# bryanlimy/tf2-cyclegan

Measured on AMD Instinct MI355X. Metric: images/sec (whole node) horse2zebra 256×256, higher is better.
Workload: dtype bf16; 1 GPU; model=cyclegan-resnet9-patchgan, global_batch=4, per_gpu_batch=4, image_size=256, parallelism=dp1

## Files before the change

cyclegan_amd/ops/_hip/bind.cpp:

```cpp
#include <torch/extension.h>

namespace cyg {
at::Tensor conv2d_fwd(at::Tensor, at::Tensor, c10::optional<at::Tensor>,
                      int64_t, int64_t, int64_t, int64_t, int64_t, bool,
                      int64_t, double);
at::Tensor convt2d_fwd(at::Tensor, at::Tensor, c10::optional<at::Tensor>,
                       int64_t, int64_t, int64_t, int64_t, int64_t, int64_t,
                       double);
at::Tensor conv2d_dgrad(at::Tensor, at::Tensor, int64_t, int64_t, int64_t,
                        int64_t, int64_t, int64_t, int64_t, bool);
at::Tensor convt2d_dgrad(at::Tensor, at::Tensor, int64_t, int64_t, int64_t,
                         int64_t, int64_t);
at::Tensor conv2d_wgrad(at::Tensor, at::Tensor, int64_t, int64_t, int64_t,
                        int64_t, int64_t, bool);
at::Tensor mfma_probe(at::Tensor, at::Tensor);
at::Tensor mx_probe(at::Tensor, at::Tensor, int64_t, int64_t);
at::Tensor mx_probe16(at::Tensor, at::Tensor, int64_t, int64_t);
at::Tensor glds_probe(at::Tensor, at::Tensor);
at::Tensor tr_probe(int64_t);
at::Tensor quant_fp8(at::Tensor, at::Tensor);
at::Tensor quant_fp8_d(at::Tensor, at::Tensor, at::Tensor);
void amax_roll(at::Tensor, int64_t);
at::Tensor conv2d_fp8_fwd(at::Tensor, at::Tensor, at::Tensor,
                          c10::optional<at::Tensor>, c10::optional<at::Tensor>,
                          int64_t, int64_t, int64_t, int64_t, int64_t, bool, int64_t, double);
std::vector<at::Tensor> instnorm_fwd(at::Tensor, at::Tensor, at::Tensor,
                                     double, int64_t, double,
                                     c10::optional<at::Tensor>);
std::vector<at::Tensor> instnorm_bwd(at::Tensor, at::Tensor, at::Tensor,
                                     at::Tensor, at::Tensor,
                                     c10::optional<at::Tensor>, int64_t,
                                     double);
at::Tensor act_bwd(at::Tensor, at::Tensor, int64_t, double);
at::Tensor channel_sum(at::Tensor);
at::Tensor reflect_pad_fwd(at::Tensor, int64_t, int64_t, int64_t, int64_t);
at::Tensor reflect_pad_bwd(at::Tensor, int64_t, int64_t, int64_t, int64_t);
at::Tensor persample_loss_fwd(at::Tensor, at::Tensor, bool);
at::Tensor persample_loss_const_fwd(at::Tensor, double, bool);
std::vector<at::Tensor> persample_loss_bwd(at::Tensor, at::Tensor, at::Tensor,
                                           bool, bool, bool);
at::Tensor persample_loss_const_bwd(at::Tensor, double, at::Tensor, bool);
void adam_step_dev(at::Tensor, at::Tensor, at::Tensor, at::Tensor, at::Tensor,
                   double, double, double);
void shadow_gather(at::Tensor, at::Tensor, at::Tensor);
void adam_step(at::Tensor, at::Tensor, at::Tensor, at::Tensor, double, double,
               double, double, int64_t);
}

PYBIND11_MODULE(TORCH_EXTENSION_NAME, m) {
  m.def("conv2d_fwd", &cyg::conv2d_fwd);
  m.def("convt2d_fwd", &cyg::convt2d_fwd);
  m.def("conv2d_dgrad", &cyg::conv2d_dgrad);
  m.def("convt2d_dgrad", &cyg::convt2d_dgrad);
  m.def("conv2d_wgrad", &cyg::conv2d_wgrad);
  m.def("mfma_probe", &cyg::mfma_probe);
  m.def("mx_probe", &cyg::mx_probe);
  m.def("mx_probe16", &cyg::mx_probe16);
  m.def("glds_probe", &cyg::glds_probe);
  m.def("tr_probe", &cyg::tr_probe);
  m.def("quant_fp8", &cyg::quant_fp8);
  m.def("quant_fp8_d", &cyg::quant_fp8_d);
  m.def("amax_roll", &cyg::amax_roll);
  m.def("conv2d_fp8_fwd", &cyg::conv2d_fp8_fwd);
  m.def("instnorm_fwd", &cyg::instnorm_fwd);
  m.def("instnorm_bwd", &cyg::instnorm_bwd);
  m.def("act_bwd", &cyg::act_bwd);
  m.def("channel_sum", &cyg::channel_sum);
  m.def("reflect_pad_fwd", &cyg::reflect_pad_fwd);
  m.def("reflect_pad_bwd", &cyg::reflect_pad_bwd);
  m.def("persample_loss_fwd", &cyg::persample_loss_fwd);
  m.def("persample_loss_const_fwd", &cyg::persample_loss_const_fwd);
  m.def("persample_loss_bwd", &cyg::persample_loss_bwd);
  m.def("persample_loss_const_bwd", &cyg::persample_loss_const_bwd);
  m.def("adam_step", &cyg::adam_step);
  m.def("adam_step_dev", &cyg::adam_step_dev);
  m.def("shadow_gather", &cyg::shadow_gather);
}
```

cyclegan_amd/ops/_hip/conv.hip:

```cpp

#include <torch/extension.h>
#include <ATen/cuda/CUDAContext.h>

#include "common.h"

namespace cyg {

constexpr int BM = 128, BN = 64, BK = 64;
constexpr int NTHREADS = 256;
constexpr int LDK = BK + 8;

struct ConvParams {
  const short* __restrict__ x;
  const short* __restrict__ w;
  const short* __restrict__ bias;
  short* __restrict__ y;
  int B, H, W, Cin, OH, OW, Cout, KH, KW;
  int stride, pt, pl;
  int reflect;
  int act;  float slope;
  const float* dq;
  const float* dqb;
  long M, KTOT;
  int mtiles, ntiles;
};

DEV int xcd_chunk(int bid, int nb) {
  return (nb % 8 == 0) ? (bid % 8) * (nb / 8) + bid / 8 : bid;
}


template <bool IS_CONVT, bool ALIGNED, int STRIDE>
__global__ __launch_bounds__(NTHREADS) void conv_gemm_kernel(ConvParams p) {
  const int stride = STRIDE ? STRIDE : p.stride;
  __shared__ short As[BM][LDK];
  __shared__ short Bs[BN][LDK];
  __shared__ long rowxb[BM];
  __shared__ long rowyb[BM];
  __shared__ int rowih[BM], rowiw[BM];
  __shared__ char rowok[BM];

  const int tid = threadIdx.x;
  const int lane = tid & 63;
  const int wid = tid >> 6;
  const int bid = xcd_chunk(blockIdx.x, gridDim.x);
  const int mt = bid % p.mtiles, nt = bid / p.mtiles;
  const long m0 = (long)mt * BM;
  const int n0 = nt * BN;

  for (int r = tid; r < BM; r += NTHREADS) {
    long m = m0 + r;
    bool ok = m < p.M;
    long mm = ok ? m : 0;
    int ow = (int)(mm % p.OW);
    int oh = (int)((mm / p.OW) % p.OH);
    int b = (int)(mm / ((long)p.OW * p.OH));
    rowok[r] = ok;
    rowxb[r] = (long)b * p.H * p.W * p.Cin;
    rowyb[r] = ((long)(b * p.OH + oh) * p.OW + ow) * p.Cout;
    if (IS_CONVT) {
      rowih[r] = oh + p.pt;
      rowiw[r] = ow + p.pl;
    } else {
      rowih[r] = oh * stride - p.pt;
      rowiw[r] = ow * stride - p.pl;
    }
  }
  __syncthreads();

  v4f acc[4][2] = {};

  const int wr = wid >> 1, wc = wid & 1;
  const int wm0 = wr * 64, wn0 = wc * 32;
  const int fr = lane & 15;
  const int fg = lane >> 4;

  for (long k0 = 0; k0 < p.KTOT; k0 += BK) {
    if (ALIGNED) {
      #pragma unroll 2
      for (int c = tid; c < BM * (BK / 8); c += NTHREADS) {
        int row = c >> 3;
        int kc = (c & 7) * 8;
        long k = k0 + kc;
        v8s val = {};
        if (k < p.KTOT && rowok[row]) {
          int tap = (int)(k / p.Cin);
          int ci = (int)(k - (long)tap * p.Cin);
          int dkh = tap / p.KW, dkw = tap - (tap / p.KW) * p.KW;
          bool valid = true;
          int ih, iw;
          if (IS_CONVT) {
            int nh = rowih[row] - dkh, nw = rowiw[row] - dkw;
            valid = nh >= 0 && nw >= 0 && (nh % stride) == 0 &&
                    (nw % stride) == 0;
            ih = nh / stride; iw = nw / stride;
            valid = valid && ih < p.H && iw < p.W;
          } else {
            ih = rowih[row] + dkh; iw = rowiw[row] + dkw;
            if (p.reflect) {
              ih = mirror_idx(ih, p.H); iw = mirror_idx(iw, p.W);
            } else {
              valid = ih >= 0 && ih < p.H && iw >= 0 && iw < p.W;
            }
          }
          if (valid)
            val = *(const v8s*)(p.x + rowxb[row] + ((long)ih * p.W + iw) * p.Cin + ci);
        }
        *(v8s*)&As[row][kc] = val;
      }
    } else {
      for (int c = tid; c < BM * BK; c += NTHREADS) {
        int row = c >> 6;
        int kc = c & 63;
        long k = k0 + kc;
        short val = 0;
        if (k < p.KTOT && rowok[row]) {
          int tap = (int)(k / p.Cin);
          int ci = (int)(k - (long)tap * p.Cin);
          int dkh = tap / p.KW, dkw = tap - (tap / p.KW) * p.KW;
          bool valid = true;
          int ih, iw;
          if (IS_CONVT) {
            int nh = rowih[row] - dkh, nw = rowiw[row] - dkw;
            valid = nh >= 0 && nw >= 0 && (nh % stride) == 0 &&
                    (nw % stride) == 0;
            ih = nh / stride; iw = nw / stride;
            valid = valid && ih < p.H && iw < p.W;
          } else {
            ih = rowih[row] + dkh; iw = rowiw[row] + dkw;
            if (p.reflect) {
              ih = mirror_idx(ih, p.H); iw = mirror_idx(iw, p.W);
            } else {
              valid = ih >= 0 && ih < p.H && iw >= 0 && iw < p.W;
            }
          }
          if (valid)
            val = p.x[rowxb[row] + ((long)ih * p.W + iw) * p.Cin + ci];
        }
        As[row][kc] = val;
      }
    }

    if (ALIGNED) {
      #pragma unroll 2
      for (int c = tid; c < BN * (BK / 8); c += NTHREADS) {
        int n = c >> 3;
        int kc = (c & 7) * 8;
        long k = k0 + kc;
        v8s val = {};
        if (n0 + n < p.Cout && k < p.KTOT)
          val = *(const v8s*)(p.w + (long)(n0 + n) * p.KTOT + k);
        *(v8s*)&Bs[n][kc] = val;
      }
    } else {
      for (int c = tid; c < BN * BK; c += NTHREADS) {
        int n = c >> 6;
        int kc = c & 63;
        long k = k0 + kc;
        Bs[n][kc] = (n0 + n < p.Cout && k < p.KTOT)
                        ? p.w[(long)(n0 + n) * p.KTOT + k] : (short)0;
      }
    }
    __syncthreads();

    #pragma unroll
    for (int kk = 0; kk < BK; kk += 32) {
      v8bf a0 = *(const v8bf*)&As[wm0 + 0 * 16 + fr][kk + fg * 8];
      v8bf a1 = *(const v8bf*)&As[wm0 + 1 * 16 + fr][kk + fg * 8];
      v8bf a2 = *(const v8bf*)&As[wm0 + 2 * 16 + fr][kk + fg * 8];
      v8bf a3 = *(const v8bf*)&As[wm0 + 3 * 16 + fr][kk + fg * 8];
      v8bf b0 = *(const v8bf*)&Bs[wn0 + 0 * 16 + fr][kk + fg * 8];
      v8bf b1 = *(const v8bf*)&Bs[wn0 + 1 * 16 + fr][kk + fg * 8];
      acc[0][0] = __builtin_amdgcn_mfma_f32_16x16x32_bf16(a0, b0, acc[0][0], 0, 0, 0);
      acc[0][1] = __builtin_amdgcn_mfma_f32_16x16x32_bf16(a0, b1, acc[0][1], 0, 0, 0);
      acc[1][0] = __builtin_amdgcn_mfma_f32_16x16x32_bf16(a1, b0, acc[1][0], 0, 0, 0);
      acc[1][1] = __builtin_amdgcn_mfma_f32_16x16x32_bf16(a1, b1, acc[1][1], 0, 0, 0);
      acc[2][0] = __builtin_amdgcn_mfma_f32_16x16x32_bf16(a2, b0, acc[2][0], 0, 0, 0);
      acc[2][1] = __builtin_amdgcn_mfma_f32_16x16x32_bf16(a2, b1, acc[2][1], 0, 0, 0);
      acc[3][0] = __builtin_amdgcn_mfma_f32_16x16x32_bf16(a3, b0, acc[3][0], 0, 0, 0);
      acc[3][1] = __builtin_amdgcn_mfma_f32_16x16x32_bf16(a3, b1, acc[3][1], 0, 0, 0);
    }
    __syncthreads();
  }

  #pragma unroll
  for (int nf = 0; nf < 2; ++nf) {
    int n = n0 + wn0 + nf * 16 + fr;
    if (n >= p.Cout) continue;
    float bv = p.bias ? b2f(p.bias[n]) : 0.f;
    #pragma unroll
    for (int mf = 0; mf < 4; ++mf) {
      #pragma unroll
      for (int r = 0; r < 4; ++r) {
        int rl = wm0 + mf * 16 + fg * 4 + r;
        if (!rowok[rl]) continue;
        float v = apply_act(acc[mf][nf][r] + bv, p.act, p.slope);
        p.y[rowyb[rl] + n] = f2b(v);
      }
    }
  }
}


template <int NBUF, int BNT = BN>
struct ConvSmemT {
  long rowyb[BM];
  int rowih[BM], rowiw[BM];
  unsigned rowxb[BM];
  char rowok[BM];
  char _pad[16 - (BM % 16 ? BM % 16 : 16)];
  short A[NBUF][BM * BK];
  short Bt[NBUF][BNT * BK];
};
using ConvSmem = ConvSmemT<2>;

template <bool IS_CONVT, int STRIDE, int NBUF = 2, int NW = 4, int BNT = BN,
          bool PHASED = false>
__global__ __launch_bounds__(NW * 64) void conv_glds_kernel(ConvParams p) {
  constexpr int NT = NW * 64;
  constexpr int API = 16 / NW;
  constexpr int TBI = BNT / 8;
  constexpr int BPI = TBI >= NW ? TBI / NW : 1;
  constexpr int NF = BNT >= 32 ? 2 : 1;
  constexpr int NWC = BNT / (NF * 16);
  constexpr int NWR = NW / NWC;
  constexpr int MF = (BM / NWR) / 16;
  const int stride = STRIDE ? STRIDE : p.stride;
  extern __shared__ __attribute__((aligned(16))) char smem_raw[];
  auto& sm = *reinterpret_cast<ConvSmemT<NBUF, BNT>*>(smem_raw);

  const int tid = threadIdx.x;
  const int lane = tid & 63;
  const int w = tid >> 6;
  const int bid = (IS_CONVT && STRIDE == 2)
                      ? blockIdx.x : xcd_chunk(blockIdx.x, gridDim.x);
  const int mt = bid % p.mtiles, nt = bid / p.mtiles;
  const int n0 = nt * BNT;

  static_assert(!PHASED || (IS_CONVT && STRIDE == 2), "PHASED");
  const int tpp = PHASED ? (p.mtiles >> 2) : 0;
  const int phase = PHASED ? mt / tpp : 0;
  const int phh = phase >> 1, phw = phase & 1;
  const int OH2 = p.OH >> 1, OW2 = p.OW >> 1;
  const long m0 = PHASED ? (long)(mt - phase * tpp) * BM : (long)mt * BM;
  const int nvh = PHASED ? ((p.KH - phh + 1) >> 1) : 0;
  const int nvw = PHASED ? ((p.KW - phw + 1) >> 1) : 0;
  const long KEFF = PHASED ? (long)nvh * nvw * p.Cin : p.KTOT;

  for (int r = tid; r < BM; r += NT) {
    if (PHASED) {
      long mp = m0 + r;
      long Mp = (long)p.B * OH2 * OW2;
      bool ok = mp < Mp;
      long mm = ok ? mp : 0;
      int owp = (int)(mm % OW2);
      int ohp = (int)((mm / OW2) % OH2);
      int b = (int)(mm / ((long)OW2 * OH2));
      int i = 2 * ohp + ((phh + p.pt) & 1);
      int j = 2 * owp + ((phw + p.pl) & 1);
      sm.rowok[r] = ok && i < p.OH && j < p.OW;
      sm.rowxb[r] = (unsigned)((long)b * p.H * p.W * p.Cin * 2);
      sm.rowyb[r] = ((long)(b * p.OH + i) * p.OW + j) * p.Cout;
      sm.rowih[r] = (i + p.pt - phh) >> 1;
      sm.rowiw[r] = (j + p.pl - phw) >> 1;
    } else {
      long m = m0 + r;
      bool ok = m < p.M;
      long mm = ok ? m : 0;
      int ow = (int)(mm % p.OW);
      int oh = (int)((mm / p.OW) % p.OH);
      int b = (int)(mm / ((long)p.OW * p.OH));
      sm.rowok[r] = ok;
      sm.rowxb[r] = (unsigned)((long)b * p.H * p.W * p.Cin * 2);
      sm.rowyb[r] = ((long)(b * p.OH + oh) * p.OW + ow) * p.Cout;
      if (IS_CONVT) {
        sm.rowih[r] = oh + p.pt;
        sm.rowiw[r] = ow + p.pl;
      } else {
        sm.rowih[r] = oh * stride - p.pt;
        sm.rowiw[r] = ow * stride - p.pl;
      }
    }
  }
  __syncthreads();

  const int lr = lane >> 3;
  const int klog = ((lane & 7) ^ lr) << 3;
  int aih[API], aiw[API];
  unsigned axb[API];
  bool aok[API];
  #pragma unroll
  for (int j = 0; j < API; ++j) {
    int r = (w * API + j) * 8 + lr;
    aih[j] = sm.rowih[r];
    aiw[j] = sm.rowiw[r];
    axb[j] = sm.rowxb[r];
    aok[j] = sm.rowok[r];
  }
  int bn[BPI];
  #pragma unroll
  for (int j = 0; j < BPI; ++j) bn[j] = (w * BPI + j) * 8 + lr + n0;
  const bool bw_on = w * BPI < TBI;
  static_assert(BNT == 16 || BNT == 64 || BNT == 128, "BNT");

  auto rx = __builtin_amdgcn_make_buffer_rsrc(
      (void*)p.x, 0, (unsigned)((long)p.B * p.H * p.W * p.Cin * 2), 0x00020000);
  auto rw = __builtin_amdgcn_make_buffer_rsrc(
      (void*)p.w, 0, (unsigned)(p.Cout * p.KTOT * 2), 0x00020000);

  const int nk = (int)((KEFF + BK - 1) / BK);
  const bool big_ci = p.Cin >= BK;

  long kcur;
  bool kv;
  int ci, dkh, dkw;
  unsigned avo[API];
  bool avalid[API];
  unsigned bvo[BPI];
  bool bnv[BPI];

  auto recompute_a = [&]() {
    #pragma unroll
    for (int j = 0; j < API; ++j) {
      avalid[j] = false;
      avo[j] = 0xFF000000u;
      if (!aok[j]) continue;
      bool valid = true;
      int ih, iw;
      if (PHASED) {
        ih = aih[j] - dkh; iw = aiw[j] - dkw;
        valid = ih >= 0 && iw >= 0 && ih < p.H && iw < p.W;
      } else if (IS_CONVT) {
        int nh = aih[j] - dkh, nw = aiw[j] - dkw;
        valid = nh >= 0 && nw >= 0 && (nh % stride) == 0 && (nw % stride) == 0;
        ih = nh / stride; iw = nw / stride;
        valid = valid && ih < p.H && iw < p.W;
      } else {
        ih = aih[j] + dkh; iw = aiw[j] + dkw;
        if (p.reflect) {
          ih = mirror_idx(ih, p.H); iw = mirror_idx(iw, p.W);
        } else {
          valid = ih >= 0 && ih < p.H && iw >= 0 && iw < p.W;
        }
      }
      if (valid) {
        avalid[j] = true;
        avo[j] = axb[j] + (unsigned)((((long)ih * p.W + iw) * p.Cin + ci) * 2);
      }
    }
  };

  auto recompute_b = [&]() {
    long kw_idx = kcur;
    if (PHASED)
      kw_idx = ((long)(2 * dkh + phh) * p.KW + (2 * dkw + phw)) * p.Cin + ci;
    #pragma unroll
    for (int j = 0; j < BPI; ++j)
      bvo[j] = (unsigned)(((long)bn[j] * p.KTOT + kw_idx) * 2);
  };

  auto decode_tap = [&]() {
    int tap = (int)(kcur / p.Cin);
    ci = (int)(kcur - (long)tap * p.Cin);
    if (PHASED) {
      dkh = tap / nvw;
      dkw = tap - dkh * nvw;
    } else {
      dkh = tap / p.KW;
      dkw = tap - dkh * p.KW;
    }
  };

  auto init_state = [&]() {
    kcur = klog;
    kv = kcur < KEFF;
    decode_tap();
    recompute_a();
    #pragma unroll
    for (int j = 0; j < BPI; ++j) bnv[j] = bn[j] < p.Cout;
    recompute_b();
  };

  auto advance = [&]() {
    kcur += BK;
    kv = kcur < KEFF;
    if (big_ci) {
      ci += BK;
      if (ci >= p.Cin) {
        ci -= p.Cin;
        if (PHASED) {
          if (++dkw == nvw) { dkw = 0; ++dkh; }
        } else {
          if (++dkw == p.KW) { dkw = 0; ++dkh; }
        }
        recompute_a();
        recompute_b();
      } else {
        #pragma unroll
        for (int j = 0; j < API; ++j) avo[j] += BK * 2;
        #pragma unroll
        for (int j = 0; j < BPI; ++j) bvo[j] += BK * 2;
      }
    } else {
      decode_tap();
      recompute_a();
      recompute_b();
    }
  };

  auto stage = [&](int buf) {
    #pragma unroll
    for (int j = 0; j < API; ++j) {
      unsigned vo = (kv && avalid[j]) ? avo[j] : 0xFF000000u;
      __builtin_amdgcn_raw_ptr_buffer_load_lds(
          rx, (__attribute__((address_space(3))) void*)&sm.A[buf][(w * API + j) * 512],
          16, vo, 0, 0, 0);
    }
    if (bw_on) {
      #pragma unroll
      for (int j = 0; j < BPI; ++j) {
        unsigned vo = (kv && bnv[j]) ? bvo[j] : 0xFF000000u;
        __builtin_amdgcn_raw_ptr_buffer_load_lds(
            rw, (__attribute__((address_space(3))) void*)&sm.Bt[buf][(w * BPI + j) * 512],
            16, vo, 0, 0, 0);
      }
    }
  };

  v4f acc[MF][NF] = {};
  const int wr = w / NWC, wc = w % NWC;
  const int wm0 = wr * (MF * 16), wn0 = wc * (NF * 16);
  const int fr = lane & 15;
  const int fg = lane >> 4;
  const int swz = (fr & 7) << 4;

  init_state();
  stage(0);
  __syncthreads();
#ifdef CYG_DEBUG_EPI
  if (bid == 0 && tid == 0)
    printf("dbg NW=%d BNT=%d API=%d TBI=%d BPI=%d NF=%d NWC=%d MF=%d nk=%d "
           "kv=%d klog=%d bvo0=%u bnv0=%d avo0=%u avalid0=%d "
           "A0123=%d %d %d %d Bt0123=%d %d %d %d\n",
           NW, BNT, API, TBI, BPI, NF, NWC, MF, nk, (int)kv, klog, bvo[0],
           (int)bnv[0], avo[0], (int)avalid[0],
           (int)sm.A[0][0], (int)sm.A[0][1], (int)sm.A[0][2], (int)sm.A[0][3],
           (int)sm.Bt[0][0], (int)sm.Bt[0][1], (int)sm.Bt[0][2],
           (int)sm.Bt[0][3]);
#endif

  for (int kt = 0; kt < nk; ++kt) {
    if (kt + 1 < nk) {
      advance();
      stage((kt + 1) & 1);
    }
    const char* Ab = (const char*)sm.A[kt & 1];
    const char* Bb = (const char*)sm.Bt[kt & 1];
    #pragma unroll
    for (int kk = 0; kk < BK; kk += 32) {
      const int kbyte = (kk + fg * 8) * 2;
      v8bf a[MF], b[NF];
      #pragma unroll
      for (int mf = 0; mf < MF; ++mf)
        a[mf] = *(const v8bf*)(Ab + ((wm0 + mf * 16 + fr) << 7) + (kbyte ^ swz));
      #pragma unroll
      for (int nf = 0; nf < NF; ++nf)
        b[nf] = *(const v8bf*)(Bb + ((wn0 + nf * 16 + fr) << 7) + (kbyte ^ swz));
      #pragma unroll
      for (int mf = 0; mf < MF; ++mf)
        #pragma unroll
        for (int nf = 0; nf < NF; ++nf)
          acc[mf][nf] = __builtin_amdgcn_mfma_f32_16x16x32_bf16(
              a[mf], b[nf], acc[mf][nf], 0, 0, 0);
    }
    __syncthreads();
  }

  #pragma unroll
  for (int nf = 0; nf < NF; ++nf) {
    int n = n0 + wn0 + nf * 16 + fr;
    if (n >= p.Cout) continue;
    float bv = p.bias ? b2f(p.bias[n]) : 0.f;
    #pragma unroll
    for (int mf = 0; mf < MF; ++mf) {
      #pragma unroll
      for (int r = 0; r < 4; ++r) {
        int rl = wm0 + mf * 16 + fg * 4 + r;
        if (!sm.rowok[rl]) continue;
#ifdef CYG_DEBUG_EPI
        if (sm.rowyb[rl] < 0 || sm.rowyb[rl] + n >= p.M * p.Cout) {
          printf("EPI OOB bid=%d tid=%d rl=%d rowyb=%ld n=%d\n",
                 bid, tid, rl, (long)sm.rowyb[rl], n);
          continue;
        }
#endif
        float v = apply_act(acc[mf][nf][r] + bv, p.act, p.slope);
        p.y[sm.rowyb[rl] + n] = f2b(v);
      }
    }
  }
}

constexpr int HB_BM = 64;

template <int NW = 4>
__global__ __launch_bounds__(NW * 64) void conv_halo_kernel(ConvParams p) {
  constexpr int NT = NW * 64;
  const int tid = threadIdx.x;
  const int lane = tid & 63;
  const int w = tid >> 6;
  const int tiles_w = (p.OW + HB_BM - 1) / HB_BM;
  const int bid = xcd_chunk(blockIdx.x, gridDim.x);
  const int owt = bid % tiles_w;
  const int t2 = bid / tiles_w;
  const int oh = t2 % p.OH;
  const int b = t2 / p.OH;
  const int ow0 = owt * HB_BM;
  const int CW = HB_BM + p.KW - 1;
  constexpr int CG = 8;
  constexpr int SL = CG + 1;
  constexpr int halves = 2;
  const int nk = p.KH * p.KW * halves;

  extern __shared__ __attribute__((aligned(16))) char smem_raw[];
  short* xs = (short*)smem_raw;
  const int xgr = p.KH * CW * SL;
  const int xgr_pad = ((xgr + NT - 1) / NT) * NT;

  auto rx = __builtin_amdgcn_make_buffer_rsrc(
      (void*)p.x, 0, (unsigned)((long)p.B * p.H * p.W * p.Cin * 2),
      0x00020000);

  const long xbase = (long)b * p.H * p.W * p.Cin;
  {
    int g = w * 64 + lane;
    int chs = g % SL;
    int pix = g / SL;
    int col = pix % CW;
    int row = pix / CW;
    constexpr int dpix = NT / SL;
    constexpr int dchs = NT - dpix * SL;
    for (int g0 = 0; g0 < xgr_pad; g0 += NT) {
      unsigned vo = 0xFF000000u;
      if (row < p.KH && chs < CG) {
        int ih = oh - p.pt + row;
        int iw = ow0 - p.pl + col;
        bool okp = true;
        if (p.reflect) {
          ih = mirror_idx(ih, p.H);
          iw = mirror_idx(iw, p.W);
        } else {
          okp = ih >= 0 && ih < p.H && iw >= 0 && iw < p.W;
        }
        if (okp)
          vo = (unsigned)((xbase + ((long)ih * p.W + iw) * p.Cin + chs * 8) * 2);
      }
      __builtin_amdgcn_raw_ptr_buffer_load_lds(
          rx, (__attribute__((address_space(3))) void*)(xs + (long)(g0 + w * 64) * 8),
          16, vo, 0, 0, 0);
      chs += dchs;
      col += dpix;
      if (chs >= SL) { chs -= SL; ++col; }
      while (col >= CW) { col -= CW; ++row; }
    }
  }

  __syncthreads();

  constexpr int KSPLIT = NW >= 8 ? 2 : 1;
  const int mf = KSPLIT > 1 ? (w & 3) : w;
  const int kh2 = KSPLIT > 1 ? (w >> 2) : 0;
  const int fr = lane & 15;
  const int fg = lane >> 4;
  const int p0 = mf * 16;
  const v8bf bz = {};
  v4f acc = {};
  const int k0 = kh2 * (nk / KSPLIT);
  const int k1 = (kh2 == KSPLIT - 1) ? nk : (kh2 + 1) * (nk / KSPLIT);
  int tap = k0 / halves, h = k0 - tap * halves;
  int ty = tap / p.KW, tx = tap - ty * p.KW;
  #pragma unroll 8
  for (int kt = k0; kt < k1; ++kt) {
    int col = p0 + fr + tx;
    int chs = h * 4 + fg;
    v8bf a = *(const v8bf*)(xs + (((ty * CW + col) * SL + chs) << 3));
    v8bf bf = bz;
    if (fr < 8)
      bf = *(const v8bf*)(p.w + (long)fr * p.KTOT + kt * 32 + fg * 8);
    acc = __builtin_amdgcn_mfma_f32_16x16x32_bf16(a, bf, acc, 0, 0, 0);
    if (++h == halves) {
      h = 0;
      ++tap;
      if (++tx == p.KW) { tx = 0; ++ty; }
    }
  }

  if (KSPLIT > 1) {
    __syncthreads();
    float* red = (float*)xs;
    if (kh2 == 1)
      *(v4f*)&red[(mf * 64 + lane) * 4] = acc;
    __syncthreads();
    if (kh2 != 0) return;
    acc += *(const v4f*)&red[(mf * 64 + lane) * 4];
  }

  if (fr < p.Cout) {
    float bv = p.bias ? b2f(p.bias[fr]) : 0.f;
    #pragma unroll
    for (int r = 0; r < 4; ++r) {
      int ow = ow0 + p0 + fg * 4 + r;
      if (ow >= p.OW) continue;
      float v = apply_act(acc[r] + bv, p.act, p.slope);
      p.y[(((long)b * p.OH + oh) * p.OW + ow) * p.Cout + fr] = f2b(v);
    }
  }
}


#include <hip/hip_fp8.h>

constexpr int BKF = 128;
typedef int v4i __attribute__((ext_vector_type(4)));
typedef int v8i __attribute__((ext_vector_type(8)));

struct Fp8Smem {
  unsigned char A[2][BM * BKF];
  unsigned char Bt[2][BN * BKF];
  long rowyb[BM];
  int rowih[BM], rowiw[BM];
  unsigned rowxb[BM];
  char rowok[BM];
};

__global__ void quant_fp8_kernel(const short* __restrict__ x,
                                 const float* __restrict__ scale,
                                 unsigned char* __restrict__ y, long n) {
  long i = ((long)blockIdx.x * blockDim.x + threadIdx.x) * 8;
  float s = scale[0];
  if (i + 8 <= n) {
    v8s v = *(const v8s*)(x + i);
    unsigned char out[8];
    #pragma unroll
    for (int j = 0; j < 8; ++j) {
      __hip_fp8_e4m3 q(b2f(v[j]) * s);
      out[j] = q.__x;
    }
    *(uint2*)(y + i) = *(uint2*)out;
  } else if (i < n) {
    for (long k = i; k < n; ++k) {
      __hip_fp8_e4m3 q(b2f(x[k]) * scale[0]);
      y[k] = q.__x;
    }
  }
}

DEV float delayed_sx(float amax_prev) {
  return fminf(448.f / fmaxf(amax_prev, 1e-12f), 65504.f);
}

__global__ __launch_bounds__(256) void quant_fp8_d_kernel(
    const short* __restrict__ x, const float* __restrict__ amax_prev,
    float* __restrict__ amax_cur, unsigned char* __restrict__ y, long n) {
  const float s = delayed_sx(amax_prev[0]);
  float mx = 0.f;
  long t = (long)blockIdx.x * 256 + threadIdx.x;
  long nthreads = (long)gridDim.x * 256;
  for (long i = t * 8; i + 8 <= n; i += nthreads * 8) {
    v8s v = *(const v8s*)(x + i);
    unsigned char out[8];
    #pragma unroll
    for (int j = 0; j < 8; ++j) {
      float f = b2f(v[j]);
      mx = fmaxf(mx, fabsf(f));
      __hip_fp8_e4m3 q(f * s);
      out[j] = q.__x;
    }
    *(uint2*)(y + i) = *(uint2*)out;
  }
  if (blockIdx.x == 0 && threadIdx.x == 0) {
    for (long k = n & ~7L; k < n; ++k) {
      float f = b2f(x[k]);
      mx = fmaxf(mx, fabsf(f));
      __hip_fp8_e4m3 q(f * s);
      y[k] = q.__x;
    }
  }
  __shared__ float red[256];
  red[threadIdx.x] = mx;
  __syncthreads();
  for (int off = 128; off > 0; off >>= 1) {
    if (threadIdx.x < off)
      red[threadIdx.x] = fmaxf(red[threadIdx.x], red[threadIdx.x + off]);
    __syncthreads();
  }
  if (threadIdx.x == 0)
    atomicMax((unsigned*)amax_cur, __float_as_uint(red[0]));
}

__global__ void amax_roll_kernel(float* __restrict__ arena, int n, int cap) {
  int i = blockIdx.x * blockDim.x + threadIdx.x;
  if (i < n) {
    arena[i] = arena[cap + i];
    arena[cap + i] = 0.f;
  }
}

template <int STRIDE>
__global__ __launch_bounds__(NTHREADS) void conv_fp8_kernel(ConvParams p) {
  const int stride = STRIDE ? STRIDE : p.stride;
  __shared__ Fp8Smem sm;

  const int tid = threadIdx.x;
  const int lane = tid & 63;
  const int w = tid >> 6;
  const int bid = xcd_chunk(blockIdx.x, gridDim.x);
  const int mt = bid % p.mtiles, nt = bid / p.mtiles;
  const long m0 = (long)mt * BM;
  const int n0 = nt * BN;
  const bool reflect = p.reflect != 0;

  for (int r = tid; r < BM; r += NTHREADS) {
    long m = m0 + r;
    bool ok = m < p.M;
    long mm = ok ? m : 0;
    int ow = (int)(mm % p.OW);
    int oh = (int)((mm / p.OW) % p.OH);
    int b = (int)(mm / ((long)p.OW * p.OH));
    sm.rowok[r] = ok;
    sm.rowxb[r] = (unsigned)((long)b * p.H * p.W * p.Cin);
    sm.rowyb[r] = ((long)(b * p.OH + oh) * p.OW + ow) * p.Cout;
    sm.rowih[r] = oh * stride - p.pt;
    sm.rowiw[r] = ow * stride - p.pl;
  }
  __syncthreads();

  const int lr = lane >> 3;
  const int klog = ((lane & 7) ^ lr) << 4;
  int aih[4], aiw[4];
  unsigned axb[4];
  bool aok[4];
  #pragma unroll
  for (int j = 0; j < 4; ++j) {
    int r = w * 32 + j * 8 + lr;
    aih[j] = sm.rowih[r];
    aiw[j] = sm.rowiw[r];
    axb[j] = sm.rowxb[r];
    aok[j] = sm.rowok[r];
  }
  const int bn[2] = {(w * 2 + 0) * 8 + lr + n0, (w * 2 + 1) * 8 + lr + n0};

  auto rx = __builtin_amdgcn_make_buffer_rsrc(
      (void*)p.x, 0, (unsigned)((long)p.B * p.H * p.W * p.Cin), 0x00020000);
  auto rw = __builtin_amdgcn_make_buffer_rsrc(
      (void*)p.w, 0, (unsigned)(p.Cout * p.KTOT), 0x00020000);

  const int nk = (int)((p.KTOT + BKF - 1) / BKF);
  const bool big_ci = p.Cin >= BKF;

  long kcur;
  bool kv;
  int ci, dkh, dkw;
  unsigned avo[4], bvo[2];
  bool avalid[4], bnv[2];

  auto recompute_a = [&]() {
    #pragma unroll
    for (int j = 0; j < 4; ++j) {
      avalid[j] = false;
      avo[j] = 0xFF000000u;
      if (!aok[j]) continue;
      bool valid = true;
      int ih = aih[j] + dkh, iw = aiw[j] + dkw;
      if (reflect) {
        ih = mirror_idx(ih, p.H); iw = mirror_idx(iw, p.W);
      } else {
        valid = ih >= 0 && ih < p.H && iw >= 0 && iw < p.W;
      }
      if (valid) {
        avalid[j] = true;
        avo[j] = axb[j] + (unsigned)(((long)ih * p.W + iw) * p.Cin + ci);
      }
    }
  };

  auto init_state = [&]() {
    kcur = klog;
    kv = kcur < p.KTOT;
    int tap = (int)(kcur / p.Cin);
    ci = (int)(kcur - (long)tap * p.Cin);
    dkh = tap / p.KW;
    dkw = tap - dkh * p.KW;
    recompute_a();
    #pragma unroll
    for (int j = 0; j < 2; ++j) {
      bnv[j] = bn[j] < p.Cout;
      bvo[j] = (unsigned)((long)bn[j] * p.KTOT + kcur);
    }
  };

  auto advance = [&]() {
    kcur += BKF;
    kv = kcur < p.KTOT;
    #pragma unroll
    for (int j = 0; j < 2; ++j) bvo[j] += BKF;
    if (big_ci) {
      ci += BKF;
      if (ci >= p.Cin) {
        ci -= p.Cin;
        if (++dkw == p.KW) { dkw = 0; ++dkh; }
        recompute_a();
      } else {
        #pragma unroll
        for (int j = 0; j < 4; ++j) avo[j] += BKF;
      }
    } else {
      int tap = (int)(kcur / p.Cin);
      ci = (int)(kcur - (long)tap * p.Cin);
      dkh = tap / p.KW;
      dkw = tap - dkh * p.KW;
      recompute_a();
    }
  };

  auto stage = [&](int buf) {
    #pragma unroll
    for (int j = 0; j < 4; ++j) {
      unsigned vo = (kv && avalid[j]) ? avo[j] : 0xFF000000u;
      __builtin_amdgcn_raw_ptr_buffer_load_lds(
          rx, (__attribute__((address_space(3))) void*)&sm.A[buf][(w * 4 + j) * 1024],
          16, vo, 0, 0, 0);
    }
    #pragma unroll
    for (int j = 0; j < 2; ++j) {
      unsigned vo = (kv && bnv[j]) ? bvo[j] : 0xFF000000u;
      __builtin_amdgcn_raw_ptr_buffer_load_lds(
          rw, (__attribute__((address_space(3))) void*)&sm.Bt[buf][(w * 2 + j) * 1024],
          16, vo, 0, 0, 0);
    }
  };

  v4f acc[4][2] = {};
  const int wr = w >> 1, wc = w & 1;
  const int wm0 = wr * 64, wn0 = wc * 32;
  const int fr = lane & 15;
  const int fg = lane >> 4;
  const int swz = (fr & 7) << 4;

  init_state();
  stage(0);
  __syncthreads();

  for (int kt = 0; kt < nk; ++kt) {
    if (kt + 1 < nk) {
      advance();
      stage((kt + 1) & 1);
    }
    const char* Ab = (const char*)sm.A[kt & 1];
    const char* Bb = (const char*)sm.Bt[kt & 1];
    {
      const int c0 = (fg * 32) ^ swz;
      const int c1 = (fg * 32 + 16) ^ swz;
      v8i fa[4], fb[2];
      #pragma unroll
      for (int mf = 0; mf < 4; ++mf) {
        const char* r = Ab + ((wm0 + mf * 16 + fr) << 7);
        v4i lo = *(const v4i*)(r + c0);
        v4i hi = *(const v4i*)(r + c1);
        fa[mf] = __builtin_shufflevector(lo, hi, 0, 1, 2, 3, 4, 5, 6, 7);
      }
      #pragma unroll
      for (int nf = 0; nf < 2; ++nf) {
        const char* r = Bb + ((wn0 + nf * 16 + fr) << 7);
        v4i lo = *(const v4i*)(r + c0);
        v4i hi = *(const v4i*)(r + c1);
        fb[nf] = __builtin_shufflevector(lo, hi, 0, 1, 2, 3, 4, 5, 6, 7);
      }
      #pragma unroll
      for (int mf = 0; mf < 4; ++mf)
        #pragma unroll
        for (int nf = 0; nf < 2; ++nf)
          acc[mf][nf] = __builtin_amdgcn_mfma_scale_f32_16x16x128_f8f6f4(
              fa[mf], fb[nf], acc[mf][nf], 0, 0, 0, 127, 0, 127);
    }
    __syncthreads();
  }

  const float dqs = p.dq
      ? (p.dqb ? 1.f / (delayed_sx(p.dq[0]) * p.dqb[0]) : p.dq[0])
      : 1.f;
  #pragma unroll
  for (int nf = 0; nf < 2; ++nf) {
    int n = n0 + wn0 + nf * 16 + fr;
    if (n >= p.Cout) continue;
    float bv = p.bias ? b2f(p.bias[n]) : 0.f;
    #pragma unroll
    for (int mf = 0; mf < 4; ++mf) {
      #pragma unroll
      for (int r = 0; r < 4; ++r) {
        int rl = wm0 + mf * 16 + fg * 4 + r;
        if (!sm.rowok[rl]) continue;
        float v = apply_act(acc[mf][nf][r] * dqs + bv, p.act, p.slope);
        p.y[sm.rowyb[rl] + n] = f2b(v);
      }
    }
  }
}


struct WgradParams {
  const short* __restrict__ x;
  const short* __restrict__ dy;
  float* __restrict__ dw;
  float* __restrict__ ws;
  int B, H, W, Cin, OH, OW, Cout, KH, KW;
  int stride, pt, pl, reflect;
  long M, KTOT;
  int ktiles, ntiles, slices;
  long mchunks_per_slice;
};

constexpr int WG_BK = 128;
constexpr int WG_BN = 64;
constexpr int WG_BM = 64;
constexpr int WG_LDM = WG_BM + 8;

__global__ __launch_bounds__(NTHREADS) void wgrad_kernel(WgradParams p) {
  __shared__ short At[WG_BK][WG_LDM];
  __shared__ short Dt[WG_BN][WG_LDM];
  __shared__ int mih[2][WG_BM], miw[2][WG_BM];
  __shared__ long mxb[2][WG_BM];
  __shared__ char mok[2][WG_BM];

  const int tid = threadIdx.x;
  const int lane = tid & 63;
  const int wid = tid >> 6;
  const int wbid = xcd_chunk(blockIdx.x, gridDim.x);
  const int kt = wbid % p.ktiles;
  const int nt = (wbid / p.ktiles) % p.ntiles;
  const int sl = wbid / (p.ktiles * p.ntiles);
  const long k0 = (long)kt * WG_BK;
  const int n0 = nt * WG_BN;
  const long mstart = sl * p.mchunks_per_slice * WG_BM;
  long mend = mstart + p.mchunks_per_slice * WG_BM;
  if (mend > p.M) mend = p.M;

  v4f acc[4][2] = {};
  const int wr = wid >> 1, wc = wid & 1;
  const int wk0 = wr * 64, wn0 = wc * 32;
  const int fr = lane & 15, fg = lane >> 4;

  const bool a_vec = (p.Cin % 8) == 0;
  const bool d_vec = (p.Cout % 8) == 0;

  if (a_vec && d_vec && mstart < mend) {
    const int a_mloc = (tid & 15) * 4, a_kc = (tid >> 4) * 8;
    const int d_mloc = (tid & 31) * 2, d_nc = (tid >> 5) * 8;
    const long ak = k0 + a_kc;
    const bool akv = ak < p.KTOT;
    int tap = akv ? (int)(ak / p.Cin) : 0;
    const int ci = (int)(ak - (long)tap * p.Cin);
    const int dkh = tap / p.KW, dkw = tap - (tap / p.KW) * p.KW;
    const bool dnv = n0 + d_nc < p.Cout;

    auto decode = [&](int buf, long ms) {
      for (int r = tid; r < WG_BM; r += NTHREADS) {
        bool ok = ms + r < p.M;
        int mm = ok ? (int)(ms + r) : 0;
        int ow = mm % p.OW;
        int t = mm / p.OW;
        int oh = t % p.OH;
        int b = t / p.OH;
        mok[buf][r] = ok;
        mih[buf][r] = oh * p.stride - p.pt;
        miw[buf][r] = ow * p.stride - p.pl;
        mxb[buf][r] = (long)b * p.H * p.W * p.Cin;
      }
    };

    const v8s VZERO = {};
    v8s areg[4], dreg[2];
    auto load_regs = [&](int buf, long ms) {
      #pragma unroll
      for (int u = 0; u < 4; ++u) {
        areg[u] = VZERO;
        if (akv && mok[buf][a_mloc + u]) {
          int ih = mih[buf][a_mloc + u] + dkh;
          int iw = miw[buf][a_mloc + u] + dkw;
          bool valid = true;
          if (p.reflect) {
            ih = mirror_idx(ih, p.H); iw = mirror_idx(iw, p.W);
          } else {
            valid = ih >= 0 && ih < p.H && iw >= 0 && iw < p.W;
          }
          if (valid)
            areg[u] = *(const v8s*)(p.x + mxb[buf][a_mloc + u] +
                                    ((long)ih * p.W + iw) * p.Cin + ci);
        }
      }
      #pragma unroll
      for (int u = 0; u < 2; ++u) {
        dreg[u] = VZERO;
        long m = ms + d_mloc + u;
        if (dnv && m < p.M)
          dreg[u] = *(const v8s*)(p.dy + m * p.Cout + n0 + d_nc);
      }
    };

    decode(0, mstart);
    __syncthreads();
    load_regs(0, mstart);

    int cur = 0;
    for (long ms = mstart; ms < mend; ms += WG_BM, cur ^= 1) {
      #pragma unroll
      for (int j = 0; j < 8; ++j) {
        short pa[4] = {areg[0][j], areg[1][j], areg[2][j], areg[3][j]};
        *(uint2*)&At[a_kc + j][a_mloc] = *(uint2*)pa;
        short pd[2] = {dreg[0][j], dreg[1][j]};
        *(unsigned*)&Dt[d_nc + j][d_mloc] = *(unsigned*)pd;
      }
      bool more = ms + WG_BM < mend;
      if (more) decode(cur ^ 1, ms + WG_BM);
      __syncthreads();
      if (more) load_regs(cur ^ 1, ms + WG_BM);
      #pragma unroll
      for (int kk = 0; kk < WG_BM; kk += 32) {
        v8bf a0 = *(const v8bf*)&At[wk0 + 0 * 16 + fr][kk + fg * 8];
        v8bf a1 = *(const v8bf*)&At[wk0 + 1 * 16 + fr][kk + fg * 8];
        v8bf a2 = *(const v8bf*)&At[wk0 + 2 * 16 + fr][kk + fg * 8];
        v8bf a3 = *(const v8bf*)&At[wk0 + 3 * 16 + fr][kk + fg * 8];
        v8bf b0 = *(const v8bf*)&Dt[wn0 + 0 * 16 + fr][kk + fg * 8];
        v8bf b1 = *(const v8bf*)&Dt[wn0 + 1 * 16 + fr][kk + fg * 8];
        acc[0][0] = __builtin_amdgcn_mfma_f32_16x16x32_bf16(a0, b0, acc[0][0], 0, 0, 0);
        acc[0][1] = __builtin_amdgcn_mfma_f32_16x16x32_bf16(a0, b1, acc[0][1], 0, 0, 0);
        acc[1][0] = __builtin_amdgcn_mfma_f32_16x16x32_bf16(a1, b0, acc[1][0], 0, 0, 0);
        acc[1][1] = __builtin_amdgcn_mfma_f32_16x16x32_bf16(a1, b1, acc[1][1], 0, 0, 0);
        acc[2][0] = __builtin_amdgcn_mfma_f32_16x16x32_bf16(a2, b0, acc[2][0], 0, 0, 0);
        acc[2][1] = __builtin_amdgcn_mfma_f32_16x16x32_bf16(a2, b1, acc[2][1], 0, 0, 0);
        acc[3][0] = __builtin_amdgcn_mfma_f32_16x16x32_bf16(a3, b0, acc[3][0], 0, 0, 0);
        acc[3][1] = __builtin_amdgcn_mfma_f32_16x16x32_bf16(a3, b1, acc[3][1], 0, 0, 0);
      }
      __syncthreads();
    }

    #pragma unroll
    for (int nf = 0; nf < 2; ++nf) {
      int n = n0 + wn0 + nf * 16 + fr;
      if (n >= p.Cout) continue;
      #pragma unroll
      for (int kf = 0; kf < 4; ++kf) {
        #pragma unroll
        for (int r = 0; r < 4; ++r) {
          long k = k0 + wk0 + kf * 16 + fg * 4 + r;
          if (k < p.KTOT)
            atomicAdd(&p.dw[(long)n * p.KTOT + k], acc[kf][nf][r]);
        }
      }
    }
    return;
  }

  for (long ms = mstart; ms < mend; ms += WG_BM) {
    __syncthreads();
    for (int r = tid; r < WG_BM; r += NTHREADS) {
      int m = (int)(ms + r);
      bool ok = ms + r < p.M;
      int mm = ok ? m : 0;
      int ow = mm % p.OW;
      int t = mm / p.OW;
      int oh = t % p.OH;
      int b = t / p.OH;
      mok[0][r] = ok;
      mih[0][r] = oh * p.stride - p.pt;
      miw[0][r] = ow * p.stride - p.pl;
      mxb[0][r] = (long)b * p.H * p.W * p.Cin;
    }
    __syncthreads();
    {
      for (int c = tid; c < WG_BK * 8; c += NTHREADS) {
        int krow = c >> 3;
        int mc = (c & 7) * 8;
        long k = k0 + krow;
        short vals[8];
        int tap = 0, ci = 0, dkh = 0, dkw = 0;
        bool krows_ok = k < p.KTOT;
        if (krows_ok) {
          tap = (int)(k / p.Cin);
          ci = (int)(k - (long)tap * p.Cin);
          dkh = tap / p.KW; dkw = tap - dkh * p.KW;
        }
        #pragma unroll
        for (int j = 0; j < 8; ++j) {
          long m = ms + mc + j;
          short v = 0;
          if (krows_ok && m < p.M) {
            int ow = (int)(m % p.OW);
            int oh = (int)((m / p.OW) % p.OH);
            int b = (int)(m / ((long)p.OW * p.OH));
            int ih = oh * p.stride - p.pt + dkh;
            int iw = ow * p.stride - p.pl + dkw;
            bool valid = true;
            if (p.reflect) {
              ih = mirror_idx(ih, p.H); iw = mirror_idx(iw, p.W);
            } else {
              valid = ih >= 0 && ih < p.H && iw >= 0 && iw < p.W;
            }
            if (valid)
              v = p.x[(((long)b * p.H + ih) * p.W + iw) * p.Cin + ci];
          }
          vals[j] = v;
        }
        *(v8s*)&At[krow][mc] = *(v8s*)vals;
      }
    }
    if (d_vec) {
      for (int c = tid; c < (WG_BM / 2) * (WG_BN / 8); c += NTHREADS) {
        int m_loc = (c % (WG_BM / 2)) * 2;
        int nc = (c / (WG_BM / 2)) * 8;
        v8s v0 = {}, v1 = {};
        if (n0 + nc < p.Cout) {
          long m = ms + m_loc;
          if (m < p.M) v0 = *(const v8s*)(p.dy + m * p.Cout + n0 + nc);
          if (m + 1 < p.M) v1 = *(const v8s*)(p.dy + (m + 1) * p.Cout + n0 + nc);
        }
        #pragma unroll
        for (int j = 0; j < 8; ++j) {
          short pack[2] = {v0[j], v1[j]};
          *(unsigned*)&Dt[nc + j][m_loc] = *(unsigned*)pack;
        }
      }
    } else {
      for (int c = tid; c < WG_BN * 8; c += NTHREADS) {
        int n = c >> 3;
        int mc = (c & 7) * 8;
        short vals[8];
        #pragma unroll
        for (int j = 0; j < 8; ++j) {
          long m = ms + mc + j;
          vals[j] = (n0 + n < p.Cout && m < p.M)
                        ? p.dy[m * p.Cout + n0 + n] : (short)0;
        }
        *(v8s*)&Dt[n][mc] = *(v8s*)vals;
      }
    }
    __syncthreads();

    #pragma unroll
    for (int kk = 0; kk < WG_BM; kk += 32) {
      v8bf a0 = *(const v8bf*)&At[wk0 + 0 * 16 + fr][kk + fg * 8];
      v8bf a1 = *(const v8bf*)&At[wk0 + 1 * 16 + fr][kk + fg * 8];
      v8bf a2 = *(const v8bf*)&At[wk0 + 2 * 16 + fr][kk + fg * 8];
      v8bf a3 = *(const v8bf*)&At[wk0 + 3 * 16 + fr][kk + fg * 8];
      v8bf b0 = *(const v8bf*)&Dt[wn0 + 0 * 16 + fr][kk + fg * 8];
      v8bf b1 = *(const v8bf*)&Dt[wn0 + 1 * 16 + fr][kk + fg * 8];
      acc[0][0] = __builtin_amdgcn_mfma_f32_16x16x32_bf16(a0, b0, acc[0][0], 0, 0, 0);
      acc[0][1] = __builtin_amdgcn_mfma_f32_16x16x32_bf16(a0, b1, acc[0][1], 0, 0, 0);
      acc[1][0] = __builtin_amdgcn_mfma_f32_16x16x32_bf16(a1, b0, acc[1][0], 0, 0, 0);
      acc[1][1] = __builtin_amdgcn_mfma_f32_16x16x32_bf16(a1, b1, acc[1][1], 0, 0, 0);
      acc[2][0] = __builtin_amdgcn_mfma_f32_16x16x32_bf16(a2, b0, acc[2][0], 0, 0, 0);
      acc[2][1] = __builtin_amdgcn_mfma_f32_16x16x32_bf16(a2, b1, acc[2][1], 0, 0, 0);
      acc[3][0] = __builtin_amdgcn_mfma_f32_16x16x32_bf16(a3, b0, acc[3][0], 0, 0, 0);
      acc[3][1] = __builtin_amdgcn_mfma_f32_16x16x32_bf16(a3, b1, acc[3][1], 0, 0, 0);
    }
    __syncthreads();
  }

  #pragma unroll
  for (int nf = 0; nf < 2; ++nf) {
    int n = n0 + wn0 + nf * 16 + fr;
    if (n >= p.Cout) continue;
    #pragma unroll
    for (int kf = 0; kf < 4; ++kf) {
      #pragma unroll
      for (int r = 0; r < 4; ++r) {
        long k = k0 + wk0 + kf * 16 + fg * 4 + r;
        if (k < p.KTOT)
          atomicAdd(&p.dw[(long)n * p.KTOT + k], acc[kf][nf][r]);
      }
    }
  }
}


typedef bf16r v4bfx __attribute__((ext_vector_type(4)));

#define AXOR(row) ((((row) & 7) << 5) | ((((row) >> 3) & 1) << 4))
#define DXOR(row) ((((row) & 3) << 5) | ((((row) >> 3) & 1) << 4))

DEV v4bfx tr16_read(const char* plds) {
  return __builtin_amdgcn_ds_read_tr16_b64_v4bf16(
      (__attribute__((address_space(3))) v4bfx*)plds);
}

template <int WBN, int KT = 1>
struct WgSmemT {
  short A[2][KT * WG_BM * WG_BK];
  short D[2][WG_BM * WBN];
};

template <int NW = 4, int WBN = 64, int KT = 1>
__global__ __launch_bounds__(NW * 64) void wgrad_glds_kernel(WgradParams p) {
  constexpr int API = 16 / NW;
  constexpr int AT = KT * API;
  constexpr int DCH = WBN / 8;
  constexpr int DRPI = 64 / DCH;
  constexpr int TDI = (WG_BM * DCH) / 64;
  constexpr int DPI = TDI >= NW ? TDI / NW : 1;
  constexpr int NFW = (NW == 4 && WBN == 128) ? 4 : (WBN >= 32 ? 2 : 1);
  constexpr int NWCW = WBN / (NFW * 16);
  constexpr int KF = (WG_BK / (NW / NWCW)) / 16;
  extern __shared__ __attribute__((aligned(16))) char wg_smem_raw[];
  auto& sm = *reinterpret_cast<WgSmemT<WBN, KT>*>(wg_smem_raw);

  const int tid = threadIdx.x;
  const int lane = tid & 63;
  const int w = tid >> 6;
  const int wbid = xcd_chunk(blockIdx.x, gridDim.x);
  const int pairs = p.ktiles / KT;
  const int ktp = wbid % pairs;
  const int kt = ktp * KT;
  const int nt = (wbid / pairs) % p.ntiles;
  const int sl = wbid / (pairs * p.ntiles);
  const long k0 = (long)kt * WG_BK;
  const int n0 = nt * WBN;
  const long mstart = sl * p.mchunks_per_slice * WG_BM;
  long mend = mstart + p.mchunks_per_slice * WG_BM;
  if (mend > p.M) mend = p.M;
  if (mstart >= mend) {
    for (int t = 0; t < KT; ++t) {
      long chunk = (((long)sl * p.ktiles + kt + t) * p.ntiles + nt) *
                   ((long)WBN * WG_BK);
      for (int i = tid; i < WBN * WG_BK; i += NW * 64) p.ws[chunk + i] = 0.f;
    }
    return;
  }

  auto rx = __builtin_amdgcn_make_buffer_rsrc(
      (void*)p.x, 0, (unsigned)((long)p.B * p.H * p.W * p.Cin * 2), 0x00020000);
  auto rd = __builtin_amdgcn_make_buffer_rsrc(
      (void*)p.dy, 0, (unsigned)(p.M * p.Cout * 2), 0x00020000);

  int a_row[AT], a_ci[AT], a_dkh[AT], a_dkw[AT];
  bool a_kv[AT];
  #pragma unroll
  for (int t = 0; t < KT; ++t) {
    #pragma unroll
    for (int j = 0; j < API; ++j) {
      int sidx = t * API + j;
      int row = (w * API + j) * 4 + (lane >> 4);
      int cb = ((lane & 15) * 16) ^ AXOR(row);
      long k = k0 + (long)t * WG_BK + cb / 2;
      a_row[sidx] = row;
      a_kv[sidx] = k < p.KTOT;
      int tap = a_kv[sidx] ? (int)(k / p.Cin) : 0;
      a_ci[sidx] = (int)(k - (long)tap * p.Cin);
      a_dkh[sidx] = tap / p.KW;
      a_dkw[sidx] = tap - a_dkh[sidx] * p.KW;
    }
  }
  const bool dw_on = w * DPI < TDI;
  int d_row[DPI], d_n[DPI];
  #pragma unroll
  for (int j = 0; j < DPI; ++j) {
    int row = (w * DPI + j) * DRPI + lane / DCH;
    int cb = ((lane % DCH) * 16) ^
             (WBN == 128 ? AXOR(row) : WBN == 64 ? DXOR(row) : 0);
    d_row[j] = row;
    d_n[j] = n0 + cb / 2;
  }

  const unsigned C2 = (unsigned)p.Cin * 2;
  const unsigned WC2 = (unsigned)p.W * C2;
  int a_ow[AT], a_oh[AT], a_b[AT], a_ih[AT], a_iw[AT];
  unsigned avo[AT];
  bool ainb[AT], avalid[AT], a_iw_ok[AT];
  unsigned dvo[DPI];

  auto full_a = [&](int j) {
    int ih = a_ih[j], iw = a_iw[j];
    bool valid = a_kv[j];
    if (p.reflect) {
      ih = mirror_idx(ih, p.H); iw = mirror_idx(iw, p.W);
    } else {
      valid = valid && ih >= 0 && ih < p.H && iw >= 0 && iw < p.W;
    }
    avalid[j] = valid;
    avo[j] = valid ? (unsigned)(((((long)a_b[j] * p.H + ih) * p.W + iw) *
                                 p.Cin + a_ci[j]) * 2)
                   : 0xFF000000u;
  };

  #pragma unroll
  for (int j = 0; j < AT; ++j) {
    long m = mstart + a_row[j];
    a_ow[j] = (int)(m % p.OW);
    int t = (int)(m / p.OW);
    a_oh[j] = t % p.OH;
    a_b[j] = t / p.OH;
    a_ih[j] = a_oh[j] * p.stride - p.pt + a_dkh[j];
    a_iw[j] = a_ow[j] * p.stride - p.pl + a_dkw[j];
    a_iw_ok[j] = (unsigned)a_iw[j] < (unsigned)p.W;
    ainb[j] = (unsigned)a_ih[j] < (unsigned)p.H && a_iw_ok[j];
    full_a(j);
  }
  #pragma unroll
  for (int j = 0; j < DPI; ++j)
    dvo[j] = d_n[j] < p.Cout
                 ? (unsigned)(((mstart + d_row[j]) * p.Cout + d_n[j]) * 2)
                 : 0xFF000000u;

  const bool ow_fast = (p.OW == WG_BM);
  const unsigned sWC2 = (unsigned)(p.stride * (int)WC2);
  auto advance = [&]() {
    if (ow_fast) {
      #pragma unroll
      for (int j = 0; j < AT; ++j) {
        bool rare = (++a_oh[j] >= p.OH);
        if (!rare) {
          int ih = a_ih[j] + p.stride;
          a_ih[j] = ih;
          bool inb = (unsigned)ih < (unsigned)p.H;
          if (inb && ainb[j] && avalid[j]) {
            avo[j] += sWC2;
          } else {
            rare = true;
          }
          ainb[j] = inb && a_iw_ok[j];
        }
        if (rare) {
          while (a_oh[j] >= p.OH) { a_oh[j] -= p.OH; ++a_b[j]; }
          a_ih[j] = a_oh[j] * p.stride - p.pt + a_dkh[j];
          full_a(j);
          ainb[j] = ((unsigned)a_ih[j] < (unsigned)p.H) && a_iw_ok[j];
        }
      }
    } else {
      #pragma unroll
      for (int j = 0; j < AT; ++j) {
        int ow0 = a_ow[j], oh0 = a_oh[j], b0 = a_b[j];
        a_ow[j] += WG_BM;
        while (a_ow[j] >= p.OW) { a_ow[j] -= p.OW; ++a_oh[j]; }
        while (a_oh[j] >= p.OH) { a_oh[j] -= p.OH; ++a_b[j]; }
        int dih = (a_oh[j] - oh0) * p.stride;
        int diw = (a_ow[j] - ow0) * p.stride;
        a_ih[j] += dih;
        a_iw[j] += diw;
        bool inb = (unsigned)a_ih[j] < (unsigned)p.H &&
                   (unsigned)a_iw[j] < (unsigned)p.W;
        if (a_b[j] == b0 && inb && ainb[j] && avalid[j]) {
          avo[j] += (unsigned)(dih * (int)WC2 + diw * (int)C2);
        } else {
          full_a(j);
        }
        ainb[j] = inb;
      }
    }
    #pragma unroll
    for (int j = 0; j < DPI; ++j) dvo[j] += (unsigned)(WG_BM * p.Cout * 2);
  };

  auto stage = [&](int buf, long ms, bool tail) {
    #pragma unroll
    for (int t = 0; t < KT; ++t) {
      #pragma unroll
      for (int j = 0; j < API; ++j) {
        int sidx = t * API + j;
        unsigned vo = (!tail || ms + a_row[sidx] < p.M) ? avo[sidx]
                                                        : 0xFF000000u;
        __builtin_amdgcn_raw_ptr_buffer_load_lds(
            rx, (__attribute__((address_space(3))) void*)
                &sm.A[buf][t * (WG_BM * WG_BK) + (w * API + j) * 512],
            16, vo, 0, 0, 0);
      }
    }
    if (dw_on) {
      #pragma unroll
      for (int j = 0; j < DPI; ++j) {
        unsigned vo = (!tail || ms + d_row[j] < p.M) ? dvo[j] : 0xFF000000u;
        __builtin_amdgcn_raw_ptr_buffer_load_lds(
            rd, (__attribute__((address_space(3))) void*)&sm.D[buf][(w * DPI + j) * 512],
            16, vo, 0, 0, 0);
      }
    }
  };

  v4f acc[KT][KF][NFW] = {};
  const int wr = w / NWCW, wc = w % NWCW;
  const int wk0 = wr * (KF * 16), wn0 = wc * (NFW * 16);
  const int fr = lane & 15, fg = lane >> 4;
  const int jg = lane & 15;
  const int tr_row_a = jg >> 2;
  const int tr_cb_a = (jg & 3) * 8;

  int a_base[KF][2], d_base[NFW][2];
  #pragma unroll
  for (int kf = 0; kf < KF; ++kf) {
    #pragma unroll
    for (int h = 0; h < 2; ++h) {
      int row = fg * 8 + tr_row_a + 4 * h;
      int cbl = (wk0 + kf * 16) * 2 + tr_cb_a;
      a_base[kf][h] = row * 256 + (cbl ^ AXOR(row));
    }
  }
  #pragma unroll
  for (int nf = 0; nf < NFW; ++nf) {
    #pragma unroll
    for (int h = 0; h < 2; ++h) {
      int row = fg * 8 + tr_row_a + 4 * h;
      int cbl = (wn0 + nf * 16) * 2 + tr_cb_a;
      d_base[nf][h] = row * (WBN * 2) +
          (cbl ^ (WBN == 128 ? AXOR(row) : WBN == 64 ? DXOR(row) : 0));
    }
  }

  stage(0, mstart, mstart + WG_BM > p.M);
  __syncthreads();

  int cur = 0;
  for (long ms = mstart; ms < mend; ms += WG_BM, cur ^= 1) {
    if (ms + WG_BM < mend) {
      advance();
      stage(cur ^ 1, ms + WG_BM, ms + 2 * WG_BM > p.M);
    }
    const char* Ab = (const char*)sm.A[cur];
    const char* Db = (const char*)sm.D[cur];
    #pragma unroll
    for (int kk = 0; kk < WG_BM; kk += 32) {
      v8bf bfr[NFW];
      #pragma unroll
      for (int nf = 0; nf < NFW; ++nf) {
        v4bfx lo = tr16_read(Db + kk * (WBN * 2) + d_base[nf][0]);
        v4bfx hi = tr16_read(Db + kk * (WBN * 2) + d_base[nf][1]);
        bfr[nf] = __builtin_shufflevector(lo, hi, 0, 1, 2, 3, 4, 5, 6, 7);
      }
      #pragma unroll
      for (int t = 0; t < KT; ++t) {
        const char* At = Ab + t * (WG_BM * WG_BK * 2);
        v8bf a[KF];
        #pragma unroll
        for (int kf = 0; kf < KF; ++kf) {
          v4bfx lo = tr16_read(At + kk * 256 + a_base[kf][0]);
          v4bfx hi = tr16_read(At + kk * 256 + a_base[kf][1]);
          a[kf] = __builtin_shufflevector(lo, hi, 0, 1, 2, 3, 4, 5, 6, 7);
        }
        #pragma unroll
        for (int kf = 0; kf < KF; ++kf)
          #pragma unroll
          for (int nf = 0; nf < NFW; ++nf)
            acc[t][kf][nf] = __builtin_amdgcn_mfma_f32_16x16x32_bf16(
                a[kf], bfr[nf], acc[t][kf][nf], 0, 0, 0);
      }
    }
    __syncthreads();
  }

  #pragma unroll
  for (int t = 0; t < KT; ++t) {
    long chunk = (((long)sl * p.ktiles + kt + t) * p.ntiles + nt) *
                 ((long)WBN * WG_BK);
    #pragma unroll
    for (int nf = 0; nf < NFW; ++nf) {
      int nl = wn0 + nf * 16 + fr;
      if (nl >= WBN) continue;
      #pragma unroll
      for (int kf = 0; kf < KF; ++kf) {
        int kl = wk0 + kf * 16 + fg * 4;
        *(float4*)&p.ws[chunk + (long)nl * WG_BK + kl] =
            *(const float4*)&acc[t][kf][nf];
      }
    }
  }
}

__global__ void wgrad_reduce_kernel(const float* __restrict__ ws,
                                    float* __restrict__ dw, long KTOT,
                                    int Cout, int ktiles, int ntiles,
                                    int slices, int wbn) {
  long idx = (long)blockIdx.x * blockDim.x + threadIdx.x;
  long total = (long)ktiles * WG_BK * ntiles * wbn;
  if (idx >= total) return;
  int kl = (int)(idx % WG_BK);
  long t = idx / WG_BK;
  int kt = (int)(t % ktiles);
  t /= ktiles;
  int nl = (int)(t % wbn);
  int nt = (int)(t / wbn);
  long k = (long)kt * WG_BK + kl;
  int n = nt * wbn + nl;
  if (k >= KTOT || n >= Cout) return;
  long stride = (long)ktiles * ntiles * wbn * WG_BK;
  long off = (((long)kt * ntiles + nt) * wbn + nl) * WG_BK + kl;
  float s0 = 0, s1 = 0, s2 = 0, s3 = 0;
  int sl = 0;
  for (; sl + 4 <= slices; sl += 4) {
    s0 += ws[off + (sl + 0) * stride];
    s1 += ws[off + (sl + 1) * stride];
    s2 += ws[off + (sl + 2) * stride];
    s3 += ws[off + (sl + 3) * stride];
  }
  for (; sl < slices; ++sl) s0 += ws[off + sl * stride];
  dw[(long)n * KTOT + k] = (s0 + s1) + (s2 + s3);
}

__global__ void reflect_fold_kernel(const short* __restrict__ dxp,
                                    short* __restrict__ dx,
                                    int B, int H, int W, int C,
                                    int pt, int pb, int pl, int pr) {
  long idx = (long)blockIdx.x * blockDim.x + threadIdx.x;
  int gpr = C / 8;
  long total = (long)B * H * W * gpr;
  if (idx >= total) return;
  int g = (int)(idx % gpr);
  long t = idx / gpr;
  int j = (int)(t % W);
  t /= W;
  int i = (int)(t % H);
  int b = (int)(t / H);
  int HP = H + pt + pb, WP = W + pl + pr;
  float s[8] = {};
  int hc[3] = {pt + i, pt - i, pt + 2 * (H - 1) - i};
  int wc_[3] = {pl + j, pl - j, pl + 2 * (W - 1) - j};
  #pragma unroll
  for (int a = 0; a < 3; ++a) {
    int qh = hc[a];
    if (qh < 0 || qh >= HP) continue;
    if (a > 0 && qh == hc[0]) continue;
    if (a == 2 && qh == hc[1]) continue;
    if (mirror_idx(qh - pt, H) != i) continue;
    #pragma unroll
    for (int d = 0; d < 3; ++d) {
      int qw = wc_[d];
      if (qw < 0 || qw >= WP) continue;
      if (d > 0 && qw == wc_[0]) continue;
      if (d == 2 && qw == wc_[1]) continue;
      if (mirror_idx(qw - pl, W) != j) continue;
      v8s v = *(const v8s*)(dxp + (((long)b * HP + qh) * WP + qw) * C + g * 8);
      #pragma unroll
      for (int e = 0; e < 8; ++e) s[e] += b2f(v[e]);
    }
  }
  v8s out;
  #pragma unroll
  for (int e = 0; e < 8; ++e) out[e] = f2b(s[e]);
  *(v8s*)(dx + (((long)b * H + i) * W + j) * C + g * 8) = out;
}


static inline int cdiv(long a, long b) { return (int)((a + b - 1) / b); }

template <bool IS_CONVT, bool ALIGNED>
static void launch_conv_s(const ConvParams& p, dim3 grid, hipStream_t stream) {
  switch (p.stride) {
    case 1:
      hipLaunchKernelGGL((conv_gemm_kernel<IS_CONVT, ALIGNED, 1>), grid,
                         dim3(NTHREADS), 0, stream, p);
      break;
    case 2:
      hipLaunchKernelGGL((conv_gemm_kernel<IS_CONVT, ALIGNED, 2>), grid,
                         dim3(NTHREADS), 0, stream, p);
      break;
    default:
      hipLaunchKernelGGL((conv_gemm_kernel<IS_CONVT, ALIGNED, 0>), grid,
                         dim3(NTHREADS), 0, stream, p);
  }
}

static int conv_nw() {
  static int v = []() {
    const char* e = getenv("CYG_CONV_NW");
    return e ? atoi(e) : 8;
  }();
  return v;
}

static int conv_bn() {
  static int v = []() {
    const char* e = getenv("CYG_CONV_BN");
    return e ? atoi(e) : 128;
  }();
  return v;
}

template <bool IS_CONVT, int STRIDE, int NBUF, int NW, int BNT,
          bool PHASED = false>
static void launch_one_glds(const ConvParams& p, dim3 grid,
                            hipStream_t stream) {
  constexpr size_t SMB = sizeof(ConvSmemT<NBUF, BNT>);
  static bool init = []() {
    hipFuncSetAttribute(
        (const void*)(conv_glds_kernel<IS_CONVT, STRIDE, NBUF, NW, BNT,
                                       PHASED>),
        hipFuncAttributeMaxDynamicSharedMemorySize, (int)SMB);
    return true;
  }();
  (void)init;
  hipLaunchKernelGGL(
      (conv_glds_kernel<IS_CONVT, STRIDE, NBUF, NW, BNT, PHASED>), grid,
      dim3(NW * 64), SMB, stream, p);
  hipError_t err = hipGetLastError();
  TORCH_CHECK(err == hipSuccess, "conv_glds launch failed (NW=", NW,
              " BNT=", BNT, " PHASED=", PHASED, "): ",
              hipGetErrorString(err));
}

template <bool IS_CONVT>
static void launch_glds_s(const ConvParams& p, dim3 grid, hipStream_t stream) {
  if constexpr (!IS_CONVT) {
    static const bool use_halo = []() {
      const char* e = getenv("CYG_HALO");
      return e && atoi(e) != 0;
    }();
    if (use_halo && p.Cout == 8 && p.stride == 1 && p.Cin == 64) {
      const int CW = HB_BM + p.KW - 1;
      const int xgr = p.KH * CW * 9;
      const int xgr_pad = ((xgr + 511) / 512) * 512;
      const size_t smb = (size_t)xgr_pad * 16;
      if (smb <= 150 * 1024) {
        static bool init = []() {
          hipFuncSetAttribute((const void*)(conv_halo_kernel<8>),
                              hipFuncAttributeMaxDynamicSharedMemorySize,
                              150 * 1024);
          return true;
        }();
        (void)init;
        const int tiles_w = (p.OW + HB_BM - 1) / HB_BM;
        dim3 gh((long)p.B * p.OH * tiles_w);
        hipLaunchKernelGGL((conv_halo_kernel<8>), gh, dim3(512), smb,
                           stream, p);
        hipError_t err = hipGetLastError();
        TORCH_CHECK(err == hipSuccess, "conv_halo launch failed: ",
                    hipGetErrorString(err));
        return;
      }
    }
  }
  if (p.Cout <= 16) {
    ConvParams q = p;
    q.ntiles = (p.Cout + 15) / 16;
    dim3 g2((long)q.mtiles * q.ntiles);
    switch (p.stride) {
      case 1: launch_one_glds<IS_CONVT, 1, 2, 8, 16>(q, g2, stream); return;
      case 2: launch_one_glds<IS_CONVT, 2, 2, 8, 16>(q, g2, stream); return;
      default: launch_one_glds<IS_CONVT, 0, 2, 8, 16>(q, g2, stream); return;
    }
  }
  if (conv_nw() == 8 && conv_bn() == 128 && (p.Cout % 128) == 0) {
    ConvParams q = p;
    q.ntiles = (p.Cout + 127) / 128;
    dim3 g2((long)q.mtiles * q.ntiles);
    switch (p.stride) {
      case 1: launch_one_glds<IS_CONVT, 1, 2, 8, 128>(q, g2, stream); return;
      case 2: launch_one_glds<IS_CONVT, 2, 2, 8, 128>(q, g2, stream); return;
      default: launch_one_glds<IS_CONVT, 0, 2, 8, 128>(q, g2, stream); return;
    }
  }
  if (conv_nw() == 8) {
    switch (p.stride) {
      case 1: launch_one_glds<IS_CONVT, 1, 2, 8, 64>(p, grid, stream); return;
      case 2: launch_one_glds<IS_CONVT, 2, 2, 8, 64>(p, grid, stream); return;
      default: launch_one_glds<IS_CONVT, 0, 2, 8, 64>(p, grid, stream); return;
    }
  }
  switch (p.stride) {
    case 1: launch_one_glds<IS_CONVT, 1, 2, 4, 64>(p, grid, stream); break;
    case 2: launch_one_glds<IS_CONVT, 2, 2, 4, 64>(p, grid, stream); break;
    default: launch_one_glds<IS_CONVT, 0, 2, 4, 64>(p, grid, stream);
  }
}

static void launch_conv(const ConvParams& p, bool is_convt, hipStream_t stream) {
  dim3 grid(p.mtiles * p.ntiles);
  bool aligned = (p.Cin % 8) == 0;
  bool glds_ok = aligned &&
                 (long)p.B * p.H * p.W * p.Cin * 2 < (1L << 31) &&
                 (long)p.Cout * p.KTOT * 2 < (1L << 31);
  if (glds_ok && is_convt && p.stride == 2 && (p.OH % 2) == 0 &&
      (p.OW % 2) == 0) {
    ConvParams q = p;
    long Mp = (long)q.B * (q.OH / 2) * (q.OW / 2);
    q.mtiles = 4 * cdiv(Mp, BM);
    if (conv_nw() == 8 && conv_bn() == 128 && (q.Cout % 128) == 0) {
      q.ntiles = (q.Cout + 127) / 128;
      dim3 g2((long)q.mtiles * q.ntiles);
      launch_one_glds<true, 2, 2, 8, 128, true>(q, g2, stream);
    } else if (conv_nw() == 8) {
      dim3 g2((long)q.mtiles * q.ntiles);
      launch_one_glds<true, 2, 2, 8, 64, true>(q, g2, stream);
    } else {
      dim3 g2((long)q.mtiles * q.ntiles);
      launch_one_glds<true, 2, 2, 4, 64, true>(q, g2, stream);
    }
    return;
  }
  if (glds_ok) {
    if (is_convt) launch_glds_s<true>(p, grid, stream);
    else launch_glds_s<false>(p, grid, stream);
    return;
  }
  if (is_convt) {
    if (aligned) launch_conv_s<true, true>(p, grid, stream);
    else launch_conv_s<true, false>(p, grid, stream);
  } else {
    if (aligned) launch_conv_s<false, true>(p, grid, stream);
    else launch_conv_s<false, false>(p, grid, stream);
  }
}

static ConvParams fill_common(const at::Tensor& x, const at::Tensor& w,
                              const c10::optional<at::Tensor>& bias,
                              at::Tensor& y, int stride, int act, double slope) {
  ConvParams p{};
  p.x = (const short*)x.const_data_ptr();
  p.w = (const short*)w.const_data_ptr();
  p.bias = bias.has_value() ? (const short*)bias->const_data_ptr() : nullptr;
  p.y = (short*)y.mutable_data_ptr();
  p.B = x.size(0); p.H = x.size(1); p.W = x.size(2); p.Cin = x.size(3);
  p.OH = y.size(1); p.OW = y.size(2); p.Cout = y.size(3);
  p.KH = w.size(1); p.KW = w.size(2);
  p.stride = stride;
  p.act = act; p.slope = (float)slope;
  p.M = (long)p.B * p.OH * p.OW;
  p.KTOT = (long)p.KH * p.KW * p.Cin;
  p.mtiles = cdiv(p.M, BM);
  p.ntiles = cdiv(p.Cout, BN);
  return p;
}

static void check_conv_inputs(const at::Tensor& x, const at::Tensor& w) {
  TORCH_CHECK(x.is_cuda() && w.is_cuda(), "conv: tensors must be on GPU");
  TORCH_CHECK(x.scalar_type() == at::kBFloat16 && w.scalar_type() == at::kBFloat16,
              "conv: GPU path is bf16 (got ", x.scalar_type(), ")");
  TORCH_CHECK(x.is_contiguous() && w.is_contiguous(), "conv: need contiguous");
  TORCH_CHECK(w.size(3) == x.size(3), "conv: Cin mismatch");
}

at::Tensor conv2d_fwd(at::Tensor x, at::Tensor w, c10::optional<at::Tensor> bias,
                      int64_t stride, int64_t pt, int64_t pb, int64_t pl,
                      int64_t pr, bool reflect, int64_t act, double slope) {
  check_conv_inputs(x, w);
  int H = x.size(1), W = x.size(2);
  int KH = w.size(1), KW = w.size(2);
  int OH = (H + pt + pb - KH) / stride + 1;
  int OW = (W + pl + pr - KW) / stride + 1;
  auto y = at::empty({x.size(0), OH, OW, w.size(0)}, x.options());
  auto p = fill_common(x, w, bias, y, stride, act, slope);
  p.pt = pt; p.pl = pl; p.reflect = reflect ? 1 : 0;
  launch_conv(p, false, at::cuda::getCurrentCUDAStream());
  return y;
}

at::Tensor convt2d_fwd(at::Tensor x, at::Tensor w, c10::optional<at::Tensor> bias,
                       int64_t stride, int64_t pt, int64_t pl,
                       int64_t out_h, int64_t out_w, int64_t act, double slope) {
  check_conv_inputs(x, w);
  auto y = at::empty({x.size(0), out_h, out_w, w.size(0)}, x.options());
  auto p = fill_common(x, w, bias, y, stride, act, slope);
  p.pt = pt; p.pl = pl; p.reflect = 0;
  launch_conv(p, true, at::cuda::getCurrentCUDAStream());
  return y;
}

at::Tensor conv2d_dgrad(at::Tensor dy, at::Tensor wt, int64_t H, int64_t W,
                        int64_t stride, int64_t pt, int64_t pb, int64_t pl,
                        int64_t pr, bool reflect) {
  check_conv_inputs(dy, wt);
  auto stream = at::cuda::getCurrentCUDAStream();
  if (!reflect) {
    auto dx = at::empty({dy.size(0), H, W, wt.size(0)}, dy.options());
    auto p = fill_common(dy, wt, c10::nullopt, dx, stride, ACT_NONE, 0.0);
    p.pt = pt; p.pl = pl;
    launch_conv(p, true, stream);
    return dx;
  }
  long HP = H + pt + pb, WP = W + pl + pr;
  auto dxp = at::empty({dy.size(0), HP, WP, wt.size(0)}, dy.options());
  auto p = fill_common(dy, wt, c10::nullopt, dxp, stride, ACT_NONE, 0.0);
  p.pt = 0; p.pl = 0;
  launch_conv(p, true, stream);
  auto dx = at::empty({dy.size(0), H, W, wt.size(0)}, dy.options());
  TORCH_CHECK(wt.size(0) % 8 == 0, "reflect dgrad: Cin % 8 != 0");
  long total = dx.numel() / 8;
  int threads = 256;
  hipLaunchKernelGGL(reflect_fold_kernel, dim3(cdiv(total, threads)),
                     dim3(threads), 0, stream,
                     (const short*)dxp.const_data_ptr(),
                     (short*)dx.mutable_data_ptr(),
                     (int)dy.size(0), (int)H, (int)W, (int)wt.size(0),
                     (int)pt, (int)pb, (int)pl, (int)pr);
  return dx;
}

at::Tensor convt2d_dgrad(at::Tensor dy, at::Tensor wt, int64_t IH, int64_t IW,
                         int64_t stride, int64_t pt, int64_t pl) {
  check_conv_inputs(dy, wt);
  int KH = wt.size(1), KW = wt.size(2);
  auto dx = at::empty({dy.size(0), IH, IW, wt.size(0)}, dy.options());
  auto p = fill_common(dy, wt, c10::nullopt, dx, stride, ACT_NONE, 0.0);
  p.pt = pt; p.pl = pl; p.reflect = 0;
  launch_conv(p, false, at::cuda::getCurrentCUDAStream());
  return dx;
}

at::Tensor conv2d_wgrad(at::Tensor x, at::Tensor dy, int64_t KH, int64_t KW,
                        int64_t stride, int64_t pt, int64_t pl, bool reflect) {
  TORCH_CHECK(x.is_cuda() && dy.is_cuda() && x.is_contiguous() && dy.is_contiguous());
  TORCH_CHECK(x.scalar_type() == at::kBFloat16 && dy.scalar_type() == at::kBFloat16);
  TORCH_CHECK(dy.size(0) == x.size(0));
  WgradParams p{};
  p.x = (const short*)x.const_data_ptr();
  p.dy = (const short*)dy.const_data_ptr();
  p.B = x.size(0); p.H = x.size(1); p.W = x.size(2); p.Cin = x.size(3);
  p.OH = dy.size(1); p.OW = dy.size(2); p.Cout = dy.size(3);
  p.KH = KH; p.KW = KW; p.stride = stride; p.pt = pt; p.pl = pl;
  p.reflect = reflect ? 1 : 0;
  p.M = (long)p.B * p.OH * p.OW;
  p.KTOT = (long)KH * KW * p.Cin;
  p.ktiles = cdiv(p.KTOT, WG_BK);
  p.ntiles = cdiv(p.Cout, WG_BN);
  long mchunks = (p.M + WG_BM - 1) / WG_BM;
  static int tgt_blocks = []() {
    const char* e = getenv("CYG_WG_BLOCKS");
    return e ? atoi(e) : 512;
  }();
  int target = std::max<long>(1, tgt_blocks / ((long)p.ktiles * p.ntiles));
  int slices = (int)std::min<long>(mchunks, target);
  p.mchunks_per_slice = (mchunks + slices - 1) / slices;
  p.slices = (int)((mchunks + p.mchunks_per_slice - 1) / p.mchunks_per_slice);
  dim3 grid((long)p.ktiles * p.ntiles * p.slices);
  bool glds_ok = (p.Cin % 8) == 0 && (p.Cout % 8) == 0 &&
                 (long)p.B * p.H * p.W * p.Cin * 2 < (1L << 31) &&
                 p.M * p.Cout * 2 < (1L << 31);
  auto stream = at::cuda::getCurrentCUDAStream();
  if (glds_ok) {
    auto dw = at::empty({p.Cout, (long)KH, (long)KW, p.Cin},
                        x.options().dtype(at::kFloat));
    p.dw = (float*)dw.mutable_data_ptr();
    int wbn = (conv_nw() == 8 && conv_bn() == 128 && (p.Cout % 128) == 0)
                  ? 128 : WG_BN;
    if (p.Cout <= 16) wbn = 16;
    if (wbn != WG_BN) {
      p.ntiles = (p.Cout + wbn - 1) / wbn;
      long mchunks = (p.M + WG_BM - 1) / WG_BM;
      static int tgt2 = []() {
        const char* e = getenv("CYG_WG_BLOCKS");
        return e ? atoi(e) : 512;
      }();
      int target = std::max<long>(1, tgt2 / ((long)p.ktiles * p.ntiles));
      p.slices = (int)std::min<long>(mchunks, target);
      p.mchunks_per_slice = (mchunks + p.slices - 1) / p.slices;
      p.slices = (int)((mchunks + p.mchunks_per_slice - 1) /
                       p.mchunks_per_slice);
      grid = dim3((long)p.ktiles * p.ntiles * p.slices);
    }
    static int wg_nw = []() {
      const char* e = getenv("CYG_WG_NW");
      return e ? atoi(e) : 8;
    }();
    static int wg_kt = []() {
      const char* e = getenv("CYG_WG_KT");
      return e ? atoi(e) : 1;
    }();
    bool kt2 = wbn == 128 && wg_nw == 8 && wg_kt == 2 &&
               (p.ktiles % 2) == 0;
    if (kt2) {
      long mchunks2 = (p.M + WG_BM - 1) / WG_BM;
      int pairs = p.ktiles / 2;
      int target2 =
          std::max<long>(1, tgt_blocks / ((long)pairs * p.ntiles));
      p.slices = (int)std::min<long>(mchunks2, target2);
      p.mchunks_per_slice = (mchunks2 + p.slices - 1) / p.slices;
      p.slices = (int)((mchunks2 + p.mchunks_per_slice - 1) /
                       p.mchunks_per_slice);
      grid = dim3((long)pairs * p.ntiles * p.slices);
    }
    auto ws = at::empty({(long)p.slices * p.ktiles * p.ntiles *
                         wbn * WG_BK},
                        x.options().dtype(at::kFloat));
    p.ws = (float*)ws.mutable_data_ptr();
    if (wbn == 128) {
      constexpr size_t SMB = sizeof(WgSmemT<128>);
      constexpr size_t SMB2 = sizeof(WgSmemT<128, 2>);
      static bool init = []() {
        hipFuncSetAttribute((const void*)(wgrad_glds_kernel<8, 128>),
                            hipFuncAttributeMaxDynamicSharedMemorySize,
                            (int)SMB);
        hipFuncSetAttribute((const void*)(wgrad_glds_kernel<4, 128>),
                            hipFuncAttributeMaxDynamicSharedMemorySize,
                            (int)SMB);
        hipFuncSetAttribute((const void*)(wgrad_glds_kernel<8, 128, 2>),
                            hipFuncAttributeMaxDynamicSharedMemorySize,
                            (int)SMB2);
        return true;
      }();
      (void)init;
      if (kt2)
        hipLaunchKernelGGL((wgrad_glds_kernel<8, 128, 2>), grid, dim3(512),
                           SMB2, stream, p);
      else if (wg_nw == 4)
        hipLaunchKernelGGL((wgrad_glds_kernel<4, 128>), grid, dim3(256), SMB,
                           stream, p);
      else
        hipLaunchKernelGGL((wgrad_glds_kernel<8, 128>), grid, dim3(512), SMB,
                           stream, p);
    } else if (wbn == 16) {
      hipLaunchKernelGGL((wgrad_glds_kernel<8, 16>), grid, dim3(512),
                         sizeof(WgSmemT<16>), stream, p);
    } else if (conv_nw() == 8) {
      hipLaunchKernelGGL((wgrad_glds_kernel<8, 64>), grid, dim3(512),
                         sizeof(WgSmemT<64>), stream, p);
    } else {
      hipLaunchKernelGGL((wgrad_glds_kernel<4, 64>), grid, dim3(NTHREADS),
                         sizeof(WgSmemT<64>), stream, p);
    }
    long total = (long)p.ktiles * WG_BK * p.ntiles * wbn;
    hipLaunchKernelGGL(wgrad_reduce_kernel, dim3(cdiv(total, 256)),
                       dim3(256), 0, stream,
                       (const float*)ws.const_data_ptr(), p.dw, p.KTOT,
                       p.Cout, p.ktiles, p.ntiles, p.slices, wbn);
    return dw;
  }
  auto dw = at::zeros({p.Cout, (long)KH, (long)KW, p.Cin},
                      x.options().dtype(at::kFloat));
  p.dw = (float*)dw.mutable_data_ptr();
  hipLaunchKernelGGL(wgrad_kernel, grid, dim3(NTHREADS), 0, stream, p);
  return dw;
}

at::Tensor quant_fp8(at::Tensor x, at::Tensor scale) {
  TORCH_CHECK(x.is_cuda() && x.scalar_type() == at::kBFloat16 && x.is_contiguous());
  TORCH_CHECK(scale.scalar_type() == at::kFloat);
  auto y = at::empty_like(x, x.options().dtype(at::kByte));
  long n = x.numel();
  long blocks = (n / 8 + 255) / 256 + 1;
  hipLaunchKernelGGL(quant_fp8_kernel, dim3((unsigned)blocks), dim3(256), 0,
                     at::cuda::getCurrentCUDAStream(),
                     (const short*)x.const_data_ptr(),
                     (const float*)scale.const_data_ptr(),
                     (unsigned char*)y.mutable_data_ptr(), n);
  return y;
}

at::Tensor quant_fp8_d(at::Tensor x, at::Tensor amax_prev,
                       at::Tensor amax_cur) {
  TORCH_CHECK(x.is_cuda() && x.scalar_type() == at::kBFloat16 &&
              x.is_contiguous());
  TORCH_CHECK(amax_prev.scalar_type() == at::kFloat &&
              amax_cur.scalar_type() == at::kFloat);
  auto y = at::empty_like(x, x.options().dtype(at::kByte));
  long n = x.numel();
  long blocks = std::min<long>((n / 8 + 255) / 256 + 1, 768);
  hipLaunchKernelGGL(quant_fp8_d_kernel, dim3((unsigned)blocks), dim3(256), 0,
                     at::cuda::getCurrentCUDAStream(),
                     (const short*)x.const_data_ptr(),
                     (const float*)amax_prev.const_data_ptr(),
                     (float*)amax_cur.mutable_data_ptr(),
                     (unsigned char*)y.mutable_data_ptr(), n);
  return y;
}

void amax_roll(at::Tensor arena, int64_t n) {
  TORCH_CHECK(arena.is_cuda() && arena.scalar_type() == at::kFloat &&
              arena.dim() == 2 && arena.size(0) == 2 && arena.is_contiguous());
  int cap = (int)arena.size(1);
  TORCH_CHECK(n <= cap);
  hipLaunchKernelGGL(amax_roll_kernel, dim3(cdiv(n, 256)), dim3(256), 0,
                     at::cuda::getCurrentCUDAStream(),
                     (float*)arena.mutable_data_ptr(), (int)n, cap);
}

at::Tensor conv2d_fp8_fwd(at::Tensor xq, at::Tensor wq, at::Tensor dq,
                          c10::optional<at::Tensor> sw,
                          c10::optional<at::Tensor> bias, int64_t stride,
                          int64_t pt, int64_t pb, int64_t pl, int64_t pr,
                          bool reflect, int64_t act, double slope) {
  TORCH_CHECK(xq.is_cuda() && xq.scalar_type() == at::kByte && xq.is_contiguous());
  TORCH_CHECK(wq.scalar_type() == at::kByte && wq.is_contiguous());
  TORCH_CHECK(xq.size(3) == wq.size(3) && xq.size(3) % 16 == 0,
              "fp8 conv: Cin % 16 != 0");
  int H = xq.size(1), W = xq.size(2);
  int KH = wq.size(1), KW = wq.size(2);
  int OH = (H + pt + pb - KH) / stride + 1;
  int OW = (W + pl + pr - KW) / stride + 1;
  auto y = at::empty({xq.size(0), OH, OW, wq.size(0)},
                     xq.options().dtype(at::kBFloat16));
  ConvParams p{};
  p.x = (const short*)xq.const_data_ptr();
  p.w = (const short*)wq.const_data_ptr();
  p.bias = bias.has_value() ? (const short*)bias->const_data_ptr() : nullptr;
  p.dq = (const float*)dq.const_data_ptr();
  p.dqb = sw.has_value() ? (const float*)sw->const_data_ptr() : nullptr;
  p.y = (short*)y.mutable_data_ptr();
  p.B = xq.size(0); p.H = H; p.W = W; p.Cin = xq.size(3);
  p.OH = OH; p.OW = OW; p.Cout = wq.size(0);
  p.KH = KH; p.KW = KW;
  p.stride = stride; p.pt = pt; p.pl = pl;
  p.reflect = reflect ? 1 : 0;
  p.act = act; p.slope = (float)slope;
  p.M = (long)p.B * OH * OW;
  p.KTOT = (long)KH * KW * p.Cin;
  p.mtiles = cdiv(p.M, BM);
  p.ntiles = cdiv(p.Cout, BN);
  TORCH_CHECK((long)p.B * H * W * p.Cin < (1L << 31) &&
              (long)p.Cout * p.KTOT < (1L << 31));
  auto stream = at::cuda::getCurrentCUDAStream();
  dim3 grid(p.mtiles * p.ntiles);
  switch (p.stride) {
    case 1: hipLaunchKernelGGL((conv_fp8_kernel<1>), grid, dim3(NTHREADS), 0, stream, p); break;
    case 2: hipLaunchKernelGGL((conv_fp8_kernel<2>), grid, dim3(NTHREADS), 0, stream, p); break;
    default: hipLaunchKernelGGL((conv_fp8_kernel<0>), grid, dim3(NTHREADS), 0, stream, p);
  }
  return y;
}

__global__ void glds_probe_kernel(const float* x, const unsigned* voff,
                                  int nbytes, float* out) {
  __shared__ float lds[128];
  int l = threadIdx.x;
  lds[l] = -1.f; lds[64 + l] = -1.f;
  __syncthreads();
  auto rsrc = __builtin_amdgcn_make_buffer_rsrc((void*)x, 0, nbytes, 0x00020000);
  __builtin_amdgcn_raw_ptr_buffer_load_lds(
      rsrc, (__attribute__((address_space(3))) void*)&lds[0], 16, voff[l], 0,
      0, 0);
  __builtin_amdgcn_s_waitcnt(0);
  __syncthreads();
  out[l] = lds[l];
  out[64 + l] = lds[64 + l];
}

at::Tensor glds_probe(at::Tensor x, at::Tensor voff) {
  TORCH_CHECK(x.is_cuda() && x.scalar_type() == at::kFloat);
  TORCH_CHECK(voff.scalar_type() == at::kInt && voff.numel() == 64);
  auto out = at::empty({128}, x.options());
  hipLaunchKernelGGL(glds_probe_kernel, dim3(1), dim3(64), 0,
                     at::cuda::getCurrentCUDAStream(),
                     (const float*)x.const_data_ptr(),
                     (const unsigned*)voff.const_data_ptr(),
                     (int)(x.numel() * 4), (float*)out.mutable_data_ptr());
  return out;
}

typedef bf16r v4bf __attribute__((ext_vector_type(4)));
typedef short v4sh __attribute__((ext_vector_type(4)));
__global__ void tr_probe_kernel(short* out, int mode) {
  __shared__ short lds[1024];
  int l = threadIdx.x;
  for (int i = l; i < 1024; i += 64) lds[i] = (short)i;
  __syncthreads();
  int addr;
  switch (mode) {
    case 0: addr = (l & 15) + (l >> 4) * 64; break;
    case 1: addr = 0; break;
    case 2: addr = l * 4; break;
    default: addr = (l & 15) * 2 + (l >> 4) * 64; break;
  }
  auto p = (__attribute__((address_space(3))) v4bf*)(
      (__attribute__((address_space(3))) short*)lds + addr);
  v4bf r = __builtin_amdgcn_ds_read_tr16_b64_v4bf16(p);
  #pragma unroll
  for (int j = 0; j < 4; ++j) out[l * 4 + j] = ((v4sh&)r)[j];
}

at::Tensor tr_probe(int64_t mode) {
  auto out = at::empty({256}, at::TensorOptions().dtype(at::kShort).device(at::kCUDA));
  hipLaunchKernelGGL(tr_probe_kernel, dim3(1), dim3(64), 0,
                     at::cuda::getCurrentCUDAStream(),
                     (short*)out.mutable_data_ptr(), (int)mode);
  return out;
}

typedef int v8i_ __attribute__((ext_vector_type(8)));
typedef float v16f_ __attribute__((ext_vector_type(16)));
__global__ void mx_probe_kernel(const int* a, const int* b, float* d,
                                int sa, int sb) {
  int lane = threadIdx.x & 63;
  v8i_ av = *(const v8i_*)(a + lane * 8);
  v8i_ bv = *(const v8i_*)(b + lane * 8);
  v16f_ acc = {};
  acc = __builtin_amdgcn_mfma_scale_f32_32x32x64_f8f6f4(
      av, bv, acc, 0, 0, 0, sa, 0, sb);
  #pragma unroll
  for (int r = 0; r < 16; ++r) d[lane * 16 + r] = acc[r];
}

__global__ void mx_probe16_kernel(const int* a, const int* b, float* d,
                                  int sa, int sb) {
  int lane = threadIdx.x & 63;
  v8i_ av = *(const v8i_*)(a + lane * 8);
  v8i_ bv = *(const v8i_*)(b + lane * 8);
  v4f acc = {};
  acc = __builtin_amdgcn_mfma_scale_f32_16x16x128_f8f6f4(
      av, bv, acc, 0, 0, 0, sa, 0, sb);
  #pragma unroll
  for (int r = 0; r < 4; ++r) d[lane * 4 + r] = acc[r];
}

at::Tensor mx_probe16(at::Tensor a, at::Tensor b, int64_t sa, int64_t sb) {
  TORCH_CHECK(a.is_cuda() && a.scalar_type() == at::kInt &&
              a.sizes() == at::IntArrayRef({64, 8}) &&
              b.sizes() == at::IntArrayRef({64, 8}));
  auto d = at::empty({64, 4}, a.options().dtype(at::kFloat));
  hipLaunchKernelGGL(mx_probe16_kernel, dim3(1), dim3(64), 0,
                     at::cuda::getCurrentCUDAStream(),
                     (const int*)a.contiguous().const_data_ptr(),
                     (const int*)b.contiguous().const_data_ptr(),
                     (float*)d.mutable_data_ptr(), (int)sa, (int)sb);
  return d;
}

at::Tensor mx_probe(at::Tensor a, at::Tensor b, int64_t sa, int64_t sb) {
  TORCH_CHECK(a.is_cuda() && a.scalar_type() == at::kInt &&
              a.sizes() == at::IntArrayRef({64, 8}) &&
              b.sizes() == at::IntArrayRef({64, 8}));
  auto d = at::empty({64, 16}, a.options().dtype(at::kFloat));
  hipLaunchKernelGGL(mx_probe_kernel, dim3(1), dim3(64), 0,
                     at::cuda::getCurrentCUDAStream(),
                     (const int*)a.contiguous().const_data_ptr(),
                     (const int*)b.contiguous().const_data_ptr(),
                     (float*)d.mutable_data_ptr(), (int)sa, (int)sb);
  return d;
}

__global__ void mfma_probe_kernel(const short* a, const short* bt, float* c) {
  int lane = threadIdx.x & 63;
  int fr = lane & 15, fg = lane >> 4;
  v8bf av = *(const v8bf*)(a + fr * 32 + fg * 8);
  v8bf bv = *(const v8bf*)(bt + fr * 32 + fg * 8);
  v4f d = {};
  d = __builtin_amdgcn_mfma_f32_16x16x32_bf16(av, bv, d, 0, 0, 0);
  #pragma unroll
  for (int r = 0; r < 4; ++r) c[(fg * 4 + r) * 16 + fr] = d[r];
}

at::Tensor mfma_probe(at::Tensor a, at::Tensor bt) {
  TORCH_CHECK(a.sizes() == at::IntArrayRef({16, 32}) &&
              bt.sizes() == at::IntArrayRef({16, 32}));
  auto c = at::empty({16, 16}, a.options().dtype(at::kFloat));
  hipLaunchKernelGGL(mfma_probe_kernel, dim3(1), dim3(64), 0,
                     at::cuda::getCurrentCUDAStream(),
                     (const short*)a.contiguous().const_data_ptr(),
                     (const short*)bt.contiguous().const_data_ptr(),
                     (float*)c.mutable_data_ptr());
  return c;
}

}
```

cyclegan_amd/ops/_hip/norm_elem.hip:

```cpp

#include <torch/extension.h>
#include <ATen/cuda/CUDAContext.h>

#include "common.h"

namespace cyg {

constexpr int NT = 256;

static inline int cdiv64(long a, long b) { return (int)((a + b - 1) / b); }

__global__ __launch_bounds__(NT) void in_reduce_kernel(
    const short* __restrict__ x, float* __restrict__ psum,
    float* __restrict__ psq, int B, long HW, int C, int S) {
  int b = blockIdx.x / S;
  int sl = blockIdx.x % S;
  long rows = (HW + S - 1) / S;
  long r0 = sl * rows, r1 = min(r0 + rows, HW);
  const int gpr = C / 8;
  const int tid = threadIdx.x;
  const short* xb = x + (long)b * HW * C;

  int g = tid % gpr;
  int rstep = NT / gpr;
  int rof = tid / gpr;
  float s[8] = {}, q[8] = {};
  #pragma unroll 4
  for (long r = r0 + rof; r < r1; r += rstep) {
    v8s v = *(const v8s*)(xb + r * C + g * 8);
    #pragma unroll
    for (int j = 0; j < 8; ++j) {
      float f = b2f(v[j]);
      s[j] += f; q[j] += f * f;
    }
  }
  __shared__ float red[NT * 17];
  #pragma unroll
  for (int j = 0; j < 8; ++j) {
    red[tid * 17 + j] = s[j];
    red[tid * 17 + 8 + j] = q[j];
  }
  __syncthreads();
  long out = ((long)sl * B + b) * C;
  for (int o = tid; o < C * 2; o += NT) {
    int c = o % C;
    int issq = o / C;
    int g2 = c / 8, j = c % 8;
    float t = 0;
    for (int k = 0; k < rstep; ++k)
      t += red[(g2 + k * gpr) * 17 + issq * 8 + j];
    (issq ? psq : psum)[out + c] = t;
  }
}



__global__ __launch_bounds__(NT) void in_stats_kernel(
    const float* __restrict__ psum, const float* __restrict__ psq,
    float* __restrict__ mean, float* __restrict__ rstd, int B, long HW,
    int C, int S, float eps) {
  int b = blockIdx.x;
  const float inv_hw = 1.f / (float)HW;
  for (int c = threadIdx.x; c < C; c += NT) {
    float sv = 0, qv = 0;
    int k = 0;
    for (; k + 4 <= S; k += 4) {
      float s0 = psum[((long)(k + 0) * B + b) * C + c];
      float s1 = psum[((long)(k + 1) * B + b) * C + c];
      float s2 = psum[((long)(k + 2) * B + b) * C + c];
      float s3 = psum[((long)(k + 3) * B + b) * C + c];
      float q0 = psq[((long)(k + 0) * B + b) * C + c];
      float q1 = psq[((long)(k + 1) * B + b) * C + c];
      float q2 = psq[((long)(k + 2) * B + b) * C + c];
      float q3 = psq[((long)(k + 3) * B + b) * C + c];
      sv += (s0 + s1) + (s2 + s3);
      qv += (q0 + q1) + (q2 + q3);
    }
    for (; k < S; ++k) {
      sv += psum[((long)k * B + b) * C + c];
      qv += psq[((long)k * B + b) * C + c];
    }
    float m = sv * inv_hw;
    float var = qv * inv_hw - m * m;
    if (var < 0.f) var = 0.f;
    mean[(long)b * C + c] = m;
    rstd[(long)b * C + c] = rsqrtf(var + eps);
  }
}

__global__ __launch_bounds__(NT) void in_bwd_stats_kernel(
    const float* __restrict__ p1, const float* __restrict__ p2,
    float* __restrict__ s1m, float* __restrict__ s2m,
    float* __restrict__ dbeta, float* __restrict__ dgamma, int B, long HW,
    int C, int S) {
  int b = blockIdx.x;
  const float inv_hw = 1.f / (float)HW;
  for (int c = threadIdx.x; c < C; c += NT) {
    float t1 = 0, t2 = 0;
    int k = 0;
    for (; k + 4 <= S; k += 4) {
      float a0 = p1[((long)(k + 0) * B + b) * C + c];
      float a1 = p1[((long)(k + 1) * B + b) * C + c];
      float a2 = p1[((long)(k + 2) * B + b) * C + c];
      float a3 = p1[((long)(k + 3) * B + b) * C + c];
      float b0 = p2[((long)(k + 0) * B + b) * C + c];
      float b1 = p2[((long)(k + 1) * B + b) * C + c];
      float b2 = p2[((long)(k + 2) * B + b) * C + c];
      float b3 = p2[((long)(k + 3) * B + b) * C + c];
      t1 += (a0 + a1) + (a2 + a3);
      t2 += (b0 + b1) + (b2 + b3);
    }
    for (; k < S; ++k) {
      t1 += p1[((long)k * B + b) * C + c];
      t2 += p2[((long)k * B + b) * C + c];
    }
    s1m[(long)b * C + c] = t1 * inv_hw;
    s2m[(long)b * C + c] = t2 * inv_hw;
    atomicAdd(&dbeta[c], t1);
    atomicAdd(&dgamma[c], t2);
  }
}

constexpr int MAXC = 2048;
__global__ __launch_bounds__(NT) void in_norm_kernel(
    const short* __restrict__ x, const float* __restrict__ gamma,
    const float* __restrict__ beta, const float* __restrict__ psum,
    const float* __restrict__ psq, float* __restrict__ mean,
    float* __restrict__ rstd, const short* __restrict__ res,
    short* __restrict__ y, int B, long HW, int C, int S, int act,
    float slope, float eps) {
  int b = blockIdx.x / S;
  int sl = blockIdx.x % S;
  long rows = (HW + S - 1) / S;
  long r0 = sl * rows, r1 = min(r0 + rows, HW);
  const int gpr = C / 8;
  const int tid = threadIdx.x;
  const long base = (long)b * HW * C;
  const float inv_hw = 1.f / (float)HW;

  __shared__ float sm[MAXC], sr[MAXC];
  __shared__ float part[2 * NT];
  if (psum == nullptr) {
    for (int c = tid; c < C; c += NT) {
      sm[c] = mean[(long)b * C + c];
      sr[c] = rstd[(long)b * C + c];
    }
  } else if (C >= NT) {
    for (int c = tid; c < C; c += NT) {
      float sv = 0, qv = 0;
      int k = 0;
      for (; k + 4 <= S; k += 4) {
        float s0 = psum[((long)(k + 0) * B + b) * C + c];
        float s1 = psum[((long)(k + 1) * B + b) * C + c];
        float s2 = psum[((long)(k + 2) * B + b) * C + c];
        float s3 = psum[((long)(k + 3) * B + b) * C + c];
        float q0 = psq[((long)(k + 0) * B + b) * C + c];
        float q1 = psq[((long)(k + 1) * B + b) * C + c];
        float q2 = psq[((long)(k + 2) * B + b) * C + c];
        float q3 = psq[((long)(k + 3) * B + b) * C + c];
        sv += (s0 + s1) + (s2 + s3);
        qv += (q0 + q1) + (q2 + q3);
      }
      for (; k < S; ++k) {
        sv += psum[((long)k * B + b) * C + c];
        qv += psq[((long)k * B + b) * C + c];
      }
      float m = sv * inv_hw;
      float var = qv * inv_hw - m * m;
      if (var < 0.f) var = 0.f;
      float rs = rsqrtf(var + eps);
      sm[c] = m;
      sr[c] = rs;
      if (sl == 0) {
        mean[(long)b * C + c] = m;
        rstd[(long)b * C + c] = rs;
      }
    }
  } else {
    const int PS = NT / C;
    const int kc = tid / C;
    const int c = tid - kc * C;
    float sv = 0, qv = 0;
    int k = kc;
    for (; k + 3 * PS < S; k += 4 * PS) {
      float s0 = psum[((long)(k + 0 * PS) * B + b) * C + c];
      float s1 = psum[((long)(k + 1 * PS) * B + b) * C + c];
      float s2 = psum[((long)(k + 2 * PS) * B + b) * C + c];
      float s3 = psum[((long)(k + 3 * PS) * B + b) * C + c];
      float q0 = psq[((long)(k + 0 * PS) * B + b) * C + c];
      float q1 = psq[((long)(k + 1 * PS) * B + b) * C + c];
      float q2 = psq[((long)(k + 2 * PS) * B + b) * C + c];
      float q3 = psq[((long)(k + 3 * PS) * B + b) * C + c];
      sv += (s0 + s1) + (s2 + s3);
      qv += (q0 + q1) + (q2 + q3);
    }
    for (; k < S; k += PS) {
      sv += psum[((long)k * B + b) * C + c];
      qv += psq[((long)k * B + b) * C + c];
    }
    part[tid] = sv;
    part[NT + tid] = qv;
    __syncthreads();
    if (tid < C) {
      float svt = 0, qvt = 0;
      for (int j = 0; j < PS; ++j) {
        svt += part[j * C + tid];
        qvt += part[NT + j * C + tid];
      }
      float m = svt * inv_hw;
      float var = qvt * inv_hw - m * m;
      if (var < 0.f) var = 0.f;
      float rs = rsqrtf(var + eps);
      sm[tid] = m;
      sr[tid] = rs;
      if (sl == 0) {
        mean[(long)b * C + tid] = m;
        rstd[(long)b * C + tid] = rs;
      }
    }
  }
  __syncthreads();

  {
    int g = tid % gpr;
    int rstep = NT / gpr;
    int rof = tid / gpr;
    #pragma unroll 4
    for (long r = r0 + rof; r < r1; r += rstep) {
      long off = base + r * C + g * 8;
      v8s v = *(const v8s*)(x + off);
      v8s rv = {};
      if (res) rv = *(const v8s*)(res + off);
      v8s out;
      #pragma unroll
      for (int j = 0; j < 8; ++j) {
        int c = g * 8 + j;
        float val = (b2f(v[j]) - sm[c]) * sr[c] * gamma[c] + beta[c];
        if (res) val += b2f(rv[j]);
        out[j] = f2b(apply_act(val, act, slope));
      }
      *(v8s*)(y + off) = out;
    }
  }
}

DEV float actbw(float d, float yy, int act, float slope) {
  if (act == ACT_RELU) return yy > 0.f ? d : 0.f;
  if (act == ACT_LRELU) return yy > 0.f ? d : d * slope;
  if (act == ACT_TANH) return d * (1.f - yy * yy);
  return d;
}

__global__ __launch_bounds__(NT) void in_bwd_reduce_kernel(
    const short* __restrict__ dy, const short* __restrict__ x,
    const short* __restrict__ yact, const float* __restrict__ mean,
    const float* __restrict__ rstd,
    float* __restrict__ p1, float* __restrict__ p2, int B, long HW, int C,
    int S, int act, float slope, float* __restrict__ dgb) {
  int b = blockIdx.x / S;
  int sl = blockIdx.x % S;
  if (blockIdx.x == 0)
    for (int i = threadIdx.x; i < 2 * C; i += NT) dgb[i] = 0.f;
  long rows = (HW + S - 1) / S;
  long r0 = sl * rows, r1 = min(r0 + rows, HW);
  const int gpr = C / 8;
  const int tid = threadIdx.x;
  const long base = (long)b * HW * C;

  int g = tid % gpr;
  int rstep = NT / gpr;
  int rof = tid / gpr;
  float a1[8] = {}, a2[8] = {};
  float mv[8], rv[8];
  #pragma unroll
  for (int j = 0; j < 8; ++j) {
    mv[j] = mean[(long)b * C + g * 8 + j];
    rv[j] = rstd[(long)b * C + g * 8 + j];
  }
  #pragma unroll 4
  for (long r = r0 + rof; r < r1; r += rstep) {
    long off = base + r * C + g * 8;
    v8s dv = *(const v8s*)(dy + off);
    v8s xv = *(const v8s*)(x + off);
    v8s yv = {};
    if (act != ACT_NONE) yv = *(const v8s*)(yact + off);
    #pragma unroll
    for (int j = 0; j < 8; ++j) {
      float d = b2f(dv[j]);
      if (act != ACT_NONE) d = actbw(d, b2f(yv[j]), act, slope);
      float xh = (b2f(xv[j]) - mv[j]) * rv[j];
      a1[j] += d; a2[j] += d * xh;
    }
  }
  __shared__ float red[NT * 17];
  #pragma unroll
  for (int j = 0; j < 8; ++j) {
    red[tid * 17 + j] = a1[j];
    red[tid * 17 + 8 + j] = a2[j];
  }
  __syncthreads();
  long out = ((long)sl * B + b) * C;
  for (int o = tid; o < C * 2; o += NT) {
    int c = o % C;
    int is2 = o / C;
    int g2 = c / 8, j = c % 8;
    float t = 0;
    for (int k = 0; k < rstep; ++k)
      t += red[(g2 + k * gpr) * 17 + is2 * 8 + j];
    (is2 ? p2 : p1)[out + c] = t;
  }
}



__global__ __launch_bounds__(NT) void in_bwd_dx_kernel(
    const short* __restrict__ dy, const short* __restrict__ x,
    const short* __restrict__ yact, const float* __restrict__ gamma,
    const float* __restrict__ mean,
    const float* __restrict__ rstd, const float* __restrict__ p1,
    const float* __restrict__ p2, short* __restrict__ dx,
    float* __restrict__ dbeta, float* __restrict__ dgamma, int B, long HW,
    int C, int S, int act, float slope) {
  const bool sready = S < 0;
  if (sready) S = -S;
  int b = blockIdx.x / S;
  int sl = blockIdx.x % S;
  long rows = (HW + S - 1) / S;
  long r0 = sl * rows, r1 = min(r0 + rows, HW);
  const int gpr = C / 8;
  const int tid = threadIdx.x;
  const long base = (long)b * HW * C;
  const float inv_hw = 1.f / (float)HW;

  __shared__ float sm1[MAXC], sm2[MAXC], smean[MAXC], srstd[MAXC];
  __shared__ float part[2 * NT];
  if (sready) {
    for (int c = tid; c < C; c += NT) {
      sm1[c] = p1[(long)b * C + c];
      sm2[c] = p2[(long)b * C + c];
      smean[c] = mean[(long)b * C + c];
      srstd[c] = rstd[(long)b * C + c];
    }
  } else if (C >= NT) {
    for (int c = tid; c < C; c += NT) {
      float t1 = 0, t2 = 0;
      int k = 0;
      for (; k + 4 <= S; k += 4) {
        float a0 = p1[((long)(k + 0) * B + b) * C + c];
        float a1 = p1[((long)(k + 1) * B + b) * C + c];
        float a2 = p1[((long)(k + 2) * B + b) * C + c];
        float a3 = p1[((long)(k + 3) * B + b) * C + c];
        float b0 = p2[((long)(k + 0) * B + b) * C + c];
        float b1 = p2[((long)(k + 1) * B + b) * C + c];
        float b2 = p2[((long)(k + 2) * B + b) * C + c];
        float b3 = p2[((long)(k + 3) * B + b) * C + c];
        t1 += (a0 + a1) + (a2 + a3);
        t2 += (b0 + b1) + (b2 + b3);
      }
      for (; k < S; ++k) {
        t1 += p1[((long)k * B + b) * C + c];
        t2 += p2[((long)k * B + b) * C + c];
      }
      sm1[c] = t1 * inv_hw;
      sm2[c] = t2 * inv_hw;
      smean[c] = mean[(long)b * C + c];
      srstd[c] = rstd[(long)b * C + c];
      if (sl == 0) {
        atomicAdd(&dbeta[c], t1);
        atomicAdd(&dgamma[c], t2);
      }
    }
  } else {
    const int PS = NT / C;
    const int kc = tid / C;
    const int c = tid - kc * C;
    float t1 = 0, t2 = 0;
    int k = kc;
    for (; k + 3 * PS < S; k += 4 * PS) {
      float a0 = p1[((long)(k + 0 * PS) * B + b) * C + c];
      float a1 = p1[((long)(k + 1 * PS) * B + b) * C + c];
      float a2 = p1[((long)(k + 2 * PS) * B + b) * C + c];
      float a3 = p1[((long)(k + 3 * PS) * B + b) * C + c];
      float b0 = p2[((long)(k + 0 * PS) * B + b) * C + c];
      float b1 = p2[((long)(k + 1 * PS) * B + b) * C + c];
      float b2 = p2[((long)(k + 2 * PS) * B + b) * C + c];
      float b3 = p2[((long)(k + 3 * PS) * B + b) * C + c];
      t1 += (a0 + a1) + (a2 + a3);
      t2 += (b0 + b1) + (b2 + b3);
    }
    for (; k < S; k += PS) {
      t1 += p1[((long)k * B + b) * C + c];
      t2 += p2[((long)k * B + b) * C + c];
    }
    part[tid] = t1;
    part[NT + tid] = t2;
    __syncthreads();
    if (tid < C) {
      float s1 = 0, s2 = 0;
      for (int j = 0; j < PS; ++j) {
        s1 += part[j * C + tid];
        s2 += part[NT + j * C + tid];
      }
      sm1[tid] = s1 * inv_hw;
      sm2[tid] = s2 * inv_hw;
      smean[tid] = mean[(long)b * C + tid];
      srstd[tid] = rstd[(long)b * C + tid];
      if (sl == 0) {
        atomicAdd(&dbeta[tid], s1);
        atomicAdd(&dgamma[tid], s2);
      }
    }
  }
  __syncthreads();

  {
    int g = tid % gpr;
    int rstep = NT / gpr;
    int rof = tid / gpr;
    #pragma unroll 4
    for (long r = r0 + rof; r < r1; r += rstep) {
      long off = base + r * C + g * 8;
      v8s dv = *(const v8s*)(dy + off);
      v8s xv = *(const v8s*)(x + off);
      v8s yv = {};
      if (act != ACT_NONE) yv = *(const v8s*)(yact + off);
      v8s out;
      #pragma unroll
      for (int j = 0; j < 8; ++j) {
        int c = g * 8 + j;
        float rs = srstd[c];
        float xh = (b2f(xv[j]) - smean[c]) * rs;
        float d = b2f(dv[j]);
        if (act != ACT_NONE) d = actbw(d, b2f(yv[j]), act, slope);
        out[j] = f2b(gamma[c] * rs * (d - sm1[c] - xh * sm2[c]));
      }
      *(v8s*)(dx + off) = out;
    }
  }
}


#define RLX_AGENT __ATOMIC_RELAXED, __HIP_MEMORY_SCOPE_AGENT
typedef __attribute__((address_space(1))) unsigned long long gu64;
typedef __attribute__((address_space(1))) unsigned int gu32;

__global__ __launch_bounds__(NT) void in_bwd_fused_kernel(
    const short* __restrict__ dy, const short* __restrict__ x,
    const short* __restrict__ yact, const float* __restrict__ gamma,
    const float* __restrict__ mean, const float* __restrict__ rstd,
    unsigned long long* __restrict__ gq,
    unsigned int* __restrict__ arrive,
    short* __restrict__ dx, float* __restrict__ dbeta,
    float* __restrict__ dgamma, int B, long HW, int C, int S, int act,
    float slope) {
  int b = blockIdx.x / S;
  int sl = blockIdx.x % S;
  long rows = (HW + S - 1) / S;
  long r0 = sl * rows, r1 = min(r0 + rows, HW);
  const int gpr = C / 8;
  const int tid = threadIdx.x;
  const long base = (long)b * HW * C;
  const float inv_hw = 1.f / (float)HW;

  int g = tid % gpr;
  int rstep = NT / gpr;
  int rof = tid / gpr;
  float a1[8] = {}, a2[8] = {};
  float mv[8], rv[8];
  #pragma unroll
  for (int j = 0; j < 8; ++j) {
    mv[j] = mean[(long)b * C + g * 8 + j];
    rv[j] = rstd[(long)b * C + g * 8 + j];
  }
  #pragma unroll 4
  for (long r = r0 + rof; r < r1; r += rstep) {
    long off = base + r * C + g * 8;
    v8s dv = *(const v8s*)(dy + off);
    v8s xv = *(const v8s*)(x + off);
    v8s yv = {};
    if (act != ACT_NONE) yv = *(const v8s*)(yact + off);
    #pragma unroll
    for (int j = 0; j < 8; ++j) {
      float d = b2f(dv[j]);
      if (act != ACT_NONE) d = actbw(d, b2f(yv[j]), act, slope);
      float xh = (b2f(xv[j]) - mv[j]) * rv[j];
      a1[j] += d; a2[j] += d * xh;
    }
  }
  __shared__ float red[NT * 17];
  #pragma unroll
  for (int j = 0; j < 8; ++j) {
    red[tid * 17 + j] = a1[j];
    red[tid * 17 + 8 + j] = a2[j];
  }
  __syncthreads();
  long gout = ((long)sl * B + b) * C;
  for (int c = tid; c < C; c += NT) {
    int g2 = c / 8, j = c % 8;
    float t1 = 0, t2 = 0;
    for (int k = 0; k < rstep; ++k) {
      t1 += red[(g2 + k * gpr) * 17 + j];
      t2 += red[(g2 + k * gpr) * 17 + 8 + j];
    }
    unsigned long long pack =
        ((unsigned long long)__float_as_uint(t2) << 32) | __float_as_uint(t1);
    __hip_atomic_store((gu64*)&gq[gout + c], pack, RLX_AGENT);
  }
  asm volatile("s_waitcnt vmcnt(0)" ::: "memory");
  __syncthreads();
  if (tid == 0)
    __hip_atomic_fetch_add((gu32*)&arrive[b], 1u, RLX_AGENT);

  __shared__ float sm1[MAXC], sm2[MAXC], smean[MAXC], srstd[MAXC];
  __shared__ int failed;
  if (tid == 0) {
    failed = 0;
    unsigned spins = 0;
    while (__hip_atomic_load((gu32*)&arrive[b], RLX_AGENT) < (unsigned)S) {
      __builtin_amdgcn_s_sleep(8);
      if (++spins > (1u << 24)) { failed = 1; break; }
    }
    __builtin_amdgcn_fence(__ATOMIC_ACQUIRE, "agent");
  }
  __syncthreads();
  if (failed) {
    for (long r = r0 + rof; r < r1; r += rstep) {
      long off = base + r * C + g * 8;
      v8s out;
      #pragma unroll
      for (int j = 0; j < 8; ++j) out[j] = f2b(__int_as_float(0x7FC00000));
      *(v8s*)(dx + off) = out;
    }
    return;
  }
  bool sl0 = (sl == 0);
  for (int c = tid; c < C; c += NT) {
    float t1 = 0, t2 = 0;
    int k = 0;
    for (; k + 4 <= S; k += 4) {
      unsigned long long v0 = gq[((long)(k + 0) * B + b) * C + c];
      unsigned long long v1 = gq[((long)(k + 1) * B + b) * C + c];
      unsigned long long v2 = gq[((long)(k + 2) * B + b) * C + c];
      unsigned long long v3 = gq[((long)(k + 3) * B + b) * C + c];
      t1 += (__uint_as_float((unsigned)v0) + __uint_as_float((unsigned)v1)) +
            (__uint_as_float((unsigned)v2) + __uint_as_float((unsigned)v3));
      t2 += (__uint_as_float((unsigned)(v0 >> 32)) +
             __uint_as_float((unsigned)(v1 >> 32))) +
            (__uint_as_float((unsigned)(v2 >> 32)) +
             __uint_as_float((unsigned)(v3 >> 32)));
    }
    for (; k < S; ++k) {
      unsigned long long v = gq[((long)k * B + b) * C + c];
      t1 += __uint_as_float((unsigned)v);
      t2 += __uint_as_float((unsigned)(v >> 32));
    }
    sm1[c] = t1 * inv_hw;
    sm2[c] = t2 * inv_hw;
    smean[c] = mean[(long)b * C + c];
    srstd[c] = rstd[(long)b * C + c];
    if (sl0) {
      atomicAdd(&dbeta[c], t1);
      atomicAdd(&dgamma[c], t2);
    }
  }
  __syncthreads();

  #pragma unroll 4
  for (long r = r0 + rof; r < r1; r += rstep) {
    long off = base + r * C + g * 8;
    v8s dv = *(const v8s*)(dy + off);
    v8s xv = *(const v8s*)(x + off);
    v8s yv = {};
    if (act != ACT_NONE) yv = *(const v8s*)(yact + off);
    v8s out;
    #pragma unroll
    for (int j = 0; j < 8; ++j) {
      int c = g * 8 + j;
      float rs = srstd[c];
      float xh = (b2f(xv[j]) - smean[c]) * rs;
      float d = b2f(dv[j]);
      if (act != ACT_NONE) d = actbw(d, b2f(yv[j]), act, slope);
      out[j] = f2b(gamma[c] * rs * (d - sm1[c] - xh * sm2[c]));
    }
    *(v8s*)(dx + off) = out;
  }
}

__global__ __launch_bounds__(NT) void in_fwd_fused_kernel(
    const short* __restrict__ x, const float* __restrict__ gamma,
    const float* __restrict__ beta,
    unsigned long long* __restrict__ gq,
    unsigned int* __restrict__ arrive,
    float* __restrict__ mean, float* __restrict__ rstd,
    const short* __restrict__ res, short* __restrict__ y, int B, long HW,
    int C, int S, int act, float slope, float eps) {
  int b = blockIdx.x / S;
  int sl = blockIdx.x % S;
  long rows = (HW + S - 1) / S;
  long r0 = sl * rows, r1 = min(r0 + rows, HW);
  const int gpr = C / 8;
  const int tid = threadIdx.x;
  const long base = (long)b * HW * C;
  const float inv_hw = 1.f / (float)HW;

  int g = tid % gpr;
  int rstep = NT / gpr;
  int rof = tid / gpr;
  float s[8] = {}, q[8] = {};
  #pragma unroll 4
  for (long r = r0 + rof; r < r1; r += rstep) {
    v8s v = *(const v8s*)(x + base + r * C + g * 8);
    #pragma unroll
    for (int j = 0; j < 8; ++j) {
      float f = b2f(v[j]);
      s[j] += f; q[j] += f * f;
    }
  }
  __shared__ float red[NT * 17];
  #pragma unroll
  for (int j = 0; j < 8; ++j) {
    red[tid * 17 + j] = s[j];
    red[tid * 17 + 8 + j] = q[j];
  }
  __syncthreads();
  long gout = ((long)sl * B + b) * C;
  for (int c = tid; c < C; c += NT) {
    int g2 = c / 8, j = c % 8;
    float ts = 0, tq = 0;
    for (int k = 0; k < rstep; ++k) {
      ts += red[(g2 + k * gpr) * 17 + j];
      tq += red[(g2 + k * gpr) * 17 + 8 + j];
    }
    unsigned long long pack =
        ((unsigned long long)__float_as_uint(tq) << 32) | __float_as_uint(ts);
    __hip_atomic_store((gu64*)&gq[gout + c], pack, RLX_AGENT);
  }
  asm volatile("s_waitcnt vmcnt(0)" ::: "memory");
  __syncthreads();
  if (tid == 0)
    __hip_atomic_fetch_add((gu32*)&arrive[b], 1u, RLX_AGENT);

  __shared__ float sm[MAXC], sr[MAXC];
  __shared__ int failed;
  if (tid == 0) {
    failed = 0;
    unsigned spins = 0;
    while (__hip_atomic_load((gu32*)&arrive[b], RLX_AGENT) < (unsigned)S) {
      __builtin_amdgcn_s_sleep(8);
      if (++spins > (1u << 24)) { failed = 1; break; }
    }
    __builtin_amdgcn_fence(__ATOMIC_ACQUIRE, "agent");
  }
  __syncthreads();
  if (failed) {
    for (long r = r0 + rof; r < r1; r += rstep) {
      long off = base + r * C + g * 8;
      v8s out;
      #pragma unroll
      for (int j = 0; j < 8; ++j) out[j] = f2b(__int_as_float(0x7FC00000));
      *(v8s*)(y + off) = out;
    }
    return;
  }
  for (int c = tid; c < C; c += NT) {
    float sv = 0, qv = 0;
    int k = 0;
    for (; k + 4 <= S; k += 4) {
      unsigned long long v0 = gq[((long)(k + 0) * B + b) * C + c];
      unsigned long long v1 = gq[((long)(k + 1) * B + b) * C + c];
      unsigned long long v2 = gq[((long)(k + 2) * B + b) * C + c];
      unsigned long long v3 = gq[((long)(k + 3) * B + b) * C + c];
      sv += (__uint_as_float((unsigned)v0) + __uint_as_float((unsigned)v1)) +
            (__uint_as_float((unsigned)v2) + __uint_as_float((unsigned)v3));
      qv += (__uint_as_float((unsigned)(v0 >> 32)) +
             __uint_as_float((unsigned)(v1 >> 32))) +
            (__uint_as_float((unsigned)(v2 >> 32)) +
             __uint_as_float((unsigned)(v3 >> 32)));
    }
    for (; k < S; ++k) {
      unsigned long long v = gq[((long)k * B + b) * C + c];
      sv += __uint_as_float((unsigned)v);
      qv += __uint_as_float((unsigned)(v >> 32));
    }
    float m = sv * inv_hw;
    float var = qv * inv_hw - m * m;
    if (var < 0.f) var = 0.f;
    float rs = rsqrtf(var + eps);
    sm[c] = m;
    sr[c] = rs;
    if (sl == 0) {
      mean[(long)b * C + c] = m;
      rstd[(long)b * C + c] = rs;
    }
  }
  __syncthreads();

  #pragma unroll 4
  for (long r = r0 + rof; r < r1; r += rstep) {
    long off = base + r * C + g * 8;
    v8s v = *(const v8s*)(x + off);
    v8s rv = {};
    if (res) rv = *(const v8s*)(res + off);
    v8s out;
    #pragma unroll
    for (int j = 0; j < 8; ++j) {
      int c = g * 8 + j;
      float val = (b2f(v[j]) - sm[c]) * sr[c] * gamma[c] + beta[c];
      if (res) val += b2f(rv[j]);
      out[j] = f2b(apply_act(val, act, slope));
    }
    *(v8s*)(y + off) = out;
  }
}

__global__ __launch_bounds__(NT) void channel_sum_kernel(
    const short* __restrict__ x, float* __restrict__ out, long rows, int C,
    int S) {
  int sl = blockIdx.x;
  long per = (rows + S - 1) / S;
  long r0 = sl * per, r1 = min(r0 + per, rows);
  const int gpr = C / 8;
  const int tid = threadIdx.x;
  int g = tid % gpr;
  int rstep = NT / gpr;
  int rof = tid / gpr;
  float a[8] = {};
  for (long r = r0 + rof; r < r1; r += rstep) {
    v8s v = *(const v8s*)(x + r * C + g * 8);
    #pragma unroll
    for (int j = 0; j < 8; ++j) a[j] += b2f(v[j]);
  }
  __shared__ float red[NT * 17];
  #pragma unroll
  for (int j = 0; j < 8; ++j) red[tid * 17 + j] = a[j];
  __syncthreads();
  for (int c = tid; c < C; c += NT) {
    int g2 = c / 8, j = c % 8;
    float t = 0;
    for (int k = 0; k < rstep; ++k) t += red[(g2 + k * gpr) * 17 + j];
    atomicAdd(&out[c], t);
  }
}

__global__ void act_bwd_kernel(const short* __restrict__ dy,
                               const short* __restrict__ y,
                               short* __restrict__ out, long n, int act,
                               float slope) {
  long i = ((long)blockIdx.x * blockDim.x + threadIdx.x) * 8;
  if (i >= n) return;
  if (i + 8 <= n) {
    v8s dv = *(const v8s*)(dy + i);
    v8s yv = *(const v8s*)(y + i);
    v8s o;
    #pragma unroll
    for (int j = 0; j < 8; ++j) {
      float d = b2f(dv[j]), yy = b2f(yv[j]);
      float r;
      if (act == ACT_RELU) r = yy > 0.f ? d : 0.f;
      else if (act == ACT_LRELU) r = yy > 0.f ? d : d * slope;
      else r = d * (1.f - yy * yy);
      o[j] = f2b(r);
    }
    *(v8s*)(out + i) = o;
  } else {
    for (long k = i; k < n; ++k) {
      float d = b2f(dy[k]), yy = b2f(y[k]);
      float r;
      if (act == ACT_RELU) r = yy > 0.f ? d : 0.f;
      else if (act == ACT_LRELU) r = yy > 0.f ? d : d * slope;
      else r = d * (1.f - yy * yy);
      out[k] = f2b(r);
    }
  }
}

__global__ void reflect_pad_fwd_kernel(const short* __restrict__ x,
                                       short* __restrict__ y, int B, int H,
                                       int W, int C, int pt, int pb, int pl,
                                       int pr) {
  int HP = H + pt + pb, WP = W + pl + pr;
  long total = (long)B * HP * WP * C;
  long i = (long)blockIdx.x * blockDim.x + threadIdx.x;
  if (i >= total) return;
  int c = (int)(i % C);
  long t = i / C;
  int qw = (int)(t % WP);
  t /= WP;
  int qh = (int)(t % HP);
  int b = (int)(t / HP);
  int ih = mirror_idx(qh - pt, H);
  int iw = mirror_idx(qw - pl, W);
  y[i] = x[(((long)b * H + ih) * W + iw) * C + c];
}

__global__ void reflect_pad_bwd_kernel(const short* __restrict__ dyp,
                                       short* __restrict__ dx, int B, int H,
                                       int W, int C, int pt, int pb, int pl,
                                       int pr) {
  long total = (long)B * H * W * C;
  long idx = (long)blockIdx.x * blockDim.x + threadIdx.x;
  if (idx >= total) return;
  int c = (int)(idx % C);
  long t = idx / C;
  int j = (int)(t % W);
  t /= W;
  int i = (int)(t % H);
  int b = (int)(t / H);
  int HP = H + pt + pb, WP = W + pl + pr;
  float s = 0.f;
  int hc[3] = {pt + i, pt - i, pt + 2 * (H - 1) - i};
  int wc_[3] = {pl + j, pl - j, pl + 2 * (W - 1) - j};
  #pragma unroll
  for (int a = 0; a < 3; ++a) {
    int qh = hc[a];
    if (qh < 0 || qh >= HP) continue;
    if (a > 0 && qh == hc[0]) continue;
    if (a == 2 && qh == hc[1]) continue;
    #pragma unroll
    for (int d = 0; d < 3; ++d) {
      int qw = wc_[d];
      if (qw < 0 || qw >= WP) continue;
      if (d > 0 && qw == wc_[0]) continue;
      if (d == 2 && qw == wc_[1]) continue;
      s += b2f(dyp[(((long)b * HP + qh) * WP + qw) * C + c]);
    }
  }
  dx[idx] = f2b(s);
}

__global__ __launch_bounds__(NT) void persample_loss_kernel(
    const short* __restrict__ yt, const short* __restrict__ yp,
    float* __restrict__ out, long D, int squared, float cconst,
    int use_const) {
  int b = blockIdx.y;
  long base = (long)b * D;
  long per = (D + gridDim.x - 1) / gridDim.x;
  long i0 = blockIdx.x * per, i1 = min(i0 + per, D);
  float acc = 0.f;
  for (long i = i0 + threadIdx.x * 8; i < i1; i += (long)NT * 8) {
    if (i + 8 <= i1) {
      v8s pv = *(const v8s*)(yp + base + i);
      #pragma unroll
      for (int j = 0; j < 8; ++j) {
        float t = use_const ? cconst : b2f(yt[base + i + j]);
        float d = b2f(pv[j]) - t;
        acc += squared ? d * d : fabsf(d);
      }
    } else {
      for (long k = i; k < i1; ++k) {
        float t = use_const ? cconst : b2f(yt[base + k]);
        float d = b2f(yp[k + base]) - t;
        acc += squared ? d * d : fabsf(d);
      }
    }
  }
  #pragma unroll
  for (int off = 32; off; off >>= 1) acc += __shfl_down(acc, off, 64);
  __shared__ float red[NT / 64];
  if ((threadIdx.x & 63) == 0) red[threadIdx.x >> 6] = acc;
  __syncthreads();
  if (threadIdx.x == 0) {
    float s = 0;
    #pragma unroll
    for (int k = 0; k < NT / 64; ++k) s += red[k];
    atomicAdd(&out[b], s / (float)D);
  }
}

__global__ void persample_loss_bwd_kernel(
    const short* __restrict__ yt, const short* __restrict__ yp,
    const float* __restrict__ dout, short* __restrict__ gt,
    short* __restrict__ gp, long D, int squared, float cconst,
    int use_const) {
  long n = (long)gridDim.y * D;
  long i = (long)blockIdx.x * blockDim.x + threadIdx.x;
  int b = blockIdx.y;
  long base = (long)b * D;
  if (i >= D) return;
  float t = use_const ? cconst : b2f(yt[base + i]);
  float p = b2f(yp[base + i]);
  float d = p - t;
  float g = dout[b] / (float)D;
  float gpv = squared ? 2.f * d * g : (d > 0.f ? g : (d < 0.f ? -g : 0.f));
  if (gp) gp[base + i] = f2b(gpv);
  if (gt) gt[base + i] = f2b(-gpv);
  (void)n;
}

__global__ void adam_kernel(float* __restrict__ p, const float* __restrict__ g,
                            float* __restrict__ m, float* __restrict__ v,
                            long n, float lr_t, float b1, float b2,
                            float eps) {
  long i = (long)blockIdx.x * blockDim.x + threadIdx.x;
  long stride = (long)gridDim.x * blockDim.x;
  for (; i < n; i += stride) {
    float gi = g[i];
    float mi = b1 * m[i] + (1.f - b1) * gi;
    float vi = b2 * v[i] + (1.f - b2) * gi * gi;
    m[i] = mi;
    v[i] = vi;
    p[i] -= lr_t * mi / (sqrtf(vi) + eps);
  }
}

__global__ void adam_kernel_dev(float* __restrict__ p,
                                const float* __restrict__ g,
                                float* __restrict__ m, float* __restrict__ v,
                                long n, const float* __restrict__ lr_t_ptr,
                                float b1, float b2, float eps) {
  const float lr_t = *lr_t_ptr;
  long i = (long)blockIdx.x * blockDim.x + threadIdx.x;
  long stride = (long)gridDim.x * blockDim.x;
  for (; i < n; i += stride) {
    float gi = g[i];
    float mi = b1 * m[i] + (1.f - b1) * gi;
    float vi = b2 * v[i] + (1.f - b2) * gi * gi;
    m[i] = mi;
    v[i] = vi;
    p[i] -= lr_t * mi / (sqrtf(vi) + eps);
  }
}


static int slices_for(long HW, int B) {
  int s = (int)std::min<long>(std::max<long>(1, 512 / std::max(B, 1)),
                              std::max<long>(1, HW / 64));
  return std::max(1, s);
}

std::vector<at::Tensor> instnorm_fwd(at::Tensor x, at::Tensor gamma,
                                     at::Tensor beta, double eps, int64_t act,
                                     double slope,
                                     c10::optional<at::Tensor> residual) {
  TORCH_CHECK(x.is_cuda() && x.scalar_type() == at::kBFloat16 && x.is_contiguous());
  int B = x.size(0), C = x.size(3);
  long HW = (long)x.size(1) * x.size(2);
  TORCH_CHECK(C % 8 == 0 && (C / 8) <= 256 && 256 % std::min(C / 8, 256) == 0,
              "instnorm: unsupported channel count ", C);
  auto stream = at::cuda::getCurrentCUDAStream();
  auto fopt = x.options().dtype(at::kFloat);
  int S = slices_for(HW, B);
  auto mean = at::empty({B, C}, fopt);
  auto rstd = at::empty({B, C}, fopt);
  auto y = at::empty_like(x);
  const short* resf = residual.has_value()
                          ? (const short*)residual->const_data_ptr() : nullptr;

  static int fused_cap = []() {
    if (const char* e = getenv("CYG_IN_FUSED"); !(e && e[0] == '1')) return 0;
    int bpc = 0, ncu = 0, dev = 0;
    if (hipGetDevice(&dev) != hipSuccess) return 0;
    if (hipOccupancyMaxActiveBlocksPerMultiprocessor(
            &bpc, (const void*)in_fwd_fused_kernel, NT, 0) != hipSuccess)
      return 0;
    if (hipDeviceGetAttribute(&ncu, hipDeviceAttributeMultiprocessorCount,
                              dev) != hipSuccess)
      return 0;
    return bpc * ncu;
  }();
  if (fused_cap > 0 && B < fused_cap) {
    int Sf = std::max(1, std::min(S, fused_cap / B));
    auto gq = at::empty({(long)Sf * B * C}, x.options().dtype(at::kLong));
    auto arr = at::empty({B}, x.options().dtype(at::kInt));
    CHECK_HIP(hipMemsetAsync(arr.mutable_data_ptr(), 0, (size_t)B * 4,
                             stream));
    hipLaunchKernelGGL(in_fwd_fused_kernel, dim3(B * Sf), dim3(NT), 0,
                       stream, (const short*)x.const_data_ptr(),
                       (const float*)gamma.const_data_ptr(),
                       (const float*)beta.const_data_ptr(),
                       (unsigned long long*)gq.mutable_data_ptr(),
                       (unsigned int*)arr.mutable_data_ptr(),
                       (float*)mean.mutable_data_ptr(),
                       (float*)rstd.mutable_data_ptr(), resf,
                       (short*)y.mutable_data_ptr(), B, HW, C, Sf,
                       (int)act, (float)slope, (float)eps);
    return {y, mean, rstd};
  }

  auto psum = at::empty({S, B, C}, fopt);
  auto psq = at::empty({S, B, C}, fopt);
  hipLaunchKernelGGL(in_reduce_kernel, dim3(B * S), dim3(NT), 0, stream,
                     (const short*)x.const_data_ptr(),
                     (float*)psum.mutable_data_ptr(),
                     (float*)psq.mutable_data_ptr(), B, HW, C, S);
  const short* res = residual.has_value()
                         ? (const short*)residual->const_data_ptr() : nullptr;
  static bool use_stats = []() {
    const char* e = getenv("CYG_IN_STATS");
    return e && e[0] == '1';
  }();
  if (use_stats) {
    hipLaunchKernelGGL(in_stats_kernel, dim3(B), dim3(NT), 0, stream,
                       (const float*)psum.const_data_ptr(),
                       (const float*)psq.const_data_ptr(),
                       (float*)mean.mutable_data_ptr(),
                       (float*)rstd.mutable_data_ptr(), B, HW, C, S,
                       (float)eps);
    hipLaunchKernelGGL(in_norm_kernel, dim3(B * S), dim3(NT), 0, stream,
                       (const short*)x.const_data_ptr(),
                       (const float*)gamma.const_data_ptr(),
                       (const float*)beta.const_data_ptr(), nullptr, nullptr,
                       (float*)mean.mutable_data_ptr(),
                       (float*)rstd.mutable_data_ptr(), res,
                       (short*)y.mutable_data_ptr(), B, HW, C, S, (int)act,
                       (float)slope, (float)eps);
    return {y, mean, rstd};
  }
  hipLaunchKernelGGL(in_norm_kernel, dim3(B * S), dim3(NT), 0, stream,
                     (const short*)x.const_data_ptr(),
                     (const float*)gamma.const_data_ptr(),
                     (const float*)beta.const_data_ptr(),
                     (const float*)psum.const_data_ptr(),
                     (const float*)psq.const_data_ptr(),
                     (float*)mean.mutable_data_ptr(),
                     (float*)rstd.mutable_data_ptr(), res,
                     (short*)y.mutable_data_ptr(), B, HW, C, S, (int)act,
                     (float)slope, (float)eps);
  return {y, mean, rstd};
}

std::vector<at::Tensor> instnorm_bwd(at::Tensor dy, at::Tensor x,
                                     at::Tensor gamma, at::Tensor mean,
                                     at::Tensor rstd,
                                     c10::optional<at::Tensor> yact,
                                     int64_t act, double slope) {
  TORCH_CHECK(dy.is_cuda() && dy.scalar_type() == at::kBFloat16 &&
              dy.is_contiguous() && x.is_contiguous());
  int B = x.size(0), C = x.size(3);
  long HW = (long)x.size(1) * x.size(2);
  TORCH_CHECK(C % 8 == 0 && (C / 8) <= 256 && 256 % std::min(C / 8, 256) == 0,
              "instnorm_bwd: unsupported channel count ", C);
  auto stream = at::cuda::getCurrentCUDAStream();
  auto fopt = x.options().dtype(at::kFloat);
  int S = slices_for(HW, B);
  auto dx = at::empty_like(x);
  auto dgb = at::empty({2, C}, fopt);
  auto dbeta = dgb[0];
  auto dgamma = dgb[1];
  const short* yp = yact.has_value()
                        ? (const short*)yact->const_data_ptr() : nullptr;

  static int fused_cap = []() {
    if (const char* e = getenv("CYG_IN_FUSED"); !(e && e[0] == '1')) return 0;
    int bpc = 0, ncu = 0, dev = 0;
    if (hipGetDevice(&dev) != hipSuccess) return 0;
    if (hipOccupancyMaxActiveBlocksPerMultiprocessor(
            &bpc, (const void*)in_bwd_fused_kernel, NT, 0) != hipSuccess)
      return 0;
    if (hipDeviceGetAttribute(&ncu, hipDeviceAttributeMultiprocessorCount,
                              dev) != hipSuccess)
      return 0;
    return bpc * ncu;
  }();
  if (fused_cap > 0 && B < fused_cap) {
    int Sf = std::max(1, std::min(S, fused_cap / B));
    auto gq = at::empty({(long)Sf * B * C},
                        x.options().dtype(at::kLong));
    auto arr = at::empty({B}, x.options().dtype(at::kInt));
    CHECK_HIP(hipMemsetAsync(arr.mutable_data_ptr(), 0, (size_t)B * 4,
                             stream));
    CHECK_HIP(hipMemsetAsync(dgb.mutable_data_ptr(), 0,
                             (size_t)2 * C * 4, stream));
    hipLaunchKernelGGL(in_bwd_fused_kernel, dim3(B * Sf), dim3(NT), 0,
                       stream, (const short*)dy.const_data_ptr(),
                       (const short*)x.const_data_ptr(), yp,
                       (const float*)gamma.const_data_ptr(),
                       (const float*)mean.const_data_ptr(),
                       (const float*)rstd.const_data_ptr(),
                       (unsigned long long*)gq.mutable_data_ptr(),
                       (unsigned int*)arr.mutable_data_ptr(),
                       (short*)dx.mutable_data_ptr(),
                       (float*)dbeta.mutable_data_ptr(),
                       (float*)dgamma.mutable_data_ptr(), B, HW, C, Sf,
                       (int)act, (float)slope);
    return {dx, dgamma, dbeta};
  }

  auto p1 = at::empty({S, B, C}, fopt);
  auto p2 = at::empty({S, B, C}, fopt);
  hipLaunchKernelGGL(in_bwd_reduce_kernel, dim3(B * S), dim3(NT), 0, stream,
                     (const short*)dy.const_data_ptr(),
                     (const short*)x.const_data_ptr(), yp,
                     (const float*)mean.const_data_ptr(),
                     (const float*)rstd.const_data_ptr(),
                     (float*)p1.mutable_data_ptr(),
                     (float*)p2.mutable_data_ptr(), B, HW, C, S, (int)act,
                     (float)slope, (float*)dgb.mutable_data_ptr());
  static bool use_stats = []() {
    const char* e = getenv("CYG_IN_STATS");
    return e && e[0] == '1';
  }();
  if (use_stats) {
    auto s1m = at::empty({B, C}, fopt);
    auto s2m = at::empty({B, C}, fopt);
    hipLaunchKernelGGL(in_bwd_stats_kernel, dim3(B), dim3(NT), 0, stream,
                       (const float*)p1.const_data_ptr(),
                       (const float*)p2.const_data_ptr(),
                       (float*)s1m.mutable_data_ptr(),
                       (float*)s2m.mutable_data_ptr(),
                       (float*)dbeta.mutable_data_ptr(),
                       (float*)dgamma.mutable_data_ptr(), B, HW, C, S);
    hipLaunchKernelGGL(in_bwd_dx_kernel, dim3(B * S), dim3(NT), 0, stream,
                       (const short*)dy.const_data_ptr(),
                       (const short*)x.const_data_ptr(), yp,
                       (const float*)gamma.const_data_ptr(),
                       (const float*)mean.const_data_ptr(),
                       (const float*)rstd.const_data_ptr(),
                       (const float*)s1m.const_data_ptr(),
                       (const float*)s2m.const_data_ptr(),
                       (short*)dx.mutable_data_ptr(),
                       (float*)dbeta.mutable_data_ptr(),
                       (float*)dgamma.mutable_data_ptr(), B, HW, C, -S,
                       (int)act, (float)slope);
    return {dx, dgamma, dbeta};
  }
  hipLaunchKernelGGL(in_bwd_dx_kernel, dim3(B * S), dim3(NT), 0, stream,
                     (const short*)dy.const_data_ptr(),
                     (const short*)x.const_data_ptr(), yp,
                     (const float*)gamma.const_data_ptr(),
                     (const float*)mean.const_data_ptr(),
                     (const float*)rstd.const_data_ptr(),
                     (const float*)p1.const_data_ptr(),
                     (const float*)p2.const_data_ptr(),
                     (short*)dx.mutable_data_ptr(),
                     (float*)dbeta.mutable_data_ptr(),
                     (float*)dgamma.mutable_data_ptr(), B, HW, C, S,
                     (int)act, (float)slope);
  return {dx, dgamma, dbeta};
}

at::Tensor channel_sum(at::Tensor x) {
  TORCH_CHECK(x.is_cuda() && x.scalar_type() == at::kBFloat16 && x.is_contiguous());
  int C = x.size(-1);
  long rows = x.numel() / C;
  TORCH_CHECK(C % 8 == 0 && (C / 8) <= NT && NT % (C / 8) == 0,
              "channel_sum: unsupported C ", C);
  auto out = at::empty({C}, x.options().dtype(at::kFloat));
  CHECK_HIP(hipMemsetAsync(out.mutable_data_ptr(), 0, C * sizeof(float),
                           at::cuda::getCurrentCUDAStream()));
  int S = (int)std::min<long>(512, std::max<long>(1, rows / 64));
  hipLaunchKernelGGL(channel_sum_kernel, dim3(S), dim3(NT), 0,
                     at::cuda::getCurrentCUDAStream(),
                     (const short*)x.const_data_ptr(),
                     (float*)out.mutable_data_ptr(), rows, C, S);
  return out;
}

at::Tensor act_bwd(at::Tensor dy, at::Tensor y, int64_t act, double slope) {
  TORCH_CHECK(dy.is_cuda() && dy.scalar_type() == at::kBFloat16);
  auto out = at::empty_like(dy);
  long n = dy.numel();
  long blocks = (n / 8 + 255) / 256 + 1;
  hipLaunchKernelGGL(act_bwd_kernel, dim3((unsigned)blocks), dim3(256), 0,
                     at::cuda::getCurrentCUDAStream(),
                     (const short*)dy.const_data_ptr(),
                     (const short*)y.const_data_ptr(),
                     (short*)out.mutable_data_ptr(), n, (int)act,
                     (float)slope);
  return out;
}

at::Tensor reflect_pad_fwd(at::Tensor x, int64_t pt, int64_t pb, int64_t pl,
                           int64_t pr) {
  TORCH_CHECK(x.is_cuda() && x.scalar_type() == at::kBFloat16 && x.is_contiguous());
  int B = x.size(0), H = x.size(1), W = x.size(2), C = x.size(3);
  auto y = at::empty({B, H + pt + pb, W + pl + pr, C}, x.options());
  long total = y.numel();
  hipLaunchKernelGGL(reflect_pad_fwd_kernel, dim3(cdiv64(total, 256)),
                     dim3(256), 0, at::cuda::getCurrentCUDAStream(),
                     (const short*)x.const_data_ptr(),
                     (short*)y.mutable_data_ptr(), B, H, W, C, (int)pt,
                     (int)pb, (int)pl, (int)pr);
  return y;
}

at::Tensor reflect_pad_bwd(at::Tensor dyp, int64_t pt, int64_t pb, int64_t pl,
                           int64_t pr) {
  TORCH_CHECK(dyp.is_cuda() && dyp.scalar_type() == at::kBFloat16 && dyp.is_contiguous());
  int B = dyp.size(0);
  int H = dyp.size(1) - pt - pb, W = dyp.size(2) - pl - pr, C = dyp.size(3);
  auto dx = at::empty({B, H, W, C}, dyp.options());
  long total = dx.numel();
  hipLaunchKernelGGL(reflect_pad_bwd_kernel, dim3(cdiv64(total, 256)),
                     dim3(256), 0, at::cuda::getCurrentCUDAStream(),
                     (const short*)dyp.const_data_ptr(),
                     (short*)dx.mutable_data_ptr(), B, H, W, C, (int)pt,
                     (int)pb, (int)pl, (int)pr);
  return dx;
}

static at::Tensor persample_fwd_impl(c10::optional<at::Tensor> yt,
                                     at::Tensor yp, bool squared,
                                     double cconst) {
  TORCH_CHECK(yp.is_cuda() && yp.scalar_type() == at::kBFloat16 && yp.is_contiguous());
  int B = yp.size(0);
  long D = yp.numel() / B;
  auto out = at::empty({B}, yp.options().dtype(at::kFloat));
  CHECK_HIP(hipMemsetAsync(out.mutable_data_ptr(), 0, B * sizeof(float),
                           at::cuda::getCurrentCUDAStream()));
  int gx = (int)std::min<long>(32, std::max<long>(1, D / (256 * 8)));
  dim3 grid(gx, B);
  hipLaunchKernelGGL(persample_loss_kernel, grid, dim3(NT), 0,
                     at::cuda::getCurrentCUDAStream(),
                     yt.has_value() ? (const short*)yt->const_data_ptr() : nullptr,
                     (const short*)yp.const_data_ptr(),
                     (float*)out.mutable_data_ptr(), D, squared ? 1 : 0,
                     (float)cconst, yt.has_value() ? 0 : 1);
  return out;
}

at::Tensor persample_loss_fwd(at::Tensor yt, at::Tensor yp, bool squared) {
  return persample_fwd_impl(yt.contiguous(), yp, squared, 0.0);
}

at::Tensor persample_loss_const_fwd(at::Tensor yp, double cconst, bool squared) {
  return persample_fwd_impl(c10::nullopt, yp, squared, cconst);
}

std::vector<at::Tensor> persample_loss_bwd(at::Tensor yt, at::Tensor yp,
                                           at::Tensor dout, bool squared,
                                           bool need_gt, bool need_gp) {
  int B = yp.size(0);
  long D = yp.numel() / B;
  auto gt = need_gt ? at::empty_like(yt) : at::Tensor();
  auto gp = need_gp ? at::empty_like(yp) : at::Tensor();
  dim3 grid(cdiv64(D, 256), B);
  hipLaunchKernelGGL(persample_loss_bwd_kernel, grid, dim3(256), 0,
                     at::cuda::getCurrentCUDAStream(),
                     (const short*)yt.const_data_ptr(),
                     (const short*)yp.const_data_ptr(),
                     (const float*)dout.const_data_ptr(),
                     need_gt ? (short*)gt.mutable_data_ptr() : nullptr,
                     need_gp ? (short*)gp.mutable_data_ptr() : nullptr, D,
                     squared ? 1 : 0, 0.f, 0);
  return {gt, gp};
}

at::Tensor persample_loss_const_bwd(at::Tensor yp, double cconst,
                                    at::Tensor dout, bool squared) {
  int B = yp.size(0);
  long D = yp.numel() / B;
  auto gp = at::empty_like(yp);
  dim3 grid(cdiv64(D, 256), B);
  hipLaunchKernelGGL(persample_loss_bwd_kernel, grid, dim3(256), 0,
                     at::cuda::getCurrentCUDAStream(), nullptr,
                     (const short*)yp.const_data_ptr(),
                     (const float*)dout.const_data_ptr(), nullptr,
                     (short*)gp.mutable_data_ptr(), D, squared ? 1 : 0,
                     (float)cconst, 1);
  return gp;
}

void adam_step(at::Tensor p, at::Tensor g, at::Tensor m, at::Tensor v,
               double lr, double b1, double b2, double eps, int64_t t) {
  TORCH_CHECK(p.is_cuda() && p.scalar_type() == at::kFloat);
  long n = p.numel();
  double lr_t = lr * std::sqrt(1.0 - std::pow(b2, (double)t)) /
                (1.0 - std::pow(b1, (double)t));
  int blocks = (int)std::min<long>(2048, (n + 255) / 256);
  hipLaunchKernelGGL(adam_kernel, dim3(blocks), dim3(256), 0,
                     at::cuda::getCurrentCUDAStream(),
                     (float*)p.mutable_data_ptr(),
                     (const float*)g.const_data_ptr(),
                     (float*)m.mutable_data_ptr(),
                     (float*)v.mutable_data_ptr(), n, (float)lr_t, (float)b1,
                     (float)b2, (float)eps);
}

void adam_step_dev(at::Tensor p, at::Tensor g, at::Tensor m, at::Tensor v,
                   at::Tensor lr_t, double b1, double b2, double eps) {
  TORCH_CHECK(p.is_cuda() && p.scalar_type() == at::kFloat);
  TORCH_CHECK(lr_t.is_cuda() && lr_t.scalar_type() == at::kFloat);
  long n = p.numel();
  int blocks = (int)std::min<long>(2048, (n + 255) / 256);
  hipLaunchKernelGGL(adam_kernel_dev, dim3(blocks), dim3(256), 0,
                     at::cuda::getCurrentCUDAStream(),
                     (float*)p.mutable_data_ptr(),
                     (const float*)g.const_data_ptr(),
                     (float*)m.mutable_data_ptr(),
                     (float*)v.mutable_data_ptr(), n,
                     (const float*)lr_t.const_data_ptr(), (float)b1,
                     (float)b2, (float)eps);
}

}
```

cyclegan_amd/ops/conv.py:

```python

from __future__ import annotations

from typing import Optional, Tuple

import torch
import torch.nn.functional as F

from . import backend
from .shadow import (compute_weight, compute_weight_t, compute_weight_p,
                     compute_weight_tp, compute_bias_p, compute_weight_packp,
                     compute_bias_packb, fp8_weight_shadow)

ACT_NONE, ACT_RELU, ACT_LRELU, ACT_TANH = 0, 1, 2, 3

_ACT = {None: ACT_NONE, "none": ACT_NONE, "relu": ACT_RELU, "lrelu": ACT_LRELU, "tanh": ACT_TANH}


def same_pads(in_h: int, in_w: int, kh: int, kw: int, stride: int) -> Tuple[int, int, int, int]:
    out_h = -(-in_h // stride)
    out_w = -(-in_w // stride)
    ph = max(0, (out_h - 1) * stride + kh - in_h)
    pw = max(0, (out_w - 1) * stride + kw - in_w)
    return ph // 2, ph - ph // 2, pw // 2, pw - pw // 2


def _apply_act(y: torch.Tensor, act: int, slope: float) -> torch.Tensor:
    if act == ACT_RELU:
        return torch.relu(y)
    if act == ACT_LRELU:
        return F.leaky_relu(y, slope)
    if act == ACT_TANH:
        return torch.tanh(y)
    return y


def act_bwd_from_output(dy: torch.Tensor, y: torch.Tensor, act: int, slope: float) -> torch.Tensor:
    if act == ACT_RELU:
        return dy * (y > 0).to(dy.dtype)
    if act == ACT_LRELU:
        return torch.where(y > 0, dy, dy * slope)
    if act == ACT_TANH:
        return dy * (1 - y.float() * y.float()).to(dy.dtype)
    return dy


def _conv_ref(x, w, bias, stride, pads, pad_mode):
    pt, pb, pl, pr = pads
    xn = x.permute(0, 3, 1, 2)
    if pt or pb or pl or pr:
        mode = "reflect" if pad_mode == "reflect" else "constant"
        xn = F.pad(xn, (pl, pr, pt, pb), mode=mode)
    wn = w.permute(0, 3, 1, 2)
    y = F.conv2d(xn.contiguous(), wn.contiguous(), bias, stride=stride)
    return y.permute(0, 2, 3, 1)


def _convt_ref(x, w, bias, stride, pt, pl, out_h, out_w):
    xn = x.permute(0, 3, 1, 2)
    wn = w.permute(3, 0, 1, 2)
    y = F.conv_transpose2d(xn.contiguous(), wn.contiguous(), bias, stride=stride)
    y = y[:, :, pt : pt + out_h, pl : pl + out_w]
    return y.permute(0, 2, 3, 1)


def _pad_channels(t: torch.Tensor, c_to: int = 8) -> torch.Tensor:
    c = t.shape[-1]
    if c >= c_to:
        return t
    return F.pad(t, (0, c_to - c))


class _ConvFn(torch.autograd.Function):

    @staticmethod
    def forward(ctx, x, w, bias, stride, pads, reflect, act, slope):
        ext = backend.ext()
        cout = w.shape[0]
        xp = _pad_channels(x).contiguous()
        wc = compute_weight_p(w, x)
        bc = compute_bias_p(bias, x) if bias is not None else None
        y = ext.conv2d_fwd(xp, wc, bc, stride, *pads, reflect, act, slope)
        if cout < 8:
            y = y[..., :cout].contiguous()
        ctx.save_for_backward(xp, w, y)
        ctx.conf = (stride, pads, reflect, act, slope, bias is not None,
                    x.shape[3])
        return y

    @staticmethod
    def backward(ctx, dy):
        xp, w, y = ctx.saved_tensors
        stride, pads, reflect, act, slope, has_bias, cin = ctx.conf
        cout = w.shape[0]
        pt, pb, pl, pr = pads
        ext = backend.ext()
        dy = dy.contiguous()
        if act != ACT_NONE:
            dy = ext.act_bwd(dy, y, act, slope)
        dyp = _pad_channels(dy).contiguous()
        db = None
        if has_bias and ctx.needs_input_grad[2]:
            db = ext.channel_sum(dyp)[: dy.shape[-1]]
        dx = dw = None
        if ctx.needs_input_grad[0]:
            wt = compute_weight_tp(w, xp)
            dx = ext.conv2d_dgrad(dyp, wt, xp.shape[1], xp.shape[2], stride,
                                  pt, pb, pl, pr, reflect)
            if cin < 8:
                dx = dx[..., :cin].contiguous()
        if ctx.needs_input_grad[1]:
            dw = ext.conv2d_wgrad(xp, dyp, w.shape[1], w.shape[2], stride,
                                  pt, pl, reflect)
            if cout < 8 or cin < 8:
                dw = dw[:cout, :, :, :cin].contiguous()
            if dw.dtype != w.dtype:
                dw = dw.to(w.dtype)
        return dx, dw, db, None, None, None, None, None


def _head_packable(x, w, stride, pads, reflect) -> bool:
    import os
    if os.environ.get("CYG_NO_PACKHEAD") == "1":
        return False
    return (reflect and stride == 1 and pads == (3, 3, 3, 3)
            and w.shape[0] <= 8 and w.shape[1] == 7 and w.shape[2] == 7
            and w.shape[3] % 8 == 0 and w.shape[3] >= 8
            and x.shape[2] % 8 == 0 and x.shape[1] >= 7 and x.shape[2] >= 16)


def _fold_packed_dw(dwp: torch.Tensor, wshape) -> torch.Tensor:
    O, KH, KW, I = wshape
    d6 = dwp.view(8, 8, KH, 2, 8, I)
    d7 = d6.permute(0, 3, 4, 1, 2, 5).reshape(8, 16, 8, KH, I)
    dev = dwp.device
    idx = (torch.arange(KW, device=dev).view(1, -1)
           + torch.arange(8, device=dev).view(-1, 1))
    idx = idx.view(8, KW, 1, 1, 1).expand(8, KW, 8, KH, I)
    dw = d7.gather(1, idx).sum(0)
    return dw.permute(1, 2, 0, 3)[:O].contiguous()


class _ConvHeadPackedFn(torch.autograd.Function):

    @staticmethod
    def forward(ctx, x, w, bias, act, slope):
        ext = backend.ext()
        B, H, W, Cin = x.shape
        cout = w.shape[0]
        wpk = compute_weight_packp(w, x)
        bpk = compute_bias_packb(bias, x) if bias is not None else None
        xp = ext.reflect_pad_fwd(x.contiguous(), 3, 3, 3, 5)
        xf = xp.view(B, H + 6, (W + 8) // 8, 8 * Cin)
        yp = ext.conv2d_fwd(xf, wpk, bpk, 1, 0, 0, 0, 0, False, act, slope)
        y = yp.view(B, H, W, 8)
        if cout < 8:
            y = y[..., :cout].contiguous()
        ctx.save_for_backward(xp, w, y)
        ctx.conf = (act, slope, bias is not None, cout, Cin, H, W)
        return y

    @staticmethod
    def backward(ctx, dy):
        xp, w, y = ctx.saved_tensors
        act, slope, has_bias, cout, Cin, H, W = ctx.conf
        ext = backend.ext()
        dy = dy.contiguous()
        if act != ACT_NONE:
            dy = ext.act_bwd(dy, y, act, slope)
        dyp = _pad_channels(dy).contiguous()
        db = None
        if has_bias and ctx.needs_input_grad[2]:
            db = ext.channel_sum(dyp)[: dy.shape[-1]]
        dx = dw = None
        B = dyp.shape[0]
        if ctx.needs_input_grad[0]:
            wt = compute_weight_tp(w, xp)
            dx = ext.conv2d_dgrad(dyp, wt, H, W, 1, 3, 3, 3, 3, True)
        if ctx.needs_input_grad[1]:
            xf = xp.view(B, H + 6, (W + 8) // 8, 8 * Cin)
            dy_pk = dyp.view(B, H, W // 8, 64)
            dwp = ext.conv2d_wgrad(xf, dy_pk, 7, 2, 1, 0, 0, False)
            dw = _fold_packed_dw(dwp, tuple(w.shape))
            if dw.dtype != w.dtype:
                dw = dw.to(w.dtype)
        return dx, dw, db, None, None


_FP8_MODE = False


def set_fp8_mode(on: bool):
    global _FP8_MODE
    _FP8_MODE = bool(on)


def fp8_mode() -> bool:
    return _FP8_MODE


class _ConvFp8Fn(torch.autograd.Function):

    @staticmethod
    def forward(ctx, x, w, bias, stride, pads, reflect, act, slope):
        from . import fp8_state
        ext = backend.ext()
        cout = w.shape[0]
        xp = _pad_channels(x).contiguous()
        wq, sw = fp8_weight_shadow(w)
        prev, cur, fresh = fp8_state.slots_for(w)
        if fresh:
            prev.copy_(xp.detach().abs().amax().float().clamp(min=1e-12))
        xq = ext.quant_fp8_d(xp, prev, cur)
        bc = compute_bias_p(bias, x) if bias is not None else None
        y = ext.conv2d_fp8_fwd(xq, wq, prev, sw, bc, stride, *pads,
                               reflect, act, slope)
        if cout < 8:
            y = y[..., :cout].contiguous()
        ctx.save_for_backward(xp, w, y)
        ctx.conf = (stride, pads, reflect, act, slope, bias is not None,
                    x.shape[3])
        return y

    backward = _ConvFn.backward


class _ConvTFn(torch.autograd.Function):
    @staticmethod
    def forward(ctx, x, w, bias, stride, pt, pl, out_h, out_w, act, slope):
        ext = backend.ext()
        wc = compute_weight(w, x)
        bc = compute_weight(bias, x) if bias is not None else None
        y = ext.convt2d_fwd(x, wc, bc, stride, pt, pl, out_h, out_w, act, slope)
        ctx.save_for_backward(x, w, y)
        ctx.conf = (stride, pt, pl, act, slope, bias is not None)
        return y

    @staticmethod
    def backward(ctx, dy):
        x, w, y = ctx.saved_tensors
        stride, pt, pl, act, slope, has_bias = ctx.conf
        ext = backend.ext()
        dy = dy.contiguous()
        if act != ACT_NONE:
            dy = ext.act_bwd(dy, y, act, slope)
        dx = dw = db = None
        if ctx.needs_input_grad[0]:
            wt = compute_weight_t(w, x)
            dx = ext.convt2d_dgrad(dy, wt, x.shape[1], x.shape[2], stride, pt, pl)
        if ctx.needs_input_grad[1]:
            dwc = ext.conv2d_wgrad(dy, x, w.shape[1], w.shape[2], stride,
                                   pt, pl, False)
            dw = dwc.permute(3, 1, 2, 0).contiguous()
            if dw.dtype != w.dtype:
                dw = dw.to(w.dtype)
        if has_bias and ctx.needs_input_grad[2]:
            db = dy.float().sum(dim=(0, 1, 2))
        return dx, dw, db, None, None, None, None, None, None, None


def conv2d(
    x: torch.Tensor,
    w: torch.Tensor,
    bias: Optional[torch.Tensor] = None,
    stride: int = 1,
    padding: str | Tuple[int, int, int, int] = "valid",
    pad_mode: str = "zeros",
    act: Optional[str] = None,
    slope: float = 0.2,
) -> torch.Tensor:
    kh, kw = w.shape[1], w.shape[2]
    if padding == "valid":
        pads = (0, 0, 0, 0)
    elif padding == "same":
        pads = same_pads(x.shape[1], x.shape[2], kh, kw, stride)
    else:
        pads = tuple(padding)
    a = _ACT[act]
    if backend.use_hip(x, w):
        if _head_packable(x, w, stride, pads, pad_mode == "reflect"):
            return _ConvHeadPackedFn.apply(x, w, bias, a, slope)
        if (_FP8_MODE and x.dtype == torch.bfloat16
                and w.shape[3] % 16 == 0 and w.shape[3] >= 256
                and stride == 1
                and ((w.shape[1] == 3 and x.shape[0] >= 12)
                     or w.shape[1] == 4)):
            return _ConvFp8Fn.apply(x, w, bias, stride, pads,
                                    pad_mode == "reflect", a, slope)
        return _ConvFn.apply(x, w, bias, stride, pads, pad_mode == "reflect", a, slope)
    wc = w if w.dtype == x.dtype else w.to(x.dtype)
    bc = bias if (bias is None or bias.dtype == x.dtype) else bias.to(x.dtype)
    y = _conv_ref(x, wc, bc, stride, pads, pad_mode)
    return _apply_act(y, a, slope)


def conv_transpose2d(
    x: torch.Tensor,
    w: torch.Tensor,
    bias: Optional[torch.Tensor] = None,
    stride: int = 2,
    act: Optional[str] = None,
    slope: float = 0.2,
) -> torch.Tensor:
    kh, kw = w.shape[1], w.shape[2]
    out_h, out_w = x.shape[1] * stride, x.shape[2] * stride
    pt, _, pl, _ = same_pads(out_h, out_w, kh, kw, stride)
    a = _ACT[act]
    if backend.use_hip(x, w):
        return _ConvTFn.apply(x, w, bias, stride, pt, pl, out_h, out_w, a, slope)
    wc = w if w.dtype == x.dtype else w.to(x.dtype)
    bc = bias if (bias is None or bias.dtype == x.dtype) else bias.to(x.dtype)
    y = _convt_ref(x, wc, bc, stride, pt, pl, out_h, out_w)
    return _apply_act(y, a, slope)
```

cyclegan_amd/ops/norm.py:

```python

from __future__ import annotations

from typing import Optional

import torch

from . import backend
from .conv import ACT_NONE, ACT_RELU, ACT_LRELU, _ACT

EPS_DEFAULT = 1e-3


def _in_ref(x, gamma, beta, eps, act, slope, residual):
    cdt = torch.float32 if x.dtype == torch.bfloat16 else x.dtype
    xf = x.to(cdt)
    mean = xf.mean(dim=(1, 2), keepdim=True)
    var = xf.var(dim=(1, 2), unbiased=False, keepdim=True)
    y = (xf - mean) * torch.rsqrt(var + eps)
    y = y * gamma.to(cdt) + beta.to(cdt)
    y = y.to(x.dtype)
    if residual is not None:
        y = y + residual
    if act == ACT_RELU:
        y = torch.relu(y)
    elif act == ACT_LRELU:
        y = torch.nn.functional.leaky_relu(y, slope)
    return y


class _InstNormFn(torch.autograd.Function):
    @staticmethod
    def forward(ctx, x, gamma, beta, eps, act, slope, residual):
        ext = backend.ext()
        y, mean, rstd = ext.instnorm_fwd(x, gamma.float(), beta.float(), eps, act, slope,
                                         residual)
        ctx.save_for_backward(x, gamma, mean, rstd, y)
        ctx.conf = (eps, act, slope, residual is not None)
        return y

    @staticmethod
    def backward(ctx, dy):
        x, gamma, mean, rstd, y = ctx.saved_tensors
        eps, act, slope, has_res = ctx.conf
        ext = backend.ext()
        dy = dy.contiguous()
        if has_res and act != ACT_NONE:
            dy = ext.act_bwd(dy, y, act, slope)
            dres = dy
            dx, dgamma, dbeta = ext.instnorm_bwd(dy, x, gamma.float(), mean,
                                                 rstd, None, ACT_NONE, 0.0)
        else:
            dres = dy if has_res else None
            dx, dgamma, dbeta = ext.instnorm_bwd(
                dy, x, gamma.float(), mean, rstd,
                y if act != ACT_NONE else None, act, slope)
        return (dx, dgamma.to(gamma.dtype), dbeta, None, None, None, dres)


def instance_norm(
    x: torch.Tensor,
    gamma: torch.Tensor,
    beta: torch.Tensor,
    eps: float = EPS_DEFAULT,
    act: Optional[str] = None,
    slope: float = 0.2,
    residual: Optional[torch.Tensor] = None,
) -> torch.Tensor:
    a = _ACT[act]
    if backend.use_hip(x, gamma):
        return _InstNormFn.apply(x, gamma, beta, eps, a, slope, residual)
    return _in_ref(x, gamma, beta, eps, a, slope, residual)
```

Baseline: 326.1 images/s.

## Fuse instance-norm statistics into conv epilogue and pass partial sums to norm

Conv and transposed-conv forward kernels now accumulate per-channel sum and sum-of-squares of the rounded bf16 outputs in the epilogue and write per-tile partial slabs. The slabs are attached to the output tensor and handed to instance_norm, so the norm kernel can skip its separate statistics pass over the activation. Also adds an optional backward mode that recomputes the activation mask from x instead of reading y, and a vectorised reflect-pad kernel. Costs extra epilogue reductions, shared-memory traffic and small slab allocations, and relies on a Python tensor attribute to carry the stats.

```diff
diff --git a/cyclegan_amd/ops/_hip/bind.cpp b/cyclegan_amd/ops/_hip/bind.cpp
--- a/cyclegan_amd/ops/_hip/bind.cpp
+++ b/cyclegan_amd/ops/_hip/bind.cpp
@@ -7,6 +7,14 @@
 at::Tensor convt2d_fwd(at::Tensor, at::Tensor, c10::optional<at::Tensor>,
                        int64_t, int64_t, int64_t, int64_t, int64_t, int64_t,
                        double);
+std::vector<at::Tensor> conv2d_fwd_stats(at::Tensor, at::Tensor,
+                                         c10::optional<at::Tensor>, int64_t,
+                                         int64_t, int64_t, int64_t, int64_t,
+                                         bool, int64_t, double);
+std::vector<at::Tensor> convt2d_fwd_stats(at::Tensor, at::Tensor,
+                                          c10::optional<at::Tensor>, int64_t,
+                                          int64_t, int64_t, int64_t, int64_t,
+                                          int64_t, double);
 at::Tensor conv2d_dgrad(at::Tensor, at::Tensor, int64_t, int64_t, int64_t,
                         int64_t, int64_t, int64_t, int64_t, bool);
 at::Tensor convt2d_dgrad(at::Tensor, at::Tensor, int64_t, int64_t, int64_t,
@@ -26,11 +34,13 @@
                           int64_t, int64_t, int64_t, int64_t, int64_t, bool, int64_t, double);
 std::vector<at::Tensor> instnorm_fwd(at::Tensor, at::Tensor, at::Tensor,
                                      double, int64_t, double,
-                                     c10::optional<at::Tensor>);
+                                     c10::optional<at::Tensor>,
+                                     c10::optional<at::Tensor>,
+                                     c10::optional<at::Tensor>, int64_t);
 std::vector<at::Tensor> instnorm_bwd(at::Tensor, at::Tensor, at::Tensor,
                                      at::Tensor, at::Tensor,
                                      c10::optional<at::Tensor>, int64_t,
-                                     double);
+                                     double, c10::optional<at::Tensor>);
 at::Tensor act_bwd(at::Tensor, at::Tensor, int64_t, double);
 at::Tensor channel_sum(at::Tensor);
 at::Tensor reflect_pad_fwd(at::Tensor, int64_t, int64_t, int64_t, int64_t);
@@ -50,6 +60,8 @@
 PYBIND11_MODULE(TORCH_EXTENSION_NAME, m) {
   m.def("conv2d_fwd", &cyg::conv2d_fwd);
   m.def("convt2d_fwd", &cyg::convt2d_fwd);
+  m.def("conv2d_fwd_stats", &cyg::conv2d_fwd_stats);
+  m.def("convt2d_fwd_stats", &cyg::convt2d_fwd_stats);
   m.def("conv2d_dgrad", &cyg::conv2d_dgrad);
   m.def("convt2d_dgrad", &cyg::convt2d_dgrad);
   m.def("conv2d_wgrad", &cyg::conv2d_wgrad);
@@ -62,8 +74,13 @@
   m.def("quant_fp8_d", &cyg::quant_fp8_d);
   m.def("amax_roll", &cyg::amax_roll);
   m.def("conv2d_fp8_fwd", &cyg::conv2d_fp8_fwd);
-  m.def("instnorm_fwd", &cyg::instnorm_fwd);
-  m.def("instnorm_bwd", &cyg::instnorm_bwd);
+  m.def("instnorm_fwd", &cyg::instnorm_fwd, py::arg("x"), py::arg("gamma"),
+        py::arg("beta"), py::arg("eps"), py::arg("act"), py::arg("slope"),
+        py::arg("residual"), py::arg("psum") = py::none(),
+        py::arg("psq") = py::none(), py::arg("nslabs") = 0);
+  m.def("instnorm_bwd", &cyg::instnorm_bwd, py::arg("dy"), py::arg("x"),
+        py::arg("gamma"), py::arg("mean"), py::arg("rstd"), py::arg("yact"),
+        py::arg("act"), py::arg("slope"), py::arg("beta") = py::none());
   m.def("act_bwd", &cyg::act_bwd);
   m.def("channel_sum", &cyg::channel_sum);
   m.def("reflect_pad_fwd", &cyg::reflect_pad_fwd);
diff --git a/cyclegan_amd/ops/_hip/conv.hip b/cyclegan_amd/ops/_hip/conv.hip
--- a/cyclegan_amd/ops/_hip/conv.hip
+++ b/cyclegan_amd/ops/_hip/conv.hip
@@ -23,6 +23,9 @@
   const float* dqb;
   long M, KTOT;
   int mtiles, ntiles;
+  float* psum;
+  float* psq;
+  int tps;
 };
 
 DEV int xcd_chunk(int bid, int nb) {
@@ -476,6 +479,7 @@
     __syncthreads();
   }
 
+  float cs[NF] = {}, cq[NF] = {};
   #pragma unroll
   for (int nf = 0; nf < NF; ++nf) {
     int n = n0 + wn0 + nf * 16 + fr;
@@ -495,8 +499,45 @@
         }
 #endif
         float v = apply_act(acc[mf][nf][r] + bv, p.act, p.slope);
-        p.y[sm.rowyb[rl] + n] = f2b(v);
-      }
+        short hv = f2b(v);
+        p.y[sm.rowyb[rl] + n] = hv;
+        float fv = b2f(hv);
+        cs[nf] += fv;
+        cq[nf] += fv * fv;
+      }
+    }
+  }
+
+  if (p.psum != nullptr) {
+    float* red = reinterpret_cast<float*>(sm.A[0]);
+    static_assert(NWR * BNT * 2 * sizeof(float) <= sizeof(sm.A[0]), "red");
+    #pragma unroll
+    for (int nf = 0; nf < NF; ++nf) {
+      float s = cs[nf], q = cq[nf];
+      s += __shfl_xor(s, 16, 64);
+      q += __shfl_xor(q, 16, 64);
+      s += __shfl_xor(s, 32, 64);
+      q += __shfl_xor(q, 32, 64);
+      if (fg == 0) {
+        int col = wn0 + nf * 16 + fr;
+        red[(wr * BNT + col) * 2] = s;
+        red[(wr * BNT + col) * 2 + 1] = q;
+      }
+    }
+    __syncthreads();
+    if (tid < BNT && n0 + tid < p.Cout) {
+      float s = 0.f, q = 0.f;
+      #pragma unroll
+      for (int k = 0; k < NWR; ++k) {
+        s += red[(k * BNT + tid) * 2];
+        q += red[(k * BNT + tid) * 2 + 1];
+      }
+      const int mtl = PHASED ? mt - phase * tpp : mt;
+      const int b = mtl / p.tps;
+      const int slice = phase * p.tps + (mtl - b * p.tps);
+      const long o = ((long)slice * p.B + b) * p.Cout + n0 + tid;
+      p.psum[o] = s;
+      p.psq[o] = q;
     }
   }
 }
@@ -1669,14 +1710,44 @@
   }
 }
 
+static bool glds_eligible(const ConvParams& p) {
+  return (p.Cin % 8) == 0 &&
+         (long)p.B * p.H * p.W * p.Cin * 2 < (1L << 31) &&
+         (long)p.Cout * p.KTOT * 2 < (1L << 31);
+}
+
+static bool phased_eligible(const ConvParams& p, bool is_convt) {
+  return glds_eligible(p) && is_convt && p.stride == 2 && (p.OH % 2) == 0 &&
+         (p.OW % 2) == 0;
+}
+
+static int stats_slabs(const ConvParams& p, bool is_convt, int* tps) {
+  static const int cap = []() {
+    const char* off = getenv("CYG_NO_CONV_STATS");
+    if (off && off[0] == '1') return 0;
+    const char* e = getenv("CYG_CONV_STATS_MAXSLABS");
+    return e ? atoi(e) : 128;
+  }();
+  if (cap <= 0 || !glds_eligible(p) || p.Cout <= 16 || (p.Cout % 8) != 0)
+    return 0;
+  long per, ns;
+  if (phased_eligible(p, is_convt)) {
+    per = (long)(p.OH / 2) * (p.OW / 2);
+    ns = 4 * (per / BM);
+  } else {
+    per = (long)p.OH * p.OW;
+    ns = per / BM;
+  }
+  if (per % BM != 0 || ns > cap) return 0;
+  *tps = (int)(per / BM);
+  return (int)ns;
+}
+
 static void launch_conv(const ConvParams& p, bool is_convt, hipStream_t stream) {
   dim3 grid(p.mtiles * p.ntiles);
   bool aligned = (p.Cin % 8) == 0;
-  bool glds_ok = aligned &&
-                 (long)p.B * p.H * p.W * p.Cin * 2 < (1L << 31) &&
-                 (long)p.Cout * p.KTOT * 2 < (1L << 31);
-  if (glds_ok && is_convt && p.stride == 2 && (p.OH % 2) == 0 &&
-      (p.OW % 2) == 0) {
+  bool glds_ok = glds_eligible(p);
+  if (phased_eligible(p, is_convt)) {
     ConvParams q = p;
     long Mp = (long)q.B * (q.OH / 2) * (q.OW / 2);
     q.mtiles = 4 * cdiv(Mp, BM);
@@ -1735,9 +1806,28 @@
   TORCH_CHECK(w.size(3) == x.size(3), "conv: Cin mismatch");
 }
 
-at::Tensor conv2d_fwd(at::Tensor x, at::Tensor w, c10::optional<at::Tensor> bias,
-                      int64_t stride, int64_t pt, int64_t pb, int64_t pl,
-                      int64_t pr, bool reflect, int64_t act, double slope) {
+static std::vector<at::Tensor> run_fwd(ConvParams& p, at::Tensor& y,
+                                       bool is_convt, bool want_stats) {
+  std::vector<at::Tensor> out{y};
+  int tps = 0;
+  int ns = want_stats ? stats_slabs(p, is_convt, &tps) : 0;
+  if (ns > 0) {
+    auto ps = at::empty({2, ns, (long)p.B, (long)p.Cout},
+                        y.options().dtype(at::kFloat));
+    p.psum = (float*)ps.mutable_data_ptr();
+    p.psq = p.psum + (long)ns * p.B * p.Cout;
+    p.tps = tps;
+    out.push_back(ps[0]);
+    out.push_back(ps[1]);
+  }
+  launch_conv(p, is_convt, at::cuda::getCurrentCUDAStream());
+  return out;
+}
+
+static std::vector<at::Tensor> conv2d_fwd_impl(
+    at::Tensor x, at::Tensor w, c10::optional<at::Tensor> bias,
+    int64_t stride, int64_t pt, int64_t pb, int64_t pl, int64_t pr,
+    bool reflect, int64_t act, double slope, bool want_stats) {
   check_conv_inputs(x, w);
   int H = x.size(1), W = x.size(2);
   int KH = w.size(1), KW = w.size(2);
@@ -1746,19 +1836,48 @@
   auto y = at::empty({x.size(0), OH, OW, w.size(0)}, x.options());
   auto p = fill_common(x, w, bias, y, stride, act, slope);
   p.pt = pt; p.pl = pl; p.reflect = reflect ? 1 : 0;
-  launch_conv(p, false, at::cuda::getCurrentCUDAStream());
-  return y;
-}
-
-at::Tensor convt2d_fwd(at::Tensor x, at::Tensor w, c10::optional<at::Tensor> bias,
-                       int64_t stride, int64_t pt, int64_t pl,
-                       int64_t out_h, int64_t out_w, int64_t act, double slope) {
+  return run_fwd(p, y, false, want_stats);
+}
+
+static std::vector<at::Tensor> convt2d_fwd_impl(
+    at::Tensor x, at::Tensor w, c10::optional<at::Tensor> bias,
+    int64_t stride, int64_t pt, int64_t pl, int64_t out_h, int64_t out_w,
+    int64_t act, double slope, bool want_stats) {
   check_conv_inputs(x, w);
   auto y = at::empty({x.size(0), out_h, out_w, w.size(0)}, x.options());
   auto p = fill_common(x, w, bias, y, stride, act, slope);
   p.pt = pt; p.pl = pl; p.reflect = 0;
-  launch_conv(p, true, at::cuda::getCurrentCUDAStream());
-  return y;
+  return run_fwd(p, y, true, want_stats);
+}
+
+at::Tensor conv2d_fwd(at::Tensor x, at::Tensor w, c10::optional<at::Tensor> bias,
+                      int64_t stride, int64_t pt, int64_t pb, int64_t pl,
+                      int64_t pr, bool reflect, int64_t act, double slope) {
+  return conv2d_fwd_impl(x, w, bias, stride, pt, pb, pl, pr, reflect, act,
+                         slope, false)[0];
+}
+
+std::vector<at::Tensor> conv2d_fwd_stats(
+    at::Tensor x, at::Tensor w, c10::optional<at::Tensor> bias,
+    int64_t stride, int64_t pt, int64_t pb, int64_t pl, int64_t pr,
+    bool reflect, int64_t act, double slope) {
+  return conv2d_fwd_impl(x, w, bias, stride, pt, pb, pl, pr, reflect, act,
+                         slope, true);
+}
+
+at::Tensor convt2d_fwd(at::Tensor x, at::Tensor w, c10::optional<at::Tensor> bias,
+                       int64_t stride, int64_t pt, int64_t pl,
+                       int64_t out_h, int64_t out_w, int64_t act, double slope) {
+  return convt2d_fwd_impl(x, w, bias, stride, pt, pl, out_h, out_w, act,
+                          slope, false)[0];
+}
+
+std::vector<at::Tensor> convt2d_fwd_stats(
+    at::Tensor x, at::Tensor w, c10::optional<at::Tensor> bias,
+    int64_t stride, int64_t pt, int64_t pl, int64_t out_h, int64_t out_w,
+    int64_t act, double slope) {
+  return convt2d_fwd_impl(x, w, bias, stride, pt, pl, out_h, out_w, act,
+                          slope, true);
 }
 
 at::Tensor conv2d_dgrad(at::Tensor dy, at::Tensor wt, int64_t H, int64_t W,
diff --git a/cyclegan_amd/ops/_hip/norm_elem.hip b/cyclegan_amd/ops/_hip/norm_elem.hip
--- a/cyclegan_amd/ops/_hip/norm_elem.hip
+++ b/cyclegan_amd/ops/_hip/norm_elem.hip
@@ -121,13 +121,17 @@
   }
 }
 
+DEV float in_affine(float xv, float m, float rs, float g, float b) {
+  return __fmaf_rn((xv - m) * rs, g, b);
+}
+
 constexpr int MAXC = 2048;
 __global__ __launch_bounds__(NT) void in_norm_kernel(
     const short* __restrict__ x, const float* __restrict__ gamma,
     const float* __restrict__ beta, const float* __restrict__ psum,
     const float* __restrict__ psq, float* __restrict__ mean,
     float* __restrict__ rstd, const short* __restrict__ res,
-    short* __restrict__ y, int B, long HW, int C, int S, int act,
+    short* __restrict__ y, int B, long HW, int C, int S, int NS, int act,
     float slope, float eps) {
   int b = blockIdx.x / S;
   int sl = blockIdx.x % S;
@@ -149,7 +153,7 @@
     for (int c = tid; c < C; c += NT) {
       float sv = 0, qv = 0;
       int k = 0;
-      for (; k + 4 <= S; k += 4) {
+      for (; k + 4 <= NS; k += 4) {
         float s0 = psum[((long)(k + 0) * B + b) * C + c];
         float s1 = psum[((long)(k + 1) * B + b) * C + c];
         float s2 = psum[((long)(k + 2) * B + b) * C + c];
@@ -161,7 +165,7 @@
         sv += (s0 + s1) + (s2 + s3);
         qv += (q0 + q1) + (q2 + q3);
       }
-      for (; k < S; ++k) {
+      for (; k < NS; ++k) {
         sv += psum[((long)k * B + b) * C + c];
         qv += psq[((long)k * B + b) * C + c];
       }
@@ -182,7 +186,7 @@
     const int c = tid - kc * C;
     float sv = 0, qv = 0;
     int k = kc;
-    for (; k + 3 * PS < S; k += 4 * PS) {
+    for (; k + 3 * PS < NS; k += 4 * PS) {
       float s0 = psum[((long)(k + 0 * PS) * B + b) * C + c];
       float s1 = psum[((long)(k + 1 * PS) * B + b) * C + c];
       float s2 = psum[((long)(k + 2 * PS) * B + b) * C + c];
@@ -194,7 +198,7 @@
       sv += (s0 + s1) + (s2 + s3);
       qv += (q0 + q1) + (q2 + q3);
     }
-    for (; k < S; k += PS) {
+    for (; k < NS; k += PS) {
       sv += psum[((long)k * B + b) * C + c];
       qv += psq[((long)k * B + b) * C + c];
     }
@@ -235,7 +239,7 @@
       #pragma unroll
       for (int j = 0; j < 8; ++j) {
         int c = g * 8 + j;
-        float val = (b2f(v[j]) - sm[c]) * sr[c] * gamma[c] + beta[c];
+        float val = in_affine(b2f(v[j]), sm[c], sr[c], gamma[c], beta[c]);
         if (res) val += b2f(rv[j]);
         out[j] = f2b(apply_act(val, act, slope));
       }
@@ -244,6 +248,7 @@
   }
 }
 
+constexpr int MASK_NONE = 0, MASK_YACT = 1, MASK_X = 2;
 DEV float actbw(float d, float yy, int act, float slope) {
   if (act == ACT_RELU) return yy > 0.f ? d : 0.f;
   if (act == ACT_LRELU) return yy > 0.f ? d : d * slope;
@@ -251,9 +256,11 @@
   return d;
 }
 
+template <int MM>
 __global__ __launch_bounds__(NT) void in_bwd_reduce_kernel(
     const short* __restrict__ dy, const short* __restrict__ x,
-    const short* __restrict__ yact, const float* __restrict__ mean,
+    const short* __restrict__ yact, const float* __restrict__ gamma,
+    const float* __restrict__ beta, const float* __restrict__ mean,
     const float* __restrict__ rstd,
     float* __restrict__ p1, float* __restrict__ p2, int B, long HW, int C,
     int S, int act, float slope, float* __restrict__ dgb) {
@@ -271,11 +278,15 @@
   int rstep = NT / gpr;
   int rof = tid / gpr;
   float a1[8] = {}, a2[8] = {};
-  float mv[8], rv[8];
+  float mv[8], rv[8], gv[8] = {}, bv[8] = {};
   #pragma unroll
   for (int j = 0; j < 8; ++j) {
     mv[j] = mean[(long)b * C + g * 8 + j];
     rv[j] = rstd[(long)b * C + g * 8 + j];
+    if (MM == MASK_X) {
+      gv[j] = gamma[g * 8 + j];
+      bv[j] = beta[g * 8 + j];
+    }
   }
   #pragma unroll 4
   for (long r = r0 + rof; r < r1; r += rstep) {
@@ -283,12 +294,15 @@
     v8s dv = *(const v8s*)(dy + off);
     v8s xv = *(const v8s*)(x + off);
     v8s yv = {};
-    if (act != ACT_NONE) yv = *(const v8s*)(yact + off);
+    if (MM == MASK_YACT) yv = *(const v8s*)(yact + off);
     #pragma unroll
     for (int j = 0; j < 8; ++j) {
       float d = b2f(dv[j]);
-      if (act != ACT_NONE) d = actbw(d, b2f(yv[j]), act, slope);
-      float xh = (b2f(xv[j]) - mv[j]) * rv[j];
+      float xf = b2f(xv[j]);
+      if (MM == MASK_YACT) d = actbw(d, b2f(yv[j]), act, slope);
+      if (MM == MASK_X)
+        d = actbw(d, in_affine(xf, mv[j], rv[j], gv[j], bv[j]), act, slope);
+      float xh = (xf - mv[j]) * rv[j];
       a1[j] += d; a2[j] += d * xh;
     }
   }
@@ -313,10 +327,11 @@
 
 
 
+template <int MM>
 __global__ __launch_bounds__(NT) void in_bwd_dx_kernel(
     const short* __restrict__ dy, const short* __restrict__ x,
     const short* __restrict__ yact, const float* __restrict__ gamma,
-    const float* __restrict__ mean,
+    const float* __restrict__ beta, const float* __restrict__ mean,
     const float* __restrict__ rstd, const float* __restrict__ p1,
     const float* __restrict__ p2, short* __restrict__ dx,
     float* __restrict__ dbeta, float* __restrict__ dgamma, int B, long HW,
@@ -423,15 +438,19 @@
       v8s dv = *(const v8s*)(dy + off);
       v8s xv = *(const v8s*)(x + off);
       v8s yv = {};
-      if (act != ACT_NONE) yv = *(const v8s*)(yact + off);
+      if (MM == MASK_YACT) yv = *(const v8s*)(yact + off);
       v8s out;
       #pragma unroll
       for (int j = 0; j < 8; ++j) {
         int c = g * 8 + j;
         float rs = srstd[c];
-        float xh = (b2f(xv[j]) - smean[c]) * rs;
+        float xf = b2f(xv[j]);
+        float xh = (xf - smean[c]) * rs;
         float d = b2f(dv[j]);
-        if (act != ACT_NONE) d = actbw(d, b2f(yv[j]), act, slope);
+        if (MM == MASK_YACT) d = actbw(d, b2f(yv[j]), act, slope);
+        if (MM == MASK_X)
+          d = actbw(d, in_affine(xf, smean[c], rs, gamma[c], beta[c]), act,
+                    slope);
         out[j] = f2b(gamma[c] * rs * (d - sm1[c] - xh * sm2[c]));
       }
       *(v8s*)(dx + off) = out;
@@ -444,9 +463,11 @@
 typedef __attribute__((address_space(1))) unsigned long long gu64;
 typedef __attribute__((address_space(1))) unsigned int gu32;
 
+template <int MM>
 __global__ __launch_bounds__(NT) void in_bwd_fused_kernel(
     const short* __restrict__ dy, const short* __restrict__ x,
     const short* __restrict__ yact, const float* __restrict__ gamma,
+    const float* __restrict__ beta,
     const float* __restrict__ mean, const float* __restrict__ rstd,
     unsigned long long* __restrict__ gq,
     unsigned int* __restrict__ arrive,
@@ -466,11 +487,15 @@
   int rstep = NT / gpr;
   int rof = tid / gpr;
   float a1[8] = {}, a2[8] = {};
-  float mv[8], rv[8];
+  float mv[8], rv[8], gv[8] = {}, bv[8] = {};
   #pragma unroll
   for (int j = 0; j < 8; ++j) {
     mv[j] = mean[(long)b * C + g * 8 + j];
     rv[j] = rstd[(long)b * C + g * 8 + j];
+    if (MM == MASK_X) {
+      gv[j] = gamma[g * 8 + j];
+      bv[j] = beta[g * 8 + j];
+    }
   }
   #pragma unroll 4
   for (long r = r0 + rof; r < r1; r += rstep) {
@@ -478,12 +503,15 @@
     v8s dv = *(const v8s*)(dy + off);
     v8s xv = *(const v8s*)(x + off);
     v8s yv = {};
-    if (act != ACT_NONE) yv = *(const v8s*)(yact + off);
+    if (MM == MASK_YACT) yv = *(const v8s*)(yact + off);
     #pragma unroll
     for (int j = 0; j < 8; ++j) {
       float d = b2f(dv[j]);
-      if (act != ACT_NONE) d = actbw(d, b2f(yv[j]), act, slope);
-      float xh = (b2f(xv[j]) - mv[j]) * rv[j];
+      float xf = b2f(xv[j]);
+      if (MM == MASK_YACT) d = actbw(d, b2f(yv[j]), act, slope);
+      if (MM == MASK_X)
+        d = actbw(d, in_affine(xf, mv[j], rv[j], gv[j], bv[j]), act, slope);
+      float xh = (xf - mv[j]) * rv[j];
       a1[j] += d; a2[j] += d * xh;
     }
   }
@@ -571,15 +599,19 @@
     v8s dv = *(const v8s*)(dy + off);
     v8s xv = *(const v8s*)(x + off);
     v8s yv = {};
-    if (act != ACT_NONE) yv = *(const v8s*)(yact + off);
+    if (MM == MASK_YACT) yv = *(const v8s*)(yact + off);
     v8s out;
     #pragma unroll
     for (int j = 0; j < 8; ++j) {
       int c = g * 8 + j;
       float rs = srstd[c];
-      float xh = (b2f(xv[j]) - smean[c]) * rs;
+      float xf = b2f(xv[j]);
+      float xh = (xf - smean[c]) * rs;
       float d = b2f(dv[j]);
-      if (act != ACT_NONE) d = actbw(d, b2f(yv[j]), act, slope);
+      if (MM == MASK_YACT) d = actbw(d, b2f(yv[j]), act, slope);
+      if (MM == MASK_X)
+        d = actbw(d, in_affine(xf, smean[c], rs, gamma[c], beta[c]), act,
+                  slope);
       out[j] = f2b(gamma[c] * rs * (d - sm1[c] - xh * sm2[c]));
     }
     *(v8s*)(dx + off) = out;
@@ -705,7 +737,7 @@
     #pragma unroll
     for (int j = 0; j < 8; ++j) {
       int c = g * 8 + j;
-      float val = (b2f(v[j]) - sm[c]) * sr[c] * gamma[c] + beta[c];
+      float val = in_affine(b2f(v[j]), sm[c], sr[c], gamma[c], beta[c]);
       if (res) val += b2f(rv[j]);
       out[j] = f2b(apply_act(val, act, slope));
     }
@@ -791,6 +823,27 @@
   int ih = mirror_idx(qh - pt, H);
   int iw = mirror_idx(qw - pl, W);
   y[i] = x[(((long)b * H + ih) * W + iw) * C + c];
+}
+
+template <typename IDX>
+__global__ __launch_bounds__(256) void reflect_pad_fwd_vec_kernel(
+    const short* __restrict__ x, short* __restrict__ y, int B, int H, int W,
+    int C, int pt, int pb, int pl, int pr) {
+  const int HP = H + pt + pb, WP = W + pl + pr;
+  const IDX gpr = (IDX)(C / 8);
+  const IDX total = (IDX)B * HP * WP * gpr;
+  IDX i = (IDX)blockIdx.x * 256 + threadIdx.x;
+  if (i >= total) return;
+  IDX t = i / gpr;
+  int g = (int)(i - t * gpr);
+  IDX t2 = t / (IDX)WP;
+  int qw = (int)(t - t2 * WP);
+  IDX b = t2 / (IDX)HP;
+  int qh = (int)(t2 - b * HP);
+  int ih = mirror_idx(qh - pt, H);
+  int iw = mirror_idx(qw - pl, W);
+  long src = (((long)b * H + ih) * W + iw) * C + g * 8;
+  *(v8s*)(y + (long)i * 8) = *(const v8s*)(x + src);
 }
 
 __global__ void reflect_pad_bwd_kernel(const short* __restrict__ dyp,
@@ -931,7 +984,10 @@
 std::vector<at::Tensor> instnorm_fwd(at::Tensor x, at::Tensor gamma,
                                      at::Tensor beta, double eps, int64_t act,
                                      double slope,
-                                     c10::optional<at::Tensor> residual) {
+                                     c10::optional<at::Tensor> residual,
+                                     c10::optional<at::Tensor> psum_in,
+                                     c10::optional<at::Tensor> psq_in,
+                                     int64_t nslabs) {
   TORCH_CHECK(x.is_cuda() && x.scalar_type() == at::kBFloat16 && x.is_contiguous());
   int B = x.size(0), C = x.size(3);
   long HW = (long)x.size(1) * x.size(2);
@@ -945,6 +1001,27 @@
   auto y = at::empty_like(x);
   const short* resf = residual.has_value()
                           ? (const short*)residual->const_data_ptr() : nullptr;
+
+  if (psum_in.has_value()) {
+    TORCH_CHECK(psq_in.has_value() && nslabs >= 1 &&
+                psum_in->scalar_type() == at::kFloat &&
+                psq_in->scalar_type() == at::kFloat &&
+                psum_in->is_contiguous() && psq_in->is_contiguous() &&
+                psum_in->numel() == nslabs * B * C &&
+                psq_in->numel() == nslabs * B * C,
+                "instnorm_fwd: bad precomputed slabs");
+    hipLaunchKernelGGL(in_norm_kernel, dim3(B * S), dim3(NT), 0, stream,
+                       (const short*)x.const_data_ptr(),
+                       (const float*)gamma.const_data_ptr(),
+                       (const float*)beta.const_data_ptr(),
+                       (const float*)psum_in->const_data_ptr(),
+                       (const float*)psq_in->const_data_ptr(),
+                       (float*)mean.mutable_data_ptr(),
+                       (float*)rstd.mutable_data_ptr(), resf,
+                       (short*)y.mutable_data_ptr(), B, HW, C, S,
+                       (int)nslabs, (int)act, (float)slope, (float)eps);
+    return {y, mean, rstd};
+  }
 
   static int fused_cap = []() {
     if (const char* e = getenv("CYG_IN_FUSED"); !(e && e[0] == '1')) return 0;
@@ -1002,8 +1079,8 @@
                        (const float*)beta.const_data_ptr(), nullptr, nullptr,
                        (float*)mean.mutable_data_ptr(),
                        (float*)rstd.mutable_data_ptr(), res,
-                       (short*)y.mutable_data_ptr(), B, HW, C, S, (int)act,
-                       (float)slope, (float)eps);
+                       (short*)y.mutable_data_ptr(), B, HW, C, S, S,
+                       (int)act, (float)slope, (float)eps);
     return {y, mean, rstd};
   }
   hipLaunchKernelGGL(in_norm_kernel, dim3(B * S), dim3(NT), 0, stream,
@@ -1014,18 +1091,42 @@
                      (const float*)psq.const_data_ptr(),
                      (float*)mean.mutable_data_ptr(),
                      (float*)rstd.mutable_data_ptr(), res,
-                     (short*)y.mutable_data_ptr(), B, HW, C, S, (int)act,
-                     (float)slope, (float)eps);
+                     (short*)y.mutable_data_ptr(), B, HW, C, S, S,
+                     (int)act, (float)slope, (float)eps);
   return {y, mean, rstd};
 }
+
+#define LAUNCH_MM(kern, mm, grid, stream, ...)                              \
+  do {                                                                      \
+    if ((mm) == MASK_X)                                                     \
+      hipLaunchKernelGGL(kern<MASK_X>, grid, dim3(NT), 0, stream,           \
+                         __VA_ARGS__);                                      \
+    else if ((mm) == MASK_YACT)                                             \
+      hipLaunchKernelGGL(kern<MASK_YACT>, grid, dim3(NT), 0, stream,        \
+                         __VA_ARGS__);                                      \
+    else                                                                    \
+      hipLaunchKernelGGL(kern<MASK_NONE>, grid, dim3(NT), 0, stream,        \
+                         __VA_ARGS__);                                      \
+  } while (0)
 
 std::vector<at::Tensor> instnorm_bwd(at::Tensor dy, at::Tensor x,
                                      at::Tensor gamma, at::Tensor mean,
                                      at::Tensor rstd,
                                      c10::optional<at::Tensor> yact,
-                                     int64_t act, double slope) {
+                                     int64_t act, double slope,
+                                     c10::optional<at::Tensor> beta) {
   TORCH_CHECK(dy.is_cuda() && dy.scalar_type() == at::kBFloat16 &&
               dy.is_contiguous() && x.is_contiguous());
+  TORCH_CHECK(act == ACT_NONE || yact.has_value() ||
+              ((act == ACT_RELU || act == ACT_LRELU) && beta.has_value()),
+              "instnorm_bwd: act ", act, " needs yact (or beta for relu/lrelu)");
+  TORCH_CHECK(!beta.has_value() ||
+              (beta->scalar_type() == at::kFloat && beta->numel() == x.size(3)),
+              "instnorm_bwd: beta must be fp32 [C]");
+  const float* betap =
+      beta.has_value() ? (const float*)beta->const_data_ptr() : nullptr;
+  const int mm = act == ACT_NONE ? MASK_NONE
+                                 : (yact.has_value() ? MASK_YACT : MASK_X);
   int B = x.size(0), C = x.size(3);
   long HW = (long)x.size(1) * x.size(2);
   TORCH_CHECK(C % 8 == 0 && (C / 8) <= 256 && 256 % std::min(C / 8, 256) == 0,
@@ -1045,7 +1146,8 @@
     int bpc = 0, ncu = 0, dev = 0;
     if (hipGetDevice(&dev) != hipSuccess) return 0;
     if (hipOccupancyMaxActiveBlocksPerMultiprocessor(
-            &bpc, (const void*)in_bwd_fused_kernel, NT, 0) != hipSuccess)
+            &bpc, (const void*)in_bwd_fused_kernel<MASK_YACT>, NT, 0) !=
+        hipSuccess)
       return 0;
     if (hipDeviceGetAttribute(&ncu, hipDeviceAttributeMultiprocessorCount,
                               dev) != hipSuccess)
@@ -1061,10 +1163,10 @@
                              stream));
     CHECK_HIP(hipMemsetAsync(dgb.mutable_data_ptr(), 0,
                              (size_t)2 * C * 4, stream));
-    hipLaunchKernelGGL(in_bwd_fused_kernel, dim3(B * Sf), dim3(NT), 0,
+    LAUNCH_MM(in_bwd_fused_kernel, mm, dim3(B * Sf),
                        stream, (const short*)dy.const_data_ptr(),
                        (const short*)x.const_data_ptr(), yp,
-                       (const float*)gamma.const_data_ptr(),
+                       (const float*)gamma.const_data_ptr(), betap,
                        (const float*)mean.const_data_ptr(),
                        (const float*)rstd.const_data_ptr(),
                        (unsigned long long*)gq.mutable_data_ptr(),
@@ -1078,9 +1180,10 @@
 
   auto p1 = at::empty({S, B, C}, fopt);
   auto p2 = at::empty({S, B, C}, fopt);
-  hipLaunchKernelGGL(in_bwd_reduce_kernel, dim3(B * S), dim3(NT), 0, stream,
+  LAUNCH_MM(in_bwd_reduce_kernel, mm, dim3(B * S), stream,
                      (const short*)dy.const_data_ptr(),
                      (const short*)x.const_data_ptr(), yp,
+                     (const float*)gamma.const_data_ptr(), betap,
                      (const float*)mean.const_data_ptr(),
                      (const float*)rstd.const_data_ptr(),
                      (float*)p1.mutable_data_ptr(),
@@ -1100,10 +1203,10 @@
                        (float*)s2m.mutable_data_ptr(),
                        (float*)dbeta.mutable_data_ptr(),
                        (float*)dgamma.mutable_data_ptr(), B, HW, C, S);
-    hipLaunchKernelGGL(in_bwd_dx_kernel, dim3(B * S), dim3(NT), 0, stream,
+    LAUNCH_MM(in_bwd_dx_kernel, mm, dim3(B * S), stream,
                        (const short*)dy.const_data_ptr(),
                        (const short*)x.const_data_ptr(), yp,
-                       (const float*)gamma.const_data_ptr(),
+                       (const float*)gamma.const_data_ptr(), betap,
                        (const float*)mean.const_data_ptr(),
                        (const float*)rstd.const_data_ptr(),
                        (const float*)s1m.const_data_ptr(),
@@ -1114,10 +1217,10 @@
                        (int)act, (float)slope);
     return {dx, dgamma, dbeta};
   }
-  hipLaunchKernelGGL(in_bwd_dx_kernel, dim3(B * S), dim3(NT), 0, stream,
+  LAUNCH_MM(in_bwd_dx_kernel, mm, dim3(B * S), stream,
                      (const short*)dy.const_data_ptr(),
                      (const short*)x.const_data_ptr(), yp,
-                     (const float*)gamma.const_data_ptr(),
+                     (const float*)gamma.const_data_ptr(), betap,
                      (const float*)mean.const_data_ptr(),
                      (const float*)rstd.const_data_ptr(),
                      (const float*)p1.const_data_ptr(),
@@ -1166,6 +1269,33 @@
   int B = x.size(0), H = x.size(1), W = x.size(2), C = x.size(3);
   auto y = at::empty({B, H + pt + pb, W + pl + pr, C}, x.options());
   long total = y.numel();
+  TORCH_CHECK(pt >= 0 && pb >= 0 && pl >= 0 && pr >= 0 && pt < H && pb < H &&
+              pl < W && pr < W, "reflect_pad: pads must be in [0, size)");
+  static const bool no_vec = []() {
+    const char* e = getenv("CYG_NO_PAD_VEC");
+    return e && e[0] == '1';
+  }();
+  const bool al16 = ((uintptr_t)x.const_data_ptr() % 16) == 0 &&
+                    ((uintptr_t)y.const_data_ptr() % 16) == 0;
+  if (!no_vec && C % 8 == 0 && al16 && total > 0) {
+    long nvec = total / 8;
+    TORCH_CHECK((nvec + 255) / 256 < (1L << 31), "reflect_pad: too large");
+    dim3 grid((unsigned)((nvec + 255) / 256));
+    if (nvec < (1L << 31) - 256) {
+      hipLaunchKernelGGL(reflect_pad_fwd_vec_kernel<unsigned>, grid,
+                         dim3(256), 0, at::cuda::getCurrentCUDAStream(),
+                         (const short*)x.const_data_ptr(),
+                         (short*)y.mutable_data_ptr(), B, H, W, C, (int)pt,
+                         (int)pb, (int)pl, (int)pr);
+    } else {
+      hipLaunchKernelGGL(reflect_pad_fwd_vec_kernel<unsigned long>, grid,
+                         dim3(256), 0, at::cuda::getCurrentCUDAStream(),
+                         (const short*)x.const_data_ptr(),
+                         (short*)y.mutable_data_ptr(), B, H, W, C, (int)pt,
+                         (int)pb, (int)pl, (int)pr);
+    }
+    return y;
+  }
   hipLaunchKernelGGL(reflect_pad_fwd_kernel, dim3(cdiv64(total, 256)),
                      dim3(256), 0, at::cuda::getCurrentCUDAStream(),
                      (const short*)x.const_data_ptr(),
diff --git a/cyclegan_amd/ops/conv.py b/cyclegan_amd/ops/conv.py
--- a/cyclegan_amd/ops/conv.py
+++ b/cyclegan_amd/ops/conv.py
@@ -63,6 +63,21 @@
     return y.permute(0, 2, 3, 1)
 
 
+IN_SLABS_ATTR = "_cyg_in_slabs"
+
+
+def _want_stats(bias, act) -> bool:
+    return bias is None and act == ACT_NONE
+
+
+def _attach_slabs(out):
+    if isinstance(out, tuple):
+        y, psum, psq = out
+        setattr(y, IN_SLABS_ATTR, (psum, psq))
+        return y
+    return out
+
+
 def _pad_channels(t: torch.Tensor, c_to: int = 8) -> torch.Tensor:
     c = t.shape[-1]
     if c >= c_to:
@@ -79,16 +94,27 @@
         xp = _pad_channels(x).contiguous()
         wc = compute_weight_p(w, x)
         bc = compute_bias_p(bias, x) if bias is not None else None
-        y = ext.conv2d_fwd(xp, wc, bc, stride, *pads, reflect, act, slope)
+        slabs = ()
+        if _want_stats(bias, act) and cout >= 8:
+            y, *slabs = ext.conv2d_fwd_stats(xp, wc, bc, stride, *pads,
+                                             reflect, act, slope)
+        else:
+            y = ext.conv2d_fwd(xp, wc, bc, stride, *pads, reflect, act, slope)
         if cout < 8:
             y = y[..., :cout].contiguous()
         ctx.save_for_backward(xp, w, y)
         ctx.conf = (stride, pads, reflect, act, slope, bias is not None,
                     x.shape[3])
-        return y
-
-    @staticmethod
-    def backward(ctx, dy):
+        if slabs:
+            ctx.set_materialize_grads(False)
+            ctx.mark_non_differentiable(*slabs)
+            return (y, *slabs)
+        return y
+
+    @staticmethod
+    def backward(ctx, dy, *_):
+        if dy is None:
+            return (None,) * 8
         xp, w, y = ctx.saved_tensors
         stride, pads, reflect, act, slope, has_bias, cin = ctx.conf
         cout = w.shape[0]
@@ -230,13 +256,25 @@
         ext = backend.ext()
         wc = compute_weight(w, x)
         bc = compute_weight(bias, x) if bias is not None else None
-        y = ext.convt2d_fwd(x, wc, bc, stride, pt, pl, out_h, out_w, act, slope)
+        slabs = ()
+        if _want_stats(bias, act):
+            y, *slabs = ext.convt2d_fwd_stats(x, wc, bc, stride, pt, pl,
+                                              out_h, out_w, act, slope)
+        else:
+            y = ext.convt2d_fwd(x, wc, bc, stride, pt, pl, out_h, out_w, act,
+                                slope)
         ctx.save_for_backward(x, w, y)
         ctx.conf = (stride, pt, pl, act, slope, bias is not None)
-        return y
-
-    @staticmethod
-    def backward(ctx, dy):
+        if slabs:
+            ctx.set_materialize_grads(False)
+            ctx.mark_non_differentiable(*slabs)
+            return (y, *slabs)
+        return y
+
+    @staticmethod
+    def backward(ctx, dy, *_):
+        if dy is None:
+            return (None,) * 10
         x, w, y = ctx.saved_tensors
         stride, pt, pl, act, slope, has_bias = ctx.conf
         ext = backend.ext()
@@ -286,7 +324,8 @@
                      or w.shape[1] == 4)):
             return _ConvFp8Fn.apply(x, w, bias, stride, pads,
                                     pad_mode == "reflect", a, slope)
-        return _ConvFn.apply(x, w, bias, stride, pads, pad_mode == "reflect", a, slope)
+        return _attach_slabs(_ConvFn.apply(x, w, bias, stride, pads,
+                                           pad_mode == "reflect", a, slope))
     wc = w if w.dtype == x.dtype else w.to(x.dtype)
     bc = bias if (bias is None or bias.dtype == x.dtype) else bias.to(x.dtype)
     y = _conv_ref(x, wc, bc, stride, pads, pad_mode)
@@ -306,7 +345,8 @@
     pt, _, pl, _ = same_pads(out_h, out_w, kh, kw, stride)
     a = _ACT[act]
     if backend.use_hip(x, w):
-        return _ConvTFn.apply(x, w, bias, stride, pt, pl, out_h, out_w, a, slope)
+        return _attach_slabs(_ConvTFn.apply(x, w, bias, stride, pt, pl, out_h,
+                                            out_w, a, slope))
     wc = w if w.dtype == x.dtype else w.to(x.dtype)
     bc = bias if (bias is None or bias.dtype == x.dtype) else bias.to(x.dtype)
     y = _convt_ref(x, wc, bc, stride, pt, pl, out_h, out_w)
diff --git a/cyclegan_amd/ops/norm.py b/cyclegan_amd/ops/norm.py
--- a/cyclegan_amd/ops/norm.py
+++ b/cyclegan_amd/ops/norm.py
@@ -1,12 +1,13 @@
 
 from __future__ import annotations
 
+import os
 from typing import Optional
 
 import torch
 
 from . import backend
-from .conv import ACT_NONE, ACT_RELU, ACT_LRELU, _ACT
+from .conv import ACT_NONE, ACT_RELU, ACT_LRELU, IN_SLABS_ATTR, _ACT
 
 EPS_DEFAULT = 1e-3
 
@@ -28,19 +29,30 @@
     return y
 
 
+def _mask_from_x(act: int) -> bool:
+    return (act in (ACT_RELU, ACT_LRELU)
+            and os.environ.get("CYG_IN_BWD_MASK_X") == "1")
+
+
 class _InstNormFn(torch.autograd.Function):
     @staticmethod
-    def forward(ctx, x, gamma, beta, eps, act, slope, residual):
+    def forward(ctx, x, gamma, beta, eps, act, slope, residual, psum, psq):
         ext = backend.ext()
-        y, mean, rstd = ext.instnorm_fwd(x, gamma.float(), beta.float(), eps, act, slope,
-                                         residual)
-        ctx.save_for_backward(x, gamma, mean, rstd, y)
+        betaf = beta.float()
+        if psum is not None:
+            y, mean, rstd = ext.instnorm_fwd(x, gamma.float(), betaf, eps, act,
+                                             slope, residual, psum, psq,
+                                             psum.shape[0])
+        else:
+            y, mean, rstd = ext.instnorm_fwd(x, gamma.float(), betaf, eps, act,
+                                             slope, residual)
+        ctx.save_for_backward(x, gamma, mean, rstd, y, betaf)
         ctx.conf = (eps, act, slope, residual is not None)
         return y
 
     @staticmethod
     def backward(ctx, dy):
-        x, gamma, mean, rstd, y = ctx.saved_tensors
+        x, gamma, mean, rstd, y, betaf = ctx.saved_tensors
         eps, act, slope, has_res = ctx.conf
         ext = backend.ext()
         dy = dy.contiguous()
@@ -51,10 +63,23 @@
                                                  rstd, None, ACT_NONE, 0.0)
         else:
             dres = dy if has_res else None
+            yact = y if (act != ACT_NONE and not _mask_from_x(act)) else None
             dx, dgamma, dbeta = ext.instnorm_bwd(
-                dy, x, gamma.float(), mean, rstd,
-                y if act != ACT_NONE else None, act, slope)
-        return (dx, dgamma.to(gamma.dtype), dbeta, None, None, None, dres)
+                dy, x, gamma.float(), mean, rstd, yact, act, slope, betaf)
+        return (dx, dgamma.to(gamma.dtype), dbeta, None, None, None, dres,
+                None, None)
+
+
+def _slabs_for(x: torch.Tensor):
+    st = getattr(x, IN_SLABS_ATTR, None)
+    if st is None or x.dim() != 4:
+        return None, None
+    psum, psq = st
+    want = (x.shape[0], x.shape[3])
+    if (psum.dim() != 3 or tuple(psum.shape[1:]) != want
+            or psq.shape != psum.shape or psum.device != x.device):
+        return None, None
+    return psum, psq
 
 
 def instance_norm(
@@ -68,5 +93,7 @@
 ) -> torch.Tensor:
     a = _ACT[act]
     if backend.use_hip(x, gamma):
-        return _InstNormFn.apply(x, gamma, beta, eps, a, slope, residual)
+        psum, psq = _slabs_for(x)
+        return _InstNormFn.apply(x, gamma, beta, eps, a, slope, residual,
+                                 psum, psq)
     return _in_ref(x, gamma, beta, eps, a, slope, residual)
```

New measurement: 335.5 images/s, median of 6. +2.9%, better.
